# caishiqing/voice-tts

Measured on AMD Instinct MI355X. Metric: audio_seconds_per_second, higher is better.
Workload: dtype bf16

## Files before the change

### include/ixtts_hip.h

```cpp
#ifndef IXTTS_HIP_H
#define IXTTS_HIP_H

#include <stddef.h>
#include <stdint.h>

#ifdef __cplusplus
extern "C" {
#endif

#define IXTTS_OK 0
#define IXTTS_ERR_ARG (-1)
#define IXTTS_ERR_HIP (-2)
#define IXTTS_ERR_STATE (-3)
#define IXTTS_ERR_NOMEM (-4)
#define IXTTS_ERR_NAME (-5)

const char* ixtts_version(void);
const char* ixtts_last_error(void);

int ixtts_aa_snake_f32(const float* x_dev, float* y_dev, const float* up12_dev, const float* down12_dev,
                       const float* log_alpha_dev, const float* log_beta_dev, int B, int C, int T, void* stream);

size_t ixtts_attn_full_workspace_bytes(int B, int H, int T);
int ixtts_attn_full_f32(const float* q_dev, const float* k_dev, const float* v_dev, float* out_dev, int B, int H, int T,
                        int head_dim, long stride_b, long stride_t, long stride_h, long ostride_b, long ostride_t,
                        long ostride_h, float scale, void* workspace_dev, size_t workspace_bytes, void* stream);

size_t ixtts_attn_full_varlen_workspace_bytes(int nseq, int H, int total_tiles);
int ixtts_attn_full_varlen_f32(const float* q_dev, const float* k_dev, const float* v_dev, float* out_dev, const int* table_dev, int nseq,
                               int total_tiles, int n_work, int H, int head_dim, long stride_t, long stride_h, long ostride_t, long ostride_h,
                               float scale, void* workspace_dev, size_t workspace_bytes, void* stream);

int ixtts_adaln_rmsnorm_f32(const float* x_dev, const float* wb_dev, const float* g_dev, float* out_dev, int B, int T, int H, float eps,
                            void* stream);
int ixtts_ln_modulate_f32(const float* x_dev, const float* shift_scale_dev, float* out_dev, int B, int T, int H, float eps, void* stream);
int ixtts_rope_qk_f32(float* qkv_dev, const float* cos_sin_dev, int B, int T, int H, int head_dim, void* stream);
int ixtts_swiglu_f32(const float* u_dev, float* out_dev, long rows, int F, void* stream);
int ixtts_wn_gate_f32(const float* a_dev, const float* g_dev, float* out_dev, int B, int C, int T, long g_stride, int g_offset, void* stream);
int ixtts_wn_gate_rows_f32(const float* a_dev, const float* g_dev, float* out_dev, long rows, int C, long rows_per_batch, int B, long g_stride,
                           int g_offset, void* stream);
int ixtts_reflect_halo_rows_f32(float* p_dev, int B, int T, int C, int left, int right, void* stream);

int ixtts_adaln_rmsnorm_varlen_f32(const float* x_dev, const float* wb_dev, const float* g_dev, float* out_dev, const int* seq_off_dev, int nseq,
                                   long rows, int H, float eps, void* stream);
int ixtts_ln_modulate_varlen_f32(const float* x_dev, const float* shift_scale_dev, float* out_dev, const int* seq_off_dev, int nseq, long rows, int H,
                                 float eps, void* stream);
int ixtts_rope_qk_varlen_f32(float* qkv_dev, const float* cos_sin_dev, const int* seq_off_dev, int nseq, long rows, int H, int head_dim, void* stream);
int ixtts_wn_gate_rows_varlen_f32(const float* a_dev, const float* g_dev, float* out_dev, long rows, int C, const int* seq_off_dev, int nseq,
                                  long g_stride, int g_offset, void* stream);
int ixtts_reflect_halo_rows_varlen_f32(float* p_dev, const int* seq_off_dev, int nseq, int C, int left, int right, void* stream);

size_t ixtts_gemm_x6_packed_bytes(int N, int K);
int ixtts_gemm_x6_pack(const float* w_dev, void* packed_dev, int N, int K, void* stream);
long ixtts_gemm_x6_rows_padded(long rows);
int ixtts_gemm_x6_split(const float* a_dev, long lda, void* planes_dev, long rows, int K, void* stream);
int ixtts_gemm_x6_f32(const void* a_planes_dev, long rows_total, long row0, const void* packed_dev, const float* bias_dev, float* c_dev, long ldc,
                      int M, int N, int K, int accumulate, int tile, void* stream);
int ixtts_gemm_x6_pair_f32(const void* a_planes_dev, long rows_total, long row0, int taps, const void* packed_dev, const float* bias_dev,
                           const float* gate_dev, long gate_ld, long rows_per_batch, int nbatch, float* c_dev, long ldc, int M, int N, int K,
                           int epilogue, int tile, void* stream);
int ixtts_gemm_x6_pair_gate_varlen_f32(const void* a_planes_dev, long rows_total, long row0, int taps, const void* packed_dev, const float* bias_dev,
                                       const float* gate_dev, long gate_ld, const int* seq_off_dev, int nseq, float* c_dev, long ldc, int M, int N,
                                       int K, int tile, void* stream);

#define IXTTS_BIGVGAN_MAX_STAGES 8
#define IXTTS_BIGVGAN_MAX_RESK 4

typedef struct ixtts_bigvgan_cfg {
  int num_mels;
  int upsample_initial_channel;
  int n_stages;
  int upsample_rates[IXTTS_BIGVGAN_MAX_STAGES];
  int upsample_kernel_sizes[IXTTS_BIGVGAN_MAX_STAGES];
  int n_resblock_kernels;
  int resblock_kernel_sizes[IXTTS_BIGVGAN_MAX_RESK];
  int resblock_dilations[IXTTS_BIGVGAN_MAX_RESK][3];
  int max_frames;
  int fast_sin;
} ixtts_bigvgan_cfg;

typedef struct ixtts_bigvgan ixtts_bigvgan;

int ixtts_bigvgan_create(ixtts_bigvgan** out, const ixtts_bigvgan_cfg* cfg);
int ixtts_bigvgan_set_tensor(ixtts_bigvgan* h, const char* name, const float* data_host, const int64_t* shape, int ndim);
int ixtts_bigvgan_finalize(ixtts_bigvgan* h);
int ixtts_bigvgan_arena(ixtts_bigvgan* h, void** ptr_dev, size_t* bytes);
int ixtts_bigvgan_adopt_arena(ixtts_bigvgan* h);
int ixtts_bigvgan_forward(ixtts_bigvgan* h, const float* mel_dev, int B, int F, float* wav_dev, void* stream);
int ixtts_bigvgan_forward_varlen(ixtts_bigvgan* h, const float* mel_dev, const int* frames_dev, const int* frames_host, int B, int Fmax,
                                 float* wav_dev, void* stream);
double ixtts_bigvgan_flops(const ixtts_bigvgan* h, int B, int F);
int ixtts_bigvgan_destroy(ixtts_bigvgan* h);

#define IXTTS_DTYPE_F32 0
#define IXTTS_DTYPE_BF16 1
#define IXTTS_DTYPE_F16 2

typedef struct ixtts_gpt_cfg {
  int model_dim;
  int layers;
  int heads;
  int n_mel_codes;
  int n_mel_pos;
  int n_text_tokens;
  int n_text_pos;
  int start_mel_token;
  int stop_mel_token;
  int max_seq;
  int max_batch;
  int weight_dtype;
} ixtts_gpt_cfg;

#define IXTTS_NGRAM_MAX 8
#define IXTTS_SEQ_BIAS_MAX 64
#define IXTTS_SEQ_BIAS_LEN 8

typedef struct ixtts_sampler_cfg {
  float repetition_penalty;
  float temperature;
  int top_k;
  float top_p;
  int do_sample;
  int suppress_stop;
  uint64_t seed;
  float typical_mass;
  float length_penalty;
  int min_new_tokens;
  int no_repeat_ngram_size;
  float min_p;
  int exp_decay_start;
  double exp_decay_factor;
  float epsilon_cutoff;
  float eta_cutoff;
  int renormalize_logits;
  int forced_eos_step;
  int n_seq_bias;
} ixtts_sampler_cfg;

typedef struct ixtts_gpt ixtts_gpt;

// ... 103 lines not shown
```

### voice-tts_amd/_lib.py

```python
import ctypes as C
import os

HERE = os.path.dirname(os.path.abspath(__file__))
LIB_PATH = os.environ.get("IXTTS_LIB") or os.path.join(HERE, "libixtts_hip.so")

MAX_STAGES = 8
MAX_RESK = 4


class BigVGANCfg(C.Structure):
    _fields_ = [
        ("num_mels", C.c_int), ("upsample_initial_channel", C.c_int), ("n_stages", C.c_int),
        ("upsample_rates", C.c_int * MAX_STAGES), ("upsample_kernel_sizes", C.c_int * MAX_STAGES),
        ("n_resblock_kernels", C.c_int), ("resblock_kernel_sizes", C.c_int * MAX_RESK),
        ("resblock_dilations", (C.c_int * 3) * MAX_RESK), ("max_frames", C.c_int), ("fast_sin", C.c_int),
    ]


class GptCfg(C.Structure):
    _fields_ = [
        ("model_dim", C.c_int), ("layers", C.c_int), ("heads", C.c_int), ("n_mel_codes", C.c_int),
        ("n_mel_pos", C.c_int), ("n_text_tokens", C.c_int), ("n_text_pos", C.c_int),
        ("start_mel_token", C.c_int), ("stop_mel_token", C.c_int), ("max_seq", C.c_int),
        ("max_batch", C.c_int), ("weight_dtype", C.c_int),
    ]


class SamplerCfg(C.Structure):
    _fields_ = [
        ("repetition_penalty", C.c_float), ("temperature", C.c_float), ("top_k", C.c_int),
        ("top_p", C.c_float), ("do_sample", C.c_int), ("suppress_stop", C.c_int), ("seed", C.c_uint64),
        ("typical_mass", C.c_float), ("length_penalty", C.c_float),
        ("min_new_tokens", C.c_int), ("no_repeat_ngram_size", C.c_int), ("min_p", C.c_float),
        ("exp_decay_start", C.c_int), ("exp_decay_factor", C.c_double), ("epsilon_cutoff", C.c_float), ("eta_cutoff", C.c_float),
        ("renormalize_logits", C.c_int), ("forced_eos_step", C.c_int), ("n_seq_bias", C.c_int),
    ]


NGRAM_MAX = 8
SEQ_BIAS_MAX = 64
SEQ_BIAS_LEN = 8

QWEN_TOPK_MAX = 64
QWEN_MAX_EOS = 8
QWEN_MAX_SLOTS = 4


class QwenCfg(C.Structure):
    _fields_ = [
        ("hidden_size", C.c_int), ("layers", C.c_int), ("heads", C.c_int), ("kv_heads", C.c_int), ("head_dim", C.c_int),
        ("intermediate_size", C.c_int), ("vocab_size", C.c_int), ("rms_norm_eps", C.c_float), ("rope_theta", C.c_float),
        ("tie_word_embeddings", C.c_int), ("max_seq", C.c_int), ("weight_dtype", C.c_int), ("n_eos", C.c_int),
        ("eos_ids", C.c_int * QWEN_MAX_EOS),
    ]


class QwenSampling(C.Structure):
    _fields_ = [("do_sample", C.c_int), ("temperature", C.c_float), ("top_k", C.c_int), ("top_p", C.c_float), ("seed", C.c_uint64)]


_P = C.c_void_p
SYMBOLS = {
    "ixtts_version": (C.c_char_p, []),
    "ixtts_last_error": (C.c_char_p, []),
    "ixtts_aa_snake_f32": (C.c_int, [_P, _P, _P, _P, _P, _P, C.c_int, C.c_int, C.c_int, _P]),
    "ixtts_attn_full_workspace_bytes": (C.c_size_t, [C.c_int, C.c_int, C.c_int]),
    "ixtts_attn_full_f32": (C.c_int, [_P, _P, _P, _P, C.c_int, C.c_int, C.c_int, C.c_int, C.c_long, C.c_long, C.c_long, C.c_long, C.c_long,
                                      C.c_long, C.c_float, _P, C.c_size_t, _P]),
    "ixtts_attn_full_varlen_workspace_bytes": (C.c_size_t, [C.c_int, C.c_int, C.c_int]),
    "ixtts_attn_full_varlen_f32": (C.c_int, [_P, _P, _P, _P, _P, C.c_int, C.c_int, C.c_int, C.c_int, C.c_int, C.c_long, C.c_long, C.c_long, C.c_long,
                                             C.c_float, _P, C.c_size_t, _P]),
    "ixtts_adaln_rmsnorm_f32": (C.c_int, [_P, _P, _P, _P, C.c_int, C.c_int, C.c_int, C.c_float, _P]),
    "ixtts_ln_modulate_f32": (C.c_int, [_P, _P, _P, C.c_int, C.c_int, C.c_int, C.c_float, _P]),
    "ixtts_rope_qk_f32": (C.c_int, [_P, _P, C.c_int, C.c_int, C.c_int, C.c_int, _P]),
    "ixtts_swiglu_f32": (C.c_int, [_P, _P, C.c_long, C.c_int, _P]),
    "ixtts_wn_gate_f32": (C.c_int, [_P, _P, _P, C.c_int, C.c_int, C.c_int, C.c_long, C.c_int, _P]),
    "ixtts_wn_gate_rows_f32": (C.c_int, [_P, _P, _P, C.c_long, C.c_int, C.c_long, C.c_int, C.c_long, C.c_int, _P]),
    "ixtts_reflect_halo_rows_f32": (C.c_int, [_P, C.c_int, C.c_int, C.c_int, C.c_int, C.c_int, _P]),
    "ixtts_adaln_rmsnorm_varlen_f32": (C.c_int, [_P, _P, _P, _P, _P, C.c_int, C.c_long, C.c_int, C.c_float, _P]),
    "ixtts_ln_modulate_varlen_f32": (C.c_int, [_P, _P, _P, _P, C.c_int, C.c_long, C.c_int, C.c_float, _P]),
    "ixtts_rope_qk_varlen_f32": (C.c_int, [_P, _P, _P, C.c_int, C.c_long, C.c_int, C.c_int, _P]),
    "ixtts_wn_gate_rows_varlen_f32": (C.c_int, [_P, _P, _P, C.c_long, C.c_int, _P, C.c_int, C.c_long, C.c_int, _P]),
    "ixtts_reflect_halo_rows_varlen_f32": (C.c_int, [_P, _P, C.c_int, C.c_int, C.c_int, C.c_int, _P]),
    "ixtts_gemm_x6_packed_bytes": (C.c_size_t, [C.c_int, C.c_int]),
    "ixtts_gemm_x6_pack": (C.c_int, [_P, _P, C.c_int, C.c_int, _P]),
    "ixtts_gemm_x6_rows_padded": (C.c_long, [C.c_long]),
    "ixtts_gemm_x6_split": (C.c_int, [_P, C.c_long, _P, C.c_long, C.c_int, _P]),
    "ixtts_gemm_x6_f32": (C.c_int, [_P, C.c_long, C.c_long, _P, _P, _P, C.c_long, C.c_int, C.c_int, C.c_int, C.c_int, C.c_int, _P]),
    "ixtts_gemm_x6_pair_f32": (C.c_int, [_P, C.c_long, C.c_long, C.c_int, _P, _P, _P, C.c_long, C.c_long, C.c_int, _P, C.c_long, C.c_int, C.c_int,
                                         C.c_int, C.c_int, C.c_int, _P]),
    "ixtts_gemm_x6_pair_gate_varlen_f32": (C.c_int, [_P, C.c_long, C.c_long, C.c_int, _P, _P, _P, C.c_long, _P, C.c_int, _P, C.c_long, C.c_int, C.c_int,
                                                     C.c_int, C.c_int, _P]),
    "ixtts_bigvgan_create": (C.c_int, [C.POINTER(_P), C.POINTER(BigVGANCfg)]),
    "ixtts_bigvgan_set_tensor": (C.c_int, [_P, C.c_char_p, _P, C.POINTER(C.c_int64), C.c_int]),
    "ixtts_bigvgan_finalize": (C.c_int, [_P]),
    "ixtts_bigvgan_arena": (C.c_int, [_P, C.POINTER(_P), C.POINTER(C.c_size_t)]),
    "ixtts_bigvgan_adopt_arena": (C.c_int, [_P]),
    "ixtts_bigvgan_forward": (C.c_int, [_P, _P, C.c_int, C.c_int, _P, _P]),
    "ixtts_bigvgan_forward_varlen": (C.c_int, [_P, _P, _P, _P, C.c_int, C.c_int, _P, _P]),
    "ixtts_bigvgan_flops": (C.c_double, [_P, C.c_int, C.c_int]),
    "ixtts_bigvgan_destroy": (C.c_int, [_P]),
    "ixtts_gpt_create": (C.c_int, [C.POINTER(_P), C.POINTER(GptCfg)]),
    "ixtts_gpt_set_tensor": (C.c_int, [_P, C.c_char_p, _P, C.POINTER(C.c_int64), C.c_int]),
    "ixtts_gpt_finalize": (C.c_int, [_P]),
    "ixtts_gpt_arena": (C.c_int, [_P, C.POINTER(_P), C.POINTER(C.c_size_t)]),
    "ixtts_gpt_adopt_arena": (C.c_int, [_P]),
    "ixtts_gpt_share_arena": (C.c_int, [_P, _P]),
    "ixtts_gpt_prefill": (C.c_int, [_P, C.c_int, _P, C.c_int, C.c_int, _P]),
    "ixtts_gpt_decode": (C.c_int, [_P, C.c_int, C.c_int, C.POINTER(SamplerCfg), _P]),
    "ixtts_gpt_decode_slots": (C.c_int, [_P, C.c_int, C.c_int, C.POINTER(SamplerCfg), C.POINTER(C.c_uint32), _P]),
    "ixtts_gpt_read": (C.c_int, [_P, C.c_int, _P, C.c_int, C.POINTER(C.c_int), C.POINTER(C.c_int), _P]),
    "ixtts_gpt_read_logits": (C.c_int, [_P, C.c_int, _P, _P]),
    "ixtts_gpt_beam_begin": (C.c_int, [_P, C.c_int, _P]),
    "ixtts_gpt_beam_decode": (C.c_int, [_P, C.c_int, C.POINTER(SamplerCfg), _P]),
    "ixtts_gpt_beam_read": (C.c_int, [_P, C.c_int, _P, C.c_int, C.POINTER(C.c_int), C.POINTER(C.c_int), C.POINTER(C.c_float), _P, _P, _P, _P]),
    "ixtts_gpt_beam_force": (C.c_int, [_P, _P, C.c_int, _P]),
    "ixtts_gpt_beam_begin_group": (C.c_int, [_P, C.c_int, C.c_int, C.c_uint64, _P]),
    "ixtts_gpt_beam_park_group": (C.c_int, [_P, C.c_int, _P]),
    "ixtts_gpt_beam_decode_groups": (C.c_int, [_P, C.c_int, C.c_int, C.POINTER(SamplerCfg), _P]),
    "ixtts_gpt_beam_decode_groups_cfg": (C.c_int, [_P, C.c_int, C.c_int, C.POINTER(SamplerCfg), _P]),
    "ixtts_gpt_beam_read_group":(C.c_int, [_P, C.c_int, C.c_int, _P, C.c_int, C.POINTER(C.c_int), C.POINTER(C.c_int), C.POINTER(C.c_float), _P, _P, _P, _P]),
    "ixtts_gpt_beam_force_group": (C.c_int, [_P, C.c_int, _P, C.c_int, _P]),
    "ixtts_gpt_read_probs": (C.c_int, [_P, C.c_int, _P, _P]),
    "ixtts_gpt_force_next": (C.c_int, [_P, C.c_int, C.c_int32, _P]),
    "ixtts_gpt_set_bans": (C.c_int, [_P, C.c_int, _P, C.c_int, _P, C.c_int, _P]),
    "ixtts_gpt_set_sequence_bias": (C.c_int, [_P, C.c_int, _P, _P, _P, C.c_int, _P]),
    "ixtts_gpt_set_forced_eos": (C.c_int, [_P, C.c_int, _P, C.c_int, _P]),
    "ixtts_gpt_latent": (C.c_int, [_P, _P, C.c_int, _P, C.c_int, _P, _P]),
    "ixtts_gpt_bench_gemv": (C.c_int, [_P, C.c_int, C.c_int, C.c_int, _P]),
    "ixtts_gpt_step_bytes": (C.c_double, [_P, C.c_int, C.c_int]),
    "ixtts_gpt_max_batch": (C.c_int, []),
    "ixtts_gpt_max_batch_for": (C.c_int, [C.c_int]),
    "ixtts_gpt_destroy": (C.c_int, [_P]),
    "ixtts_qwen_create": (C.c_int, [C.POINTER(_P), C.POINTER(QwenCfg)]),
    "ixtts_qwen_set_tensor": (C.c_int, [_P, C.c_char_p, _P, C.POINTER(C.c_int64), C.c_int]),
    "ixtts_qwen_finalize": (C.c_int, [_P]),
    "ixtts_qwen_prefill": (C.c_int, [_P, _P, C.c_int, _P]),
    "ixtts_qwen_step": (C.c_int, [_P, C.c_int, C.POINTER(QwenSampling), _P]),
    "ixtts_qwen_read": (C.c_int, [_P, _P, C.c_int, C.POINTER(C.c_int), C.POINTER(C.c_int), _P]),
    "ixtts_qwen_generate": (C.c_int, [_P, C.c_int, C.POINTER(QwenSampling), _P, C.c_int, C.POINTER(C.c_int), C.POINTER(C.c_int), _P]),
    "ixtts_qwen_read_logits": (C.c_int, [_P, _P, _P]),
    "ixtts_qwen_read_kept": (C.c_int, [_P, _P, _P, C.c_int, C.POINTER(C.c_int), _P]),
    "ixtts_qwen_draw": (C.c_int, [_P, C.c_uint64, C.c_int, _P, _P]),
    "ixtts_qwen_step_bytes": (C.c_double, [_P, C.c_int]),
    "ixtts_qwen_create_slots": (C.c_int, [C.POINTER(_P), C.POINTER(QwenCfg), C.c_int]),
    "ixtts_qwen_prefill_slots": (C.c_int, [_P, C.c_int, _P, _P, _P]),
    "ixtts_qwen_step_slots": (C.c_int, [_P, C.c_int, C.c_int, C.POINTER(QwenSampling), _P]),
    "ixtts_qwen_generate_slots": (C.c_int, [_P, C.c_int, C.c_int, C.POINTER(QwenSampling), _P]),
    "ixtts_qwen_read_slot": (C.c_int, [_P, C.c_int, _P, C.c_int, C.POINTER(C.c_int), C.POINTER(C.c_int), _P]),
    "ixtts_qwen_read_logits_slot": (C.c_int, [_P, C.c_int, _P, _P]),
    "ixtts_qwen_read_kept_slot": (C.c_int, [_P, C.c_int, _P, _P, C.c_int, C.POINTER(C.c_int), _P]),
    "ixtts_qwen_destroy": (C.c_int, [_P]),
}

_lib = None


class IxttsError(RuntimeError):
    pass


def lib():
    global _lib
    if _lib is not None:
        return _lib
    import torch
# ... 40 lines not shown
```

### voice-tts_amd/csrc/attn_full.h

```cpp
#pragma once
#include "common.h"

namespace ixtts {

constexpr int AF_D = 64;
constexpr int AF_KT = 64;
constexpr int AF_QW = 32;
constexpr int AF_WAVES = 4;
constexpr int AF_KSPLIT = 4;
constexpr int AX_KSPLIT = 5;

struct AttnFullArgs {
  const float* q;
  const float* k;
  const float* v;
  float* o;
  long sb, st, sh;
  long osb, ost, osh;
  int B, H, T;
  float scale;
  float* ws_o;
  float* ws_ml;
  const int* vl_tab;
  int vl_n, vl_tiles;
};

size_t attn_full_x3_plane_bytes(int B, int H, int T);
int launch_attn_full_x3(const AttnFullArgs& a, void* planes, bool split, hipStream_t st);
int launch_attn_full_x3_varlen(const AttnFullArgs& a, void* planes, int n_work, hipStream_t st);

}
```

### voice-tts_amd/csrc/attn_full.hip

```cpp
#include "attn_full.h"

namespace ixtts {

typedef float f32x16 __attribute__((ext_vector_type(16)));

constexpr int AF_KP = AF_D + 4;

template <int KSPLIT>
__global__ __launch_bounds__(AF_WAVES * 64) void attn_full_f32_kernel(AttnFullArgs a) {
  __shared__ __attribute__((aligned(16))) float Ks[AF_KT * AF_KP];
  __shared__ __attribute__((aligned(16))) float Vs[AF_KT * AF_D];
  const int bh = blockIdx.y, b = bh / a.H, h = bh % a.H;
  const int lane = threadIdx.x & 63, wave = threadIdx.x >> 6;
  const int l31 = lane & 31, lh = lane >> 5;
  const int q0 = blockIdx.x * (AF_WAVES * AF_QW) + wave * AF_QW;
  const float* qb = a.q + b * a.sb + h * a.sh;
  const float* kb = a.k + b * a.sb + h * a.sh;
  const float* vb = a.v + b * a.sb + h * a.sh;

  float qr[AF_D / 2];
  {
    const int qi = min(q0 + l31, a.T - 1);
    const float* qp = qb + (long)qi * a.st + 4 * lh;
    const float qs = a.scale * 1.4426950408889634f;
// ... 78 lines not shown
        for (int r = 0; r < 16; ++r) ot[j][r] *= alpha;
    }
    float psum = 0.f;
    const float* vp = Vs + (4 * lh) * AF_D + l31;
    float va[2][2];
    va[0][0] = vp[0];
    va[0][1] = vp[32];
#pragma unroll
    for (int s = 0; s < 32; ++s) {
      const int j = s >> 4, r = s & 15;
      if (s + 1 < 32) {
        const int j1 = (s + 1) >> 4, r1 = (s + 1) & 15;
        const float* vrow = vp + (j1 * 32 + (r1 & 3) + 8 * (r1 >> 2)) * AF_D;
        va[(s + 1) & 1][0] = vrow[0];
        va[(s + 1) & 1][1] = vrow[32];
      }
      const float pv = __builtin_amdgcn_exp2f(st[j][r] - mn);
      psum += pv;
      ot[0] = __builtin_amdgcn_mfma_f32_32x32x2f32(va[s & 1][0], pv, ot[0], 0, 0, 0);
      ot[1] = __builtin_amdgcn_mfma_f32_32x32x2f32(va[s & 1][1], pv, ot[1], 0, 0, 0);
    }
    psum += __shfl_xor(psum, 32, 64);
    l_run = l_run * alpha + psum;
  }
  const int qi = q0 + l31;
  if (qi < a.T) {
    if constexpr (KSPLIT == 1) {
      const float inv = 1.0f / l_run;
      float* op = a.o + b * a.osb + (long)qi * a.ost + h * a.osh;
#pragma unroll
      for (int j = 0; j < 2; ++j)
#pragma unroll
        for (int r = 0; r < 16; ++r) op[j * 32 + (r & 3) + 8 * (r >> 2) + 4 * lh] = ot[j][r] * inv;
    } else {
      const long row = ((long)blockIdx.z * a.B * a.H + bh) * a.T + qi;
      float* op = a.ws_o + row * AF_D;
#pragma unroll
      for (int j = 0; j < 2; ++j)
#pragma unroll
        for (int r = 0; r < 16; ++r) op[j * 32 + (r & 3) + 8 * (r >> 2) + 4 * lh] = ot[j][r];
      if (lh == 0) *reinterpret_cast<float2*>(a.ws_ml + row * 2) = make_float2(m_run, l_run);
    }
  }
}

template <int KSPLIT>
__global__ __launch_bounds__(256) void attn_full_merge_kernel(AttnFullArgs a) {
  const long row = (long)blockIdx.x * 4 + (threadIdx.x >> 6);
  const long rows = (long)a.B * a.H * a.T;
  if (row >= rows) return;
  const int d = threadIdx.x & 63;
  const int t = (int)(row % a.T);
  const int bh = (int)(row / a.T), b = bh / a.H, h = bh % a.H;
  float2 ml[KSPLIT];
  float o[KSPLIT];
  float M = -INFINITY;
#pragma unroll
  for (int sp = 0; sp < KSPLIT; ++sp) {
    ml[sp] = *reinterpret_cast<const float2*>(a.ws_ml + ((long)sp * rows + row) * 2);
    o[sp] = a.ws_o[((long)sp * rows + row) * AF_D + d];
    M = fmaxf(M, ml[sp].x);
  }
  float L = 0.f, O = 0.f;
#pragma unroll
  for (int sp = 0; sp < KSPLIT; ++sp) {
    const float w = (ml[sp].x > -INFINITY) ? __builtin_amdgcn_exp2f(ml[sp].x - M) : 0.f;
    L = fmaf(ml[sp].y, w, L);
    O = fmaf(o[sp], w, O);
  }
  a.o[b * a.osb + (long)t * a.ost + h * a.osh + d] = O / L;
}

}

static size_t attn_partials_bytes(int B, int H, int T) {
  return (size_t)(ixtts::AF_KSPLIT > ixtts::AX_KSPLIT ? ixtts::AF_KSPLIT : ixtts::AX_KSPLIT) * B * H * T * (ixtts::AF_D + 2) * sizeof(float);
}

extern "C" size_t ixtts_attn_full_workspace_bytes(int B, int H, int T) {
  if (B <= 0 || H <= 0 || T <= 0) return 0;
  return attn_partials_bytes(B, H, T) + ixtts::attn_full_x3_plane_bytes(B, H, T);
}

extern "C" int ixtts_attn_full_f32(const float* q_dev, const float* k_dev, const float* v_dev, float* out_dev, int B, int H, int T,
                                   int head_dim, long stride_b, long stride_t, long stride_h, long ostride_b, long ostride_t,
                                   long ostride_h, float scale, void* workspace_dev, size_t workspace_bytes, void* stream) {
  using namespace ixtts;
  IX_ARG(q_dev && k_dev && v_dev && out_dev, "attn_full: null pointer");
  IX_ARG(head_dim == AF_D, "attn_full: head_dim %d (only 64 is built)", head_dim);
  IX_ARG(B > 0 && H > 0 && T > 0 && (long)B * H <= 65535, "attn_full: bad shape B=%d H=%d T=%d", B, H, T);
  IX_ARG(stride_t % 4 == 0 && stride_h % 4 == 0 && stride_b % 4 == 0, "attn_full: strides must keep 16-byte row alignment");
  AttnFullArgs a;
  a.q = q_dev; a.k = k_dev; a.v = v_dev; a.o = out_dev;
  a.sb = stride_b; a.st = stride_t; a.sh = stride_h;
  a.osb = ostride_b; a.ost = ostride_t; a.osh = ostride_h;
  a.B = B; a.H = H; a.T = T; a.scale = scale;
  a.ws_o = a.ws_ml = nullptr;
  a.vl_tab = nullptr; a.vl_n = a.vl_tiles = 0;
  hipStream_t st = (hipStream_t)stream;
  const int qblocks = ceil_div(T, AF_WAVES * AF_QW);
  const bool have_ws = workspace_dev && workspace_bytes >= ixtts_attn_full_workspace_bytes(B, H, T);
  const bool split = have_ws && T > 4 * AF_KT && (long)qblocks * B * H * AF_WAVES < 2 * 1024;
  const char* mode = getenv("IXTTS_ATTN_FULL");
  const bool x3 = !(mode && strcmp(mode, "f32") == 0);
  const bool use_x3 = x3 && have_ws;
  if (split) {
    a.ws_o = reinterpret_cast<float*>(workspace_dev);
    a.ws_ml = a.ws_o + (size_t)(use_x3 ? AX_KSPLIT : AF_KSPLIT) * B * H * T * AF_D;
  }
  if (use_x3) {
    IX_TRY(launch_attn_full_x3(a, reinterpret_cast<char*>(workspace_dev) + attn_partials_bytes(B, H, T), split, st));
    if (split) {
      const long rows = (long)B * H * T;
      hipLaunchKernelGGL(attn_full_merge_kernel<AX_KSPLIT>, dim3((unsigned)((rows + 3) / 4)), dim3(256), 0, st, a);
    }
    IX_HIP(hipGetLastError());
    return IXTTS_OK;
  }
  if (split) {
    hipLaunchKernelGGL(attn_full_f32_kernel<AF_KSPLIT>, dim3(qblocks, B * H, AF_KSPLIT), dim3(AF_WAVES * 64), 0, st, a);
    const long rows = (long)B * H * T;
    hipLaunchKernelGGL(attn_full_merge_kernel<AF_KSPLIT>, dim3((unsigned)((rows + 3) / 4)), dim3(256), 0, st, a);
  } else {
    hipLaunchKernelGGL(attn_full_f32_kernel<1>, dim3(qblocks, B * H), dim3(AF_WAVES * 64), 0, st, a);
  }
  IX_HIP(hipGetLastError());
  return IXTTS_OK;
}

extern "C" size_t ixtts_attn_full_varlen_workspace_bytes(int nseq, int H, int total_tiles) {
  if (nseq <= 0 || H <= 0 || total_tiles <= 0) return 0;
  return (size_t)H * total_tiles * 2 * 3 * 8 * 64 * 16;
}

extern "C" int ixtts_attn_full_varlen_f32(const float* q_dev, const float* k_dev, const float* v_dev, float* out_dev, const int* table_dev, int nseq,
                                          int total_tiles, int n_work, int H, int head_dim, long stride_t, long stride_h, long ostride_t, long ostride_h,
                                          float scale, void* workspace_dev, size_t workspace_bytes, void* stream) {
  using namespace ixtts;
  IX_ARG(q_dev && k_dev && v_dev && out_dev && table_dev, "attn_full_varlen: null pointer");
  IX_ARG(head_dim == AF_D, "attn_full_varlen: head_dim %d (only 64 is built)", head_dim);
  IX_ARG(nseq > 0 && total_tiles >= nseq && n_work >= nseq && H > 0 && H <= 65535, "attn_full_varlen: bad shape nseq=%d tiles=%d work=%d H=%d", nseq, total_tiles,
         n_work, H);
  IX_ARG(stride_t % 4 == 0 && stride_h % 4 == 0, "attn_full_varlen: strides must keep 16-byte row alignment");
  IX_ARG(workspace_dev && workspace_bytes >= ixtts_attn_full_varlen_workspace_bytes(nseq, H, total_tiles), "attn_full_varlen: workspace of %zu bytes, %zu needed",
         workspace_bytes, ixtts_attn_full_varlen_workspace_bytes(nseq, H, total_tiles));
  AttnFullArgs a;
  a.q = q_dev; a.k = k_dev; a.v = v_dev; a.o = out_dev;
  a.sb = 0; a.st = stride_t; a.sh = stride_h;
  a.osb = 0; a.ost = ostride_t; a.osh = ostride_h;
  a.B = 1; a.H = H; a.T = 0; a.scale = scale;
  a.ws_o = a.ws_ml = nullptr;
  a.vl_tab = table_dev; a.vl_n = nseq; a.vl_tiles = total_tiles;
  return launch_attn_full_x3_varlen(a, workspace_dev, n_work, (hipStream_t)stream);
}
```

### voice-tts_amd/csrc/attn_full_x3.hip

```cpp
#include "attn_full.h"

namespace ixtts {

typedef float ax_f32x16 __attribute__((ext_vector_type(16)));
typedef __bf16 ax_bf16x8 __attribute__((ext_vector_type(8)));

constexpr int AX_TILE_UNITS = 3 * 8 * 64;
constexpr int AX_WAVES = 4;

size_t attn_full_x3_plane_bytes(int B, int H, int T) {
  const size_t tiles = (size_t)(T + AF_KT - 1) / AF_KT;
  return (size_t)B * H * tiles * 2 * AX_TILE_UNITS * 16;
}


template <bool VL>
__global__ __launch_bounds__(256) void attn_kv_planes_kernel(AttnFullArgs a, uint4* __restrict__ planes) {
  int tile = blockIdx.x, T = a.T;
  const float *kb, *vb;
  uint4* kdst;
  if constexpr (VL) {
    const int h = blockIdx.y, s = seq_of_row(a.vl_tab + a.vl_n + 1, a.vl_n, tile);
    const int r0 = a.vl_tab[s];
    T = a.vl_tab[s + 1] - r0;
    kdst = planes + ((size_t)h * a.vl_tiles + tile) * 2 * AX_TILE_UNITS;
    tile -= a.vl_tab[a.vl_n + 1 + s];
    kb = a.k + (long)r0 * a.st + h * a.sh;
    vb = a.v + (long)r0 * a.st + h * a.sh;
  } else {
    const int bh = blockIdx.y, b = bh / a.H, h = bh % a.H;
    const int n_tiles = (a.T + AF_KT - 1) / AF_KT;
    kb = a.k + b * a.sb + h * a.sh;
    vb = a.v + b * a.sb + h * a.sh;
    kdst = planes + ((size_t)bh * n_tiles + tile) * 2 * AX_TILE_UNITS;
  }
  uint4* vdst = kdst + AX_TILE_UNITS;
  const int t0 = tile * AF_KT;
#pragma unroll
  for (int i = 0; i < 2; ++i) {
    const int uid = threadIdx.x + 256 * i;
    const int key = uid >> 3, oct = uid & 7;
    const int t = t0 + key;
    float v[8];
    const float4* src = reinterpret_cast<const float4*>(kb + (long)min(t, T - 1) * a.st + 8 * oct);
    const float4 x0 = src[0], x1 = src[1];
    const bool live = t < T;
    v[0] = live ? x0.x : 0.f; v[1] = live ? x0.y : 0.f; v[2] = live ? x0.z : 0.f; v[3] = live ? x0.w : 0.f;
    v[4] = live ? x1.x : 0.f; v[5] = live ? x1.y : 0.f; v[6] = live ? x1.z : 0.f; v[7] = live ? x1.w : 0.f;
    uint4 ph, pm, pl;
    split8_bf16x3(v, ph, pm, pl);
    kdst[(0 * 8 + oct) * 64 + key] = ph;
    kdst[(1 * 8 + oct) * 64 + key] = pm;
    kdst[(2 * 8 + oct) * 64 + key] = pl;
  }
#pragma unroll
  for (int i = 0; i < 2; ++i) {
    const int d = threadIdx.x & 63, un = (threadIdx.x >> 6) + 4 * i;
    const int j = un >> 2, u = (un >> 1) & 1, kh = un & 1;
    float v[8];
#pragma unroll
    for (int e = 0; e < 8; ++e) {
      const int t = t0 + 32 * j + 16 * u + 8 * (e >> 2) + 4 * kh + (e & 3);
      const float x = vb[(long)min(t, T - 1) * a.st + d];
      v[e] = t < T ? x : 0.f;
    }
    uint4 ph, pm, pl;
    split8_bf16x3(v, ph, pm, pl);
    vdst[(0 * 8 + un) * 64 + d] = ph;
    vdst[(1 * 8 + un) * 64 + d] = pm;
    vdst[(2 * 8 + un) * 64 + d] = pl;
  }
}

template <int KSPLIT, bool VL = false>
__global__ __launch_bounds__(AX_WAVES * 64, 3) void attn_full_x3_kernel(AttnFullArgs a, const uint4* __restrict__ planes) {
  __shared__ uint4 Ks[AX_TILE_UNITS];
  __shared__ uint4 Vs[AX_TILE_UNITS];
  static_assert(!VL || KSPLIT == 1, "packed sequences: no key-range split");
  const int lane = threadIdx.x & 63, wave = threadIdx.x >> 6;
  const int l31 = lane & 31, lh = lane >> 5;
  int T, q0;
  const float* qb;
  const uint4* pb;
  float* ob;
  if constexpr (VL) {
    const int h = blockIdx.y;
    const int* w = a.vl_tab + 2 * (a.vl_n + 1) + 2 * blockIdx.x;
    const int s = w[0], r0 = a.vl_tab[s];
    T = a.vl_tab[s + 1] - r0;
    q0 = w[1] * (AX_WAVES * AF_QW) + wave * AF_QW;
    qb = a.q + (long)r0 * a.st + h * a.sh;
    pb = planes + ((size_t)h * a.vl_tiles + a.vl_tab[a.vl_n + 1 + s]) * 2 * AX_TILE_UNITS;
    ob = a.o + (long)r0 * a.ost + h * a.osh;
  } else {
    const int bh = blockIdx.y, b = bh / a.H, h = bh % a.H;
    T = a.T;
    q0 = blockIdx.x * (AX_WAVES * AF_QW) + wave * AF_QW;
    qb = a.q + b * a.sb + h * a.sh;
    pb = planes + (size_t)bh * ((T + AF_KT - 1) / AF_KT) * 2 * AX_TILE_UNITS;
    ob = a.o + b * a.osb + h * a.osh;
  }

  uint4 qp[4][3];
  {
    const int qi = min(q0 + l31, T - 1);
    const float* qrow = qb + (long)qi * a.st + 8 * lh;
    const float qs = a.scale * 1.4426950408889634f;
#pragma unroll
    for (int s = 0; s < 4; ++s) {
      const float4 x0 = *reinterpret_cast<const float4*>(qrow + 16 * s), x1 = *reinterpret_cast<const float4*>(qrow + 16 * s + 4);
      const float v[8] = {x0.x * qs, x0.y * qs, x0.z * qs, x0.w * qs, x1.x * qs, x1.y * qs, x1.z * qs, x1.w * qs};
      split8_bf16x3(v, qp[s][0], qp[s][1], qp[s][2]);
    }
  }
  ax_f32x16 ot[2];
#pragma unroll
  for (int j = 0; j < 2; ++j)
#pragma unroll
    for (int r = 0; r < 16; ++r) ot[j][r] = 0.f;
  float m_run = -INFINITY, l_run = 0.f;

  const int n_tiles = (T + AF_KT - 1) / AF_KT;
  const int tiles_per = (n_tiles + KSPLIT - 1) / KSPLIT;
  const int tile_lo = KSPLIT > 1 ? blockIdx.z * tiles_per : 0;
  const int tile_hi = KSPLIT > 1 ? min(n_tiles, tile_lo + tiles_per) : n_tiles;
  auto issue_tile = [&](const uint4* __restrict__ src, uint4* __restrict__ dst) {
#pragma unroll
    for (int i = 0; i < AX_TILE_UNITS / (AX_WAVES * 64); ++i)
      __builtin_amdgcn_global_load_lds((const __attribute__((address_space(1))) void*)(src + i * (AX_WAVES * 64) + threadIdx.x),
                                       (__attribute__((address_space(3))) void*)(dst + i * (AX_WAVES * 64) + wave * 64), 16, 0, 0);
  };
  auto mfma6x2 = [](ax_f32x16& c0, ax_f32x16& c1, const uint4 (&A0)[3], const uint4 (&A1)[3], const uint4 (&Bq)[3]) {
    const ax_bf16x8 a0h = __builtin_bit_cast(ax_bf16x8, A0[0]), a0m = __builtin_bit_cast(ax_bf16x8, A0[1]), a0l = __builtin_bit_cast(ax_bf16x8, A0[2]);
    const ax_bf16x8 a1h = __builtin_bit_cast(ax_bf16x8, A1[0]), a1m = __builtin_bit_cast(ax_bf16x8, A1[1]), a1l = __builtin_bit_cast(ax_bf16x8, A1[2]);
    const ax_bf16x8 bh_ = __builtin_bit_cast(ax_bf16x8, Bq[0]), bm = __builtin_bit_cast(ax_bf16x8, Bq[1]), bl = __builtin_bit_cast(ax_bf16x8, Bq[2]);
    c0 = __builtin_amdgcn_mfma_f32_32x32x16_bf16(a0l, bh_, c0, 0, 0, 0);
    c1 = __builtin_amdgcn_mfma_f32_32x32x16_bf16(a1l, bh_, c1, 0, 0, 0);
    c0 = __builtin_amdgcn_mfma_f32_32x32x16_bf16(a0h, bl, c0, 0, 0, 0);
    c1 = __builtin_amdgcn_mfma_f32_32x32x16_bf16(a1h, bl, c1, 0, 0, 0);
    c0 = __builtin_amdgcn_mfma_f32_32x32x16_bf16(a0m, bm, c0, 0, 0, 0);
    c1 = __builtin_amdgcn_mfma_f32_32x32x16_bf16(a1m, bm, c1, 0, 0, 0);
    c0 = __builtin_amdgcn_mfma_f32_32x32x16_bf16(a0m, bh_, c0, 0, 0, 0);
    c1 = __builtin_amdgcn_mfma_f32_32x32x16_bf16(a1m, bh_, c1, 0, 0, 0);
    c0 = __builtin_amdgcn_mfma_f32_32x32x16_bf16(a0h, bm, c0, 0, 0, 0);
    c1 = __builtin_amdgcn_mfma_f32_32x32x16_bf16(a1h, bm, c1, 0, 0, 0);
    c0 = __builtin_amdgcn_mfma_f32_32x32x16_bf16(a0h, bh_, c0, 0, 0, 0);
    c1 = __builtin_amdgcn_mfma_f32_32x32x16_bf16(a1h, bh_, c1, 0, 0, 0);
  };
  if (tile_lo < tile_hi) issue_tile(pb + (size_t)tile_lo * 2 * AX_TILE_UNITS, Ks);
  for (int tile = tile_lo; tile < tile_hi; ++tile) {
    const int t0 = tile * AF_KT;
    asm volatile("s_waitcnt vmcnt(0)" ::: "memory");
    __builtin_amdgcn_s_barrier();
    issue_tile(pb + ((size_t)tile * 2 + 1) * AX_TILE_UNITS, Vs);
    ax_f32x16 st[2];
#pragma unroll
    for (int j = 0; j < 2; ++j)
#pragma unroll
      for (int r = 0; r < 16; ++r) st[j][r] = 0.f;
    const uint4* kp = Ks + lh * 64 + l31;
#pragma unroll
    for (int s = 0; s < 4; ++s) {
      uint4 ka[2][3];
#pragma unroll
      for (int j = 0; j < 2; ++j)
#pragma unroll
        for (int pl = 0; pl < 3; ++pl) ka[j][pl] = kp[(pl * 8 + 2 * s) * 64 + 32 * j];
      mfma6x2(st[0], st[1], ka[0], ka[1], qp[s]);
    }
    if (t0 + AF_KT > T) {
#pragma unroll
      for (int j = 0; j < 2; ++j)
#pragma unroll
        for (int r = 0; r < 16; ++r) {
          const int key = t0 + j * 32 + (r & 3) + 8 * (r >> 2) + 4 * lh;
          if (key >= T) st[j][r] = -INFINITY;
        }
    }
    float tmax = -INFINITY;
#pragma unroll
    for (int j = 0; j < 2; ++j)
#pragma unroll
      for (int r = 0; r < 16; ++r) tmax = fmaxf(tmax, st[j][r]);
    tmax = fmaxf(tmax, __shfl_xor(tmax, 32, 64));
    const float mn = fmaxf(m_run, tmax);
    const float alpha = __builtin_amdgcn_exp2f(m_run - mn);
    m_run = mn;
    if (alpha != 1.0f) {
#pragma unroll
      for (int j = 0; j < 2; ++j)
#pragma unroll
        for (int r = 0; r < 16; ++r) ot[j][r] *= alpha;
    }
    float psum = 0.f;
#pragma unroll
    for (int j = 0; j < 2; ++j)
#pragma unroll
      for (int r = 0; r < 16; ++r) {
        st[j][r] = __builtin_amdgcn_exp2f(st[j][r] - mn);
        psum += st[j][r];
      }
    psum += __shfl_xor(psum, 32, 64);
    l_run = l_run * alpha + psum;
    asm volatile("s_waitcnt vmcnt(0)" ::: "memory");
    __builtin_amdgcn_s_barrier();
    if (tile + 1 < tile_hi) issue_tile(pb + (size_t)(tile + 1) * 2 * AX_TILE_UNITS, Ks);
    const uint4* vp = Vs + lh * 64 + l31;
#pragma unroll
    for (int s = 0; s < 4; ++s) {
      const int j = s >> 1, u = s & 1;
      uint4 va[2][3];
#pragma unroll
      for (int dh = 0; dh < 2; ++dh)
#pragma unroll
        for (int pl = 0; pl < 3; ++pl) va[dh][pl] = vp[(pl * 8 + 2 * s) * 64 + 32 * dh];
      uint4 pp[3];
      {
        float pv[8];
#pragma unroll
        for (int e = 0; e < 8; ++e) pv[e] = st[j][8 * u + e];
        split8_bf16x3(pv, pp[0], pp[1], pp[2]);
      }
      mfma6x2(ot[0], ot[1], va[0], va[1], pp);
    }
  }
  asm volatile("s_waitcnt vmcnt(0)" ::: "memory");
  const int qi = q0 + l31;
  if (qi < T) {
    if constexpr (KSPLIT == 1) {
      const float inv = 1.0f / l_run;
      float* op = ob + (long)qi * a.ost;
#pragma unroll
      for (int j = 0; j < 2; ++j)
#pragma unroll
        for (int r = 0; r < 16; ++r) op[j * 32 + (r & 3) + 8 * (r >> 2) + 4 * lh] = ot[j][r] * inv;
    } else {
      const long row = ((long)blockIdx.z * a.B * a.H + blockIdx.y) * T + qi;
      float* op = a.ws_o + row * AF_D;
#pragma unroll
      for (int j = 0; j < 2; ++j)
#pragma unroll
        for (int r = 0; r < 16; ++r) op[j * 32 + (r & 3) + 8 * (r >> 2) + 4 * lh] = ot[j][r];
      if (lh == 0) *reinterpret_cast<float2*>(a.ws_ml + row * 2) = make_float2(m_run, l_run);
    }
  }
}

int launch_attn_full_x3(const AttnFullArgs& a, void* planes, bool split, hipStream_t st) {
  const int n_tiles = ceil_div(a.T, AF_KT);
  const int qblocks = ceil_div(a.T, AX_WAVES * AF_QW);
  uint4* pl = reinterpret_cast<uint4*>(planes);
  hipLaunchKernelGGL(attn_kv_planes_kernel<false>, dim3(n_tiles, a.B * a.H), dim3(256), 0, st, a, pl);
  if (split) hipLaunchKernelGGL(attn_full_x3_kernel<AX_KSPLIT>, dim3(qblocks, a.B * a.H, AX_KSPLIT), dim3(AX_WAVES * 64), 0, st, a, (const uint4*)pl);
  else hipLaunchKernelGGL(attn_full_x3_kernel<1>, dim3(qblocks, a.B * a.H), dim3(AX_WAVES * 64), 0, st, a, (const uint4*)pl);
  IX_HIP(hipGetLastError());
  return IXTTS_OK;
}

int launch_attn_full_x3_varlen(const AttnFullArgs& a, void* planes, int n_work, hipStream_t st) {
  uint4* pl = reinterpret_cast<uint4*>(planes);
  hipLaunchKernelGGL(attn_kv_planes_kernel<true>, dim3(a.vl_tiles, a.H), dim3(256), 0, st, a, pl);
  hipLaunchKernelGGL((attn_full_x3_kernel<1, true>), dim3(n_work, a.H), dim3(AX_WAVES * 64), 0, st, a, (const uint4*)pl);
  IX_HIP(hipGetLastError());
  return IXTTS_OK;
}

}
```

### voice-tts_amd/csrc/common.h

```cpp
#pragma once
#include <type_traits>
#include <hip/hip_runtime.h>
#include <hip/hip_bf16.h>
#include <stdint.h>
#include <stdio.h>
#include <string.h>
#include <string>

#include "../../include/ixtts_hip.h"

namespace ixtts {

void set_error(const char* fmt, ...);

#define IX_HIP(expr)                                                                   \
  do {                                                                                 \
    hipError_t _e = (expr);                                                            \
    if (_e != hipSuccess) {                                                            \
      ::ixtts::set_error("%s:%d: %s -> %s", __FILE__, __LINE__, #expr, hipGetErrorString(_e)); \
      return IXTTS_ERR_HIP;                                                            \
    }                                                                                  \
  } while (0)

#define IX_ARG(cond, ...)                  \
  do {                                     \
    if (!(cond)) {                         \
      ::ixtts::set_error(__VA_ARGS__);     \
      return IXTTS_ERR_ARG;                \
    }                                      \
  } while (0)

#define IX_TRY(expr)            \
  do {                          \
    int _r = (expr);            \
    if (_r != IXTTS_OK) return _r; \
  } while (0)

static inline int ceil_div(int a, int b) { return (a + b - 1) / b; }
static inline size_t align_up(size_t x, size_t a) { return (x + a - 1) / a * a; }

typedef __hip_bfloat16 bf16;

__device__ __forceinline__ float bf16_bits_to_f32(unsigned short b) {
  return __uint_as_float(((unsigned int)b) << 16);
}
__device__ __forceinline__ int seq_of_row(const int* __restrict__ off, int n, long row) {
  int lo = 0, hi = n - 1;
  while (lo < hi) {
    const int mid = (lo + hi + 1) >> 1;
    if ((long)off[mid] <= row) lo = mid;
    else hi = mid - 1;
  }
  return lo;
}

__device__ __forceinline__ float lo_bf16(unsigned int w) { return __uint_as_float(w << 16); }
__device__ __forceinline__ float hi_bf16(unsigned int w) { return __uint_as_float(w & 0xffff0000u); }

typedef _Float16 f16;
constexpr float F16_MAX = 65504.0f;
__device__ __forceinline__ float lo_f16(unsigned int w) { return (float)__builtin_bit_cast(f16, (unsigned short)(w & 0xffffu)); }
__device__ __forceinline__ float hi_f16(unsigned int w) { return (float)__builtin_bit_cast(f16, (unsigned short)(w >> 16)); }
__device__ __forceinline__ f16 f16_sat(float v) { return (f16)__builtin_fminf(__builtin_fmaxf(v, -F16_MAX), F16_MAX); }
template <typename T>
__device__ __forceinline__ void unpack8(const uint4& r, float (&o)[8]);
template <>
__device__ __forceinline__ void unpack8<bf16>(const uint4& r, float (&o)[8]) {
  o[0] = lo_bf16(r.x); o[1] = hi_bf16(r.x); o[2] = lo_bf16(r.y); o[3] = hi_bf16(r.y);
  o[4] = lo_bf16(r.z); o[5] = hi_bf16(r.z); o[6] = lo_bf16(r.w); o[7] = hi_bf16(r.w);
}
template <>
__device__ __forceinline__ void unpack8<f16>(const uint4& r, float (&o)[8]) {
  o[0] = lo_f16(r.x); o[1] = hi_f16(r.x); o[2] = lo_f16(r.y); o[3] = hi_f16(r.y);
  o[4] = lo_f16(r.z); o[5] = hi_f16(r.z); o[6] = lo_f16(r.w); o[7] = hi_f16(r.w);
}

template <int CTRL, int ROW_MASK, int BANK_MASK>
__device__ __forceinline__ float dpp_take(float v) {
  return __builtin_bit_cast(float, __builtin_amdgcn_update_dpp(0, __builtin_bit_cast(int, v), CTRL, ROW_MASK, BANK_MASK, true));
}
__device__ __forceinline__ float wave_sum63(float v) {
  float s = v + dpp_take<0x111, 0xf, 0xf>(v);
  s += dpp_take<0x112, 0xf, 0xf>(v);
  s += dpp_take<0x113, 0xf, 0xf>(v);
  s += dpp_take<0x114, 0xf, 0xe>(s);
  s += dpp_take<0x118, 0xf, 0xc>(s);
  s += dpp_take<0x142, 0xa, 0xf>(s);
  s += dpp_take<0x143, 0xc, 0xf>(s);
  return s;
}
__device__ __forceinline__ float wave_sum(float v) {
  return __builtin_bit_cast(float, __builtin_amdgcn_readlane(__builtin_bit_cast(int, wave_sum63(v)), 63));
}
__device__ __forceinline__ float wave_max(float v) {
#pragma unroll
  for (int o = 32; o >= 1; o >>= 1) v = fmaxf(v, __shfl_xor(v, o, 64));
  return v;
}
template <int CTRL, int ROW_MASK, int BANK_MASK>
__device__ __forceinline__ float dpp_take_or_self(float v) {
  return __builtin_bit_cast(float, __builtin_amdgcn_update_dpp(__builtin_bit_cast(int, v), __builtin_bit_cast(int, v), CTRL, ROW_MASK, BANK_MASK, false));
}
__device__ __forceinline__ float wave_max_dpp(float v) {
  float s = fmaxf(v, dpp_take_or_self<0x111, 0xf, 0xf>(v));
  s = fmaxf(s, dpp_take_or_self<0x112, 0xf, 0xf>(v));
  s = fmaxf(s, dpp_take_or_self<0x113, 0xf, 0xf>(v));
  s = fmaxf(s, dpp_take_or_self<0x114, 0xf, 0xe>(s));
  s = fmaxf(s, dpp_take_or_self<0x118, 0xf, 0xc>(s));
  s = fmaxf(s, dpp_take_or_self<0x142, 0xa, 0xf>(s));
  s = fmaxf(s, dpp_take_or_self<0x143, 0xc, 0xf>(s));
  return __builtin_bit_cast(float, __builtin_amdgcn_readlane(__builtin_bit_cast(int, s), 63));
}
__device__ __forceinline__ unsigned int wave_scan_u32(unsigned int v) {
  auto take = [](unsigned int x, auto ctrl, auto rm, auto bm) {
    return (unsigned int)__builtin_amdgcn_update_dpp(0, (int)x, decltype(ctrl)::value, decltype(rm)::value, decltype(bm)::value, true);
  };
  using std::integral_constant;
  unsigned int s = v + take(v, integral_constant<int, 0x111>{}, integral_constant<int, 0xf>{}, integral_constant<int, 0xf>{});
  s += take(v, integral_constant<int, 0x112>{}, integral_constant<int, 0xf>{}, integral_constant<int, 0xf>{});
  s += take(v, integral_constant<int, 0x113>{}, integral_constant<int, 0xf>{}, integral_constant<int, 0xf>{});
  s += take(s, integral_constant<int, 0x114>{}, integral_constant<int, 0xf>{}, integral_constant<int, 0xe>{});
  s += take(s, integral_constant<int, 0x118>{}, integral_constant<int, 0xf>{}, integral_constant<int, 0xc>{});
  s += take(s, integral_constant<int, 0x142>{}, integral_constant<int, 0xa>{}, integral_constant<int, 0xf>{});
  s += take(s, integral_constant<int, 0x143>{}, integral_constant<int, 0xc>{}, integral_constant<int, 0xf>{});
  return s;
}

__device__ __forceinline__ int wave_min_i32_dpp(int v) {
  auto take = [](int x, auto ctrl, auto rm, auto bm) {
    return __builtin_amdgcn_update_dpp(x, x, decltype(ctrl)::value, decltype(rm)::value, decltype(bm)::value, false);
  };
  using std::integral_constant;
  int s = min(v, take(v, integral_constant<int, 0x111>{}, integral_constant<int, 0xf>{}, integral_constant<int, 0xf>{}));
  s = min(s, take(v, integral_constant<int, 0x112>{}, integral_constant<int, 0xf>{}, integral_constant<int, 0xf>{}));
  s = min(s, take(v, integral_constant<int, 0x113>{}, integral_constant<int, 0xf>{}, integral_constant<int, 0xf>{}));
  s = min(s, take(s, integral_constant<int, 0x114>{}, integral_constant<int, 0xf>{}, integral_constant<int, 0xe>{}));
// ... 30 lines not shown
```

### voice-tts_amd/csrc/dit_ops.hip

```cpp
#include "common.h"

namespace ixtts {

constexpr int ROW_NV = 8;

template <bool CENTER>
__global__ __launch_bounds__(256) void row_norm_mod_kernel(const float* __restrict__ x, const float* __restrict__ mw, const float* __restrict__ mb,
                                                           const float* __restrict__ g, float* __restrict__ out, long rows, int T, int H, long mstride,
                                                           float eps, float wadd, const int* __restrict__ seq_off = nullptr, int nseq = 0) {
  const long row = (long)blockIdx.x * 4 + (threadIdx.x >> 6);
  if (row >= rows) return;
  const int lane = threadIdx.x & 63;
  const int H4 = H >> 2;
  const float4* xr = reinterpret_cast<const float4*>(x + row * H);
  float4 v[ROW_NV];
#pragma unroll
  for (int i = 0; i < ROW_NV; ++i) {
    const int c = lane + 64 * i;
    v[i] = (c < H4) ? xr[c] : make_float4(0.f, 0.f, 0.f, 0.f);
  }
  float mean = 0.f;
  if constexpr (CENTER) {
    float s = 0.f;
#pragma unroll
    for (int i = 0; i < ROW_NV; ++i) s += (v[i].x + v[i].y) + (v[i].z + v[i].w);
    mean = wave_sum(s) / (float)H;
  }
  float q = 0.f;
#pragma unroll
  for (int i = 0; i < ROW_NV; ++i) {
    const int c = lane + 64 * i;
    if (c < H4) {
      const float a = v[i].x - mean, b = v[i].y - mean, cc = v[i].z - mean, d = v[i].w - mean;
      q += (a * a + b * b) + (cc * cc + d * d);
    }
  }
  float var = wave_sum(q) / (float)H;
  float corr = 0.f;
  if constexpr (CENTER) {
    if (mean * mean > 16.0f * var) {
      float r = 0.f;
#pragma unroll
      for (int i = 0; i < ROW_NV; ++i)
        if (lane + 64 * i < H4) r += ((v[i].x - mean) + (v[i].y - mean)) + ((v[i].z - mean) + (v[i].w - mean));
      corr = wave_sum(r) / (float)H;
      float q2 = 0.f;
#pragma unroll
      for (int i = 0; i < ROW_NV; ++i)
        if (lane + 64 * i < H4) {
          const float a = (v[i].x - mean) - corr, b = (v[i].y - mean) - corr, cc = (v[i].z - mean) - corr, d = (v[i].w - mean) - corr;
          q2 += (a * a + b * b) + (cc * cc + d * d);
        }
      var = wave_sum(q2) / (float)H;
    }
  }
  const float rstd = 1.0f / sqrtf(var + eps);
  const long bidx = seq_off ? seq_of_row(seq_off, nseq, row) : row / T;
  const float4* w4 = reinterpret_cast<const float4*>(mw + bidx * mstride);
  const float4* b4 = reinterpret_cast<const float4*>(mb + bidx * mstride);
  const float4* g4 = reinterpret_cast<const float4*>(g);
  float4* o4 = reinterpret_cast<float4*>(out + row * H);
#pragma unroll
  for (int i = 0; i < ROW_NV; ++i) {
    const int c = lane + 64 * i;
    if (c < H4) {
      const float4 w = w4[c], b = b4[c];
      float4 n;
      if constexpr (CENTER) n = make_float4(((v[i].x - mean) - corr) * rstd, ((v[i].y - mean) - corr) * rstd, ((v[i].z - mean) - corr) * rstd, ((v[i].w - mean) - corr) * rstd);
      else n = make_float4(v[i].x * rstd, v[i].y * rstd, v[i].z * rstd, v[i].w * rstd);
      if (g) {
        const float4 gg = g4[c];
        n.x *= gg.x; n.y *= gg.y; n.z *= gg.z; n.w *= gg.w;
      }
      o4[c] = make_float4(fmaf(w.x + wadd, n.x, b.x), fmaf(w.y + wadd, n.y, b.y), fmaf(w.z + wadd, n.z, b.z), fmaf(w.w + wadd, n.w, b.w));
    }
  }
}

__global__ __launch_bounds__(256) void rope_qk_kernel(float* __restrict__ qkv, const float2* __restrict__ tab, long rows, int T, int H, int hd,
                                                      const int* __restrict__ seq_off = nullptr, int nseq = 0) {
  const int per_row = (2 * H) >> 2;
  const long idx = (long)blockIdx.x * 256 + threadIdx.x;
  if (idx >= rows * per_row) return;
  const long row = idx / per_row;
  const int c4 = (int)(idx % per_row);
  const int col = c4 * 4;
  const int t = seq_off ? (int)(row - seq_off[seq_of_row(seq_off, nseq, row)]) : (int)(row % T);
  const int p = (col % hd) >> 1;
  float4* ptr = reinterpret_cast<float4*>(qkv + row * 3 * H + col);
  const float4 v = *ptr;
  const float2 f0 = tab[(long)t * (hd >> 1) + p], f1 = tab[(long)t * (hd >> 1) + p + 1];
  *ptr = make_float4(v.x * f0.x - v.y * f0.y, v.y * f0.x + v.x * f0.y, v.z * f1.x - v.w * f1.y, v.w * f1.x + v.z * f1.y);
}

__global__ __launch_bounds__(256) void swiglu_kernel(const float* __restrict__ u, float* __restrict__ out, long rows, int Fd) {
  const int F4 = Fd >> 2;
  const long idx = (long)blockIdx.x * 256 + threadIdx.x;
  if (idx >= rows * F4) return;
  const long row = idx / F4;
  const int c = (int)(idx % F4);
  const float4 a = reinterpret_cast<const float4*>(u + row * 2 * Fd)[c];
  const float4 b = reinterpret_cast<const float4*>(u + row * 2 * Fd + Fd)[c];
  auto f = [](float x, float y) { return x / (1.0f + expf(-x)) * y; };
  reinterpret_cast<float4*>(out + row * Fd)[c] = make_float4(f(a.x, b.x), f(a.y, b.y), f(a.z, b.z), f(a.w, b.w));
}

__global__ __launch_bounds__(256) void wn_gate_kernel(const float* __restrict__ a, const float* __restrict__ gvec, float* __restrict__ out, int B, int C, int T,
                                                      long gstride, int goff) {
  const long idx = (long)blockIdx.x * 256 + threadIdx.x;
  const long n = (long)B * C * T;
  if (idx >= n) return;
  const int t = (int)(idx % T);
  const int c = (int)((idx / T) % C);
  const int b = (int)(idx / ((long)T * C));
  const float ga = gvec[b * gstride + goff + c], gb = gvec[b * gstride + goff + C + c];
  const float xa = a[((long)b * 2 * C + c) * T + t] + ga;
  const float xb = a[((long)b * 2 * C + C + c) * T + t] + gb;
  out[idx] = tanhf(xa) * (1.0f / (1.0f + expf(-xb)));
}

__global__ __launch_bounds__(256) void wn_gate_rows_kernel(const float* __restrict__ a, const float* __restrict__ gvec, float* __restrict__ out, long rows, int C,
                                                           long rows_per_batch, int B, long gstride, int goff, const int* __restrict__ seq_off = nullptr) {
  const long idx = (long)blockIdx.x * 256 + threadIdx.x;
  const int C4 = C >> 2;
  if (idx >= rows * C4) return;
  const long r = idx / C4;
  const int c = (int)(idx % C4) * 4;
  const int b = seq_off ? seq_of_row(seq_off, B, r) : (int)min(r / rows_per_batch, (long)B - 1);
  const float4 xa = *reinterpret_cast<const float4*>(a + r * 2 * C + c);
  const float4 xb = *reinterpret_cast<const float4*>(a + r * 2 * C + C + c);
  const float4 ga = *reinterpret_cast<const float4*>(gvec + b * gstride + goff + c);
  const float4 gb = *reinterpret_cast<const float4*>(gvec + b * gstride + goff + C + c);
  float4 o;
  o.x = tanhf(xa.x + ga.x) * (1.0f / (1.0f + expf(-(xb.x + gb.x))));
  o.y = tanhf(xa.y + ga.y) * (1.0f / (1.0f + expf(-(xb.y + gb.y))));
  o.z = tanhf(xa.z + ga.z) * (1.0f / (1.0f + expf(-(xb.z + gb.z))));
  o.w = tanhf(xa.w + ga.w) * (1.0f / (1.0f + expf(-(xb.w + gb.w))));
  *reinterpret_cast<float4*>(out + r * C + c) = o;
}

__global__ __launch_bounds__(256) void reflect_halo_rows_kernel(float* __restrict__ p, int B, int T, int C, int left, int right) {
  const int C4 = C >> 2;
  const long idx = (long)blockIdx.x * 256 + threadIdx.x;
  const long per_b = (long)(left + right) * C4;
  if (idx >= per_b * B) return;
  const int b = (int)(idx / per_b);
  const int h = (int)((idx % per_b) / C4);
  const int c = (int)(idx % C4) * 4;
  float* base = p + (long)b * (left + T + right) * C;
  const int dst = h < left ? left - 1 - h : left + T + (h - left);
  const int src = h < left ? left + h + 1 : left + T - 2 - (h - left);
  *reinterpret_cast<float4*>(base + (long)dst * C + c) = *reinterpret_cast<const float4*>(base + (long)src * C + c);
}

__global__ __launch_bounds__(256) void reflect_halo_rows_varlen_kernel(float* __restrict__ p, const int* __restrict__ off, int n, int C, int left, int right) {
  const int C4 = C >> 2;
  const long idx = (long)blockIdx.x * 256 + threadIdx.x;
  const long per_b = (long)(left + right) * C4;
  if (idx >= per_b * n) return;
  const int b = (int)(idx / per_b);
  const int h = (int)((idx % per_b) / C4);
  const int c = (int)(idx % C4) * 4;
  const int o0 = off[b], T = off[b + 1] - o0 - left - right;
  if (T <= left || T <= right) return;
  float* base = p + (long)o0 * C;
  const int dst = h < left ? left - 1 - h : left + T + (h - left);
  const int src = h < left ? left + h + 1 : left + T - 2 - (h - left);
  *reinterpret_cast<float4*>(base + (long)dst * C + c) = *reinterpret_cast<const float4*>(base + (long)src * C + c);
}

}

using namespace ixtts;

extern "C" int ixtts_adaln_rmsnorm_f32(const float* x_dev, const float* wb_dev, const float* g_dev, float* out_dev, int B, int T, int H, float eps,
                                       void* stream) {
  IX_ARG(x_dev && wb_dev && g_dev && out_dev, "adaln_rmsnorm: null pointer");
  IX_ARG(B > 0 && T > 0 && H > 0 && H % 4 == 0 && H <= 64 * ROW_NV * 4, "adaln_rmsnorm: bad shape B=%d T=%d H=%d", B, T, H);
  const long rows = (long)B * T;
  hipLaunchKernelGGL(row_norm_mod_kernel<false>, dim3((unsigned)((rows + 3) / 4)), dim3(256), 0, (hipStream_t)stream, x_dev, wb_dev, wb_dev + H, g_dev, out_dev,
                     rows, T, H, (long)2 * H, eps, 0.0f);
  IX_HIP(hipGetLastError());
  return IXTTS_OK;
}

extern "C" int ixtts_ln_modulate_f32(const float* x_dev, const float* shift_scale_dev, float* out_dev, int B, int T, int H, float eps, void* stream) {
  IX_ARG(x_dev && shift_scale_dev && out_dev, "ln_modulate: null pointer");
  IX_ARG(B > 0 && T > 0 && H > 0 && H % 4 == 0 && H <= 64 * ROW_NV * 4, "ln_modulate: bad shape B=%d T=%d H=%d", B, T, H);
  const long rows = (long)B * T;
  hipLaunchKernelGGL(row_norm_mod_kernel<true>, dim3((unsigned)((rows + 3) / 4)), dim3(256), 0, (hipStream_t)stream, x_dev, shift_scale_dev + H, shift_scale_dev,
                     (const float*)nullptr, out_dev, rows, T, H, (long)2 * H, eps, 1.0f);
  IX_HIP(hipGetLastError());
  return IXTTS_OK;
}

extern "C" int ixtts_rope_qk_f32(float* qkv_dev, const float* cos_sin_dev, int B, int T, int H, int head_dim, void* stream) {
  IX_ARG(qkv_dev && cos_sin_dev, "rope_qk: null pointer");
  IX_ARG(B > 0 && T > 0 && H > 0 && head_dim > 0 && head_dim % 4 == 0 && H % head_dim == 0, "rope_qk: bad shape B=%d T=%d H=%d hd=%d", B, T, H, head_dim);
  const long n = (long)B * T * (2 * H / 4);
  hipLaunchKernelGGL(rope_qk_kernel, dim3((unsigned)((n + 255) / 256)), dim3(256), 0, (hipStream_t)stream, qkv_dev, reinterpret_cast<const float2*>(cos_sin_dev),
                     (long)B * T, T, H, head_dim);
  IX_HIP(hipGetLastError());
  return IXTTS_OK;
}

extern "C" int ixtts_swiglu_f32(const float* u_dev, float* out_dev, long rows, int F, void* stream) {
  IX_ARG(u_dev && out_dev, "swiglu: null pointer");
  IX_ARG(rows > 0 && F > 0 && F % 4 == 0, "swiglu: bad shape rows=%ld F=%d", rows, F);
  const long n = rows * (F / 4);
  hipLaunchKernelGGL(swiglu_kernel, dim3((unsigned)((n + 255) / 256)), dim3(256), 0, (hipStream_t)stream, u_dev, out_dev, rows, F);
  IX_HIP(hipGetLastError());
  return IXTTS_OK;
}

extern "C" int ixtts_wn_gate_f32(const float* a_dev, const float* g_dev, float* out_dev, int B, int C, int T, long g_stride, int g_offset, void* stream) {
  IX_ARG(a_dev && g_dev && out_dev, "wn_gate: null pointer");
  IX_ARG(B > 0 && C > 0 && T > 0 && g_offset >= 0, "wn_gate: bad shape B=%d C=%d T=%d", B, C, T);
  const long n = (long)B * C * T;
  hipLaunchKernelGGL(wn_gate_kernel, dim3((unsigned)((n + 255) / 256)), dim3(256), 0, (hipStream_t)stream, a_dev, g_dev, out_dev, B, C, T, g_stride, g_offset);
  IX_HIP(hipGetLastError());
  return IXTTS_OK;
}

extern "C" int ixtts_wn_gate_rows_f32(const float* a_dev, const float* g_dev, float* out_dev, long rows, int C, long rows_per_batch, int B, long g_stride,
                                      int g_offset, void* stream) {
  IX_ARG(a_dev && g_dev && out_dev, "wn_gate_rows: null pointer");
  IX_ARG(rows > 0 && C > 0 && C % 4 == 0 && rows_per_batch > 0 && B > 0 && g_offset >= 0 && g_offset % 4 == 0 && g_stride % 4 == 0,
         "wn_gate_rows: bad shape rows=%ld C=%d rows_per_batch=%ld B=%d", rows, C, rows_per_batch, B);
  const long n = rows * (C / 4);
  hipLaunchKernelGGL(wn_gate_rows_kernel, dim3((unsigned)((n + 255) / 256)), dim3(256), 0, (hipStream_t)stream, a_dev, g_dev, out_dev, rows, C, rows_per_batch, B,
                     g_stride, g_offset);
  IX_HIP(hipGetLastError());
  return IXTTS_OK;
}

extern "C" int ixtts_reflect_halo_rows_f32(float* p_dev, int B, int T, int C, int left, int right, void* stream) {
  IX_ARG(p_dev, "reflect_halo_rows: null pointer");
  IX_ARG(B > 0 && C > 0 && C % 4 == 0 && left >= 0 && right >= 0 && T > left && T > right, "reflect_halo_rows: bad shape B=%d T=%d C=%d left=%d right=%d", B, T, C,
         left, right);
  const long n = (long)B * (left + right) * (C / 4);
  if (n == 0) return IXTTS_OK;
  hipLaunchKernelGGL(reflect_halo_rows_kernel, dim3((unsigned)((n + 255) / 256)), dim3(256), 0, (hipStream_t)stream, p_dev, B, T, C, left, right);
  IX_HIP(hipGetLastError());
  return IXTTS_OK;
}


extern "C" int ixtts_adaln_rmsnorm_varlen_f32(const float* x_dev, const float* wb_dev, const float* g_dev, float* out_dev, const int* seq_off_dev, int nseq,
                                              long rows, int H, float eps, void* stream) {
  IX_ARG(x_dev && wb_dev && g_dev && out_dev && seq_off_dev, "adaln_rmsnorm_varlen: null pointer");
  IX_ARG(nseq > 0 && rows > 0 && H > 0 && H % 4 == 0 && H <= 64 * ROW_NV * 4, "adaln_rmsnorm_varlen: bad shape nseq=%d rows=%ld H=%d", nseq, rows, H);
  hipLaunchKernelGGL(row_norm_mod_kernel<false>, dim3((unsigned)((rows + 3) / 4)), dim3(256), 0, (hipStream_t)stream, x_dev, wb_dev, wb_dev + H, g_dev, out_dev,
                     rows, 1, H, (long)2 * H, eps, 0.0f, seq_off_dev, nseq);
  IX_HIP(hipGetLastError());
  return IXTTS_OK;
}

extern "C" int ixtts_ln_modulate_varlen_f32(const float* x_dev, const float* shift_scale_dev, float* out_dev, const int* seq_off_dev, int nseq, long rows, int H,
                                            float eps, void* stream) {
  IX_ARG(x_dev && shift_scale_dev && out_dev && seq_off_dev, "ln_modulate_varlen: null pointer");
  IX_ARG(nseq > 0 && rows > 0 && H > 0 && H % 4 == 0 && H <= 64 * ROW_NV * 4, "ln_modulate_varlen: bad shape nseq=%d rows=%ld H=%d", nseq, rows, H);
  hipLaunchKernelGGL(row_norm_mod_kernel<true>, dim3((unsigned)((rows + 3) / 4)), dim3(256), 0, (hipStream_t)stream, x_dev, shift_scale_dev + H, shift_scale_dev,
                     (const float*)nullptr, out_dev, rows, 1, H, (long)2 * H, eps, 1.0f, seq_off_dev, nseq);
  IX_HIP(hipGetLastError());
  return IXTTS_OK;
}

extern "C" int ixtts_rope_qk_varlen_f32(float* qkv_dev, const float* cos_sin_dev, const int* seq_off_dev, int nseq, long rows, int H, int head_dim, void* stream) {
  IX_ARG(qkv_dev && cos_sin_dev && seq_off_dev, "rope_qk_varlen: null pointer");
  IX_ARG(nseq > 0 && rows > 0 && H > 0 && head_dim > 0 && head_dim % 4 == 0 && H % head_dim == 0, "rope_qk_varlen: bad shape nseq=%d rows=%ld H=%d hd=%d", nseq,
         rows, H, head_dim);
  const long n = rows * (2 * H / 4);
  hipLaunchKernelGGL(rope_qk_kernel, dim3((unsigned)((n + 255) / 256)), dim3(256), 0, (hipStream_t)stream, qkv_dev, reinterpret_cast<const float2*>(cos_sin_dev),
                     rows, 1, H, head_dim, seq_off_dev, nseq);
  IX_HIP(hipGetLastError());
  return IXTTS_OK;
}

extern "C" int ixtts_wn_gate_rows_varlen_f32(const float* a_dev, const float* g_dev, float* out_dev, long rows, int C, const int* seq_off_dev, int nseq,
                                             long g_stride, int g_offset, void* stream) {
  IX_ARG(a_dev && g_dev && out_dev && seq_off_dev, "wn_gate_rows_varlen: null pointer");
  IX_ARG(rows > 0 && C > 0 && C % 4 == 0 && nseq > 0 && g_offset >= 0 && g_offset % 4 == 0 && g_stride % 4 == 0,
         "wn_gate_rows_varlen: bad shape rows=%ld C=%d nseq=%d", rows, C, nseq);
  const long n = rows * (C / 4);
  hipLaunchKernelGGL(wn_gate_rows_kernel, dim3((unsigned)((n + 255) / 256)), dim3(256), 0, (hipStream_t)stream, a_dev, g_dev, out_dev, rows, C, (long)1, nseq,
                     g_stride, g_offset, seq_off_dev);
  IX_HIP(hipGetLastError());
  return IXTTS_OK;
}

extern "C" int ixtts_reflect_halo_rows_varlen_f32(float* p_dev, const int* seq_off_dev, int nseq, int C, int left, int right, void* stream) {
  IX_ARG(p_dev && seq_off_dev, "reflect_halo_rows_varlen: null pointer");
  IX_ARG(nseq > 0 && C > 0 && C % 4 == 0 && left >= 0 && right >= 0, "reflect_halo_rows_varlen: bad shape nseq=%d C=%d left=%d right=%d", nseq, C, left, right);
  const long n = (long)nseq * (left + right) * (C / 4);
  if (n == 0) return IXTTS_OK;
  hipLaunchKernelGGL(reflect_halo_rows_varlen_kernel, dim3((unsigned)((n + 255) / 256)), dim3(256), 0, (hipStream_t)stream, p_dev, seq_off_dev, nseq, C, left,
                     right);
  IX_HIP(hipGetLastError());
  return IXTTS_OK;
}
```

### voice-tts_amd/csrc/gemm_x6.hip

```cpp
#include "common.h"

namespace ixtts {

typedef float gx_f32x16 __attribute__((ext_vector_type(16)));
typedef __bf16 gx_bf16x8 __attribute__((ext_vector_type(8)));
typedef float gx_f32x4 __attribute__((ext_vector_type(4)));
typedef unsigned int gx_u32x4 __attribute__((ext_vector_type(4)));


__global__ void gemm_x6_pack_kernel(const float* __restrict__ w, uint4* __restrict__ out, int N, int K, int Npad) {
  const long total = (long)(K / 8) * Npad;
  for (long idx = blockIdx.x * (long)blockDim.x + threadIdx.x; idx < total; idx += (long)gridDim.x * blockDim.x) {
    const int n = (int)(idx % Npad);
    const int ko = (int)(idx / Npad);
    float v[8];
#pragma unroll
    for (int e = 0; e < 8; ++e) v[e] = n < N ? w[(long)n * K + ko * 8 + e] : 0.f;
    uint4 ph, pm, pl;
    split8_bf16x3(v, ph, pm, pl);
    const int g = ko >> 1, kh = ko & 1;
    uint4* base = out + ((long)g * 6) * Npad + n;
    base[(long)(0 * 2 + kh) * Npad] = ph;
    base[(long)(1 * 2 + kh) * Npad] = pm;
    base[(long)(2 * 2 + kh) * Npad] = pl;
  }
}

__global__ __launch_bounds__(256) void gemm_x6_split_kernel(const float* __restrict__ a, long lda, uint4* __restrict__ out, int M, int K, long Mpad) {
  __shared__ float tile[64][65];
  const int r0 = blockIdx.x * 64, k0 = blockIdx.y * 64;
  const int t = threadIdx.x;
#pragma unroll
  for (int i = 0; i < 4; ++i) {
    const int r = (t >> 4) + 16 * i, kq = t & 15;
    float4 v = make_float4(0.f, 0.f, 0.f, 0.f);
    if (r0 + r < M) v = *reinterpret_cast<const float4*>(a + (long)(r0 + r) * lda + k0 + 4 * kq);
    tile[r][4 * kq + 0] = v.x; tile[r][4 * kq + 1] = v.y; tile[r][4 * kq + 2] = v.z; tile[r][4 * kq + 3] = v.w;
  }
  __syncthreads();
#pragma unroll
  for (int u = 0; u < 2; ++u) {
    const int r = t & 63, o = (t >> 6) + 4 * u;
    float v[8];
#pragma unroll
    for (int e = 0; e < 8; ++e) v[e] = tile[r][o * 8 + e];
    uint4 ph, pm, pl;
    split8_bf16x3(v, ph, pm, pl);
    const int ko = (k0 >> 3) + o, g = ko >> 1, kh = ko & 1;
    uint4* base = out + ((long)g * 6) * Mpad + r0 + r;
    base[(long)(0 * 2 + kh) * Mpad] = ph;
    base[(long)(1 * 2 + kh) * Mpad] = pm;
    base[(long)(2 * 2 + kh) * Mpad] = pl;
  }
}

enum { EPI_PLAIN = 0, EPI_SWIGLU = 1, EPI_GATE = 2 };

struct GemmX6Params {
  const uint4* Ap;
  long Mpad;
  long arow0;
  const uint4* Wp;
  const float* bias;
  float* C;
  long ldc;
  int M, N, Npad, K, accumulate, m_tiles, n_tiles;
  int tap_steps;
  int epi;
  const float* gate;
  long gate_ld, rows_per_batch;
  int nbatch;
  const int* gate_seq_off;
  unsigned long long* dbg;
};


template <int MT, int NT, int NST, int EPI = EPI_PLAIN, int ACC = 0, int SEQ = 0, int DBG = 0, int PIN = 0>
__global__ __launch_bounds__(256, (NST * (MT + NT) * 6 * 64 * 16 <= 80 * 1024) ? 2 : 1) void gemm_x6_kernel(GemmX6Params p) {
  constexpr int BM = 64 * MT, BN = 64 * NT;
  constexpr int A_UNITS = 6 * BM, W_UNITS = 6 * BN, STAGE = A_UNITS + W_UNITS;
  constexpr int NDMA = (6 * (MT + NT)) / 4;
  constexpr int NA = (6 * MT) / 4, NW = NDMA - NA;
  static_assert((6 * MT) % 4 == 0 && (6 * NT) % 4 == 0, "the A pieces and the W pieces are each dealt evenly to the 4 waves");
  static_assert(EPI == EPI_PLAIN || (ACC == 0 && NT == 2), "pair epilogues: the wave's two 32-column blocks are the two halves");
  static_assert(EPI == EPI_GATE || SEQ == 0, "the sequence table belongs to the gate epilogue");
  constexpr int D = NST - 1;
  extern __shared__ uint4 smem[];

  const int nwg = p.m_tiles * p.n_tiles;
  const int bid = blockIdx.x;
  const int xcd = bid & 7, idx = bid >> 3;
  const int qd = nwg >> 3, rm = nwg & 7;
  const int lin = (xcd < rm ? xcd * (qd + 1) : rm * (qd + 1) + (xcd - rm) * qd) + idx;
  const int m_tile = lin / p.n_tiles, n_tile = lin - m_tile * p.n_tiles;
  const int m0 = m_tile * BM, n0 = n_tile * BN;

  const int tid = threadIdx.x, lane = tid & 63;
  const int wave = __builtin_amdgcn_readfirstlane(tid >> 6);
  const int wm = wave >> 1, wn = wave & 1;
  const int l31 = lane & 31, lh = lane >> 5;

  gx_f32x16 acc[MT][NT];
#pragma unroll
  for (int i = 0; i < MT; ++i)
#pragma unroll
    for (int j = 0; j < NT; ++j)
#pragma unroll
      for (int r = 0; r < 16; ++r) acc[i][j][r] = 0.f;

  const uint4* asrc = p.Ap + p.arow0 + m0 + lane;
  const uint4* wsrc = p.Wp + n0 + lane;
  long a_off[NA], w_off[NW];
  int a_lds[NA], w_lds[NW];
#pragma unroll
  for (int q = 0; q < NA; ++q) {
    const int e = q * 4 + wave, run = e / MT, piece = e % MT;
    a_off[q] = run * p.Mpad + piece * 64;
    a_lds[q] = run * BM + piece * 64;
  }
// ... 156 lines not shown
    const bool col_ok = col < p.N;
    const float bv = (p.bias != nullptr && col_ok) ? p.bias[col] : 0.f;
#pragma unroll
    for (int i = 0; i < MT; ++i) {
      const int rbase = m0 + wm * (32 * MT) + i * 32 + 4 * lh;
#pragma unroll
      for (int r = 0; r < 16; ++r) {
        const int row = rbase + (r & 3) + 8 * (r >> 2);
        if (col_ok && row < p.M) {
          float* c = p.C + (long)row * p.ldc + col;
          float v = acc[i][j][r] + bv;
          if constexpr (ACC != 0) v += *c;
          *c = v;
        }
      }
    }
  }
  if constexpr (DBG == 3) {
    asm volatile("s_waitcnt vmcnt(0)" ::: "memory");
    wg_stamp(3);
  }
}

template <int MT, int NT, int NST, int EPI = EPI_PLAIN, int ACC = 0, int SEQ = 0, int DBG = 0, int PIN = 0>
static int launch_gemm_x6(GemmX6Params p, hipStream_t st) {
  constexpr int BM = 64 * MT, BN = 64 * NT;
  constexpr size_t smem = (size_t)NST * (6 * BM + 6 * BN) * 16;
  static_assert(smem <= 160 * 1024, "LDS stages of this tile shape");
  p.m_tiles = ceil_div(p.M, BM);
  p.n_tiles = ceil_div(p.N, BN);
  IX_ARG((long)p.n_tiles * BN <= p.Npad, "gemm_x6: packed weights padded to %d features, the %d-wide tile needs %d", p.Npad, BN, p.n_tiles * BN);
  const int taps = (p.K >> 4) / p.tap_steps;
  IX_ARG(p.arow0 + (long)p.m_tiles * BM + taps - 1 <= p.Mpad, "gemm_x6: activation planes hold %ld rows, the %d-row tiles reach row %ld", p.Mpad, BM,
         p.arow0 + (long)p.m_tiles * BM + taps - 1);
  auto kern = gemm_x6_kernel<MT, NT, NST, EPI, ACC, SEQ, DBG, PIN>;
  static bool done = false;
  if (!done) {
    IX_HIP(hipFuncSetAttribute((const void*)kern, hipFuncAttributeMaxDynamicSharedMemorySize, (int)smem));
    done = true;
  }
  hipLaunchKernelGGL(kern, dim3(p.m_tiles * p.n_tiles), dim3(256), smem, st, p);
  IX_HIP(hipGetLastError());
  return IXTTS_OK;
}

template <int MT, int NT, int NST, bool PAIR>
static int launch_gemm_x6_epilogue(const GemmX6Params& p, hipStream_t st) {
  if (p.epi == EPI_PLAIN) return p.accumulate ? launch_gemm_x6<MT, NT, NST, EPI_PLAIN, 1>(p, st) : launch_gemm_x6<MT, NT, NST, EPI_PLAIN, 0>(p, st);
  if constexpr (PAIR) {
    if (p.epi == EPI_SWIGLU) return launch_gemm_x6<MT, NT, NST, EPI_SWIGLU>(p, st);
    if (p.epi == EPI_GATE)
      return p.gate_seq_off ? launch_gemm_x6<MT, NT, NST, EPI_GATE, 0, 1>(p, st) : launch_gemm_x6<MT, NT, NST, EPI_GATE, 0, 0>(p, st);
  }
  set_error("gemm_x6: epilogue %d on a tile shape built without it", p.epi);
  return IXTTS_ERR_ARG;
}

}

using namespace ixtts;

extern "C" size_t ixtts_gemm_x6_packed_bytes(int N, int K) {
  if (N <= 0 || K <= 0 || K % 64) return 0;
  const size_t Npad = (size_t)(N + 255) / 256 * 256;
  return (size_t)(K / 16) * 6 * Npad * 16;
}

extern "C" int ixtts_gemm_x6_pack(const float* w_dev, void* packed_dev, int N, int K, void* stream) {
  IX_ARG(w_dev && packed_dev && N > 0 && K > 0 && K % 64 == 0, "gemm_x6_pack: bad argument (K must be a multiple of 64)");
  const int Npad = (N + 255) / 256 * 256;
  const long total = (long)(K / 8) * Npad;
  hipLaunchKernelGGL(gemm_x6_pack_kernel, dim3((unsigned)std::min<long>((total + 255) / 256, 4096)), dim3(256), 0, (hipStream_t)stream, w_dev,
                     reinterpret_cast<uint4*>(packed_dev), N, K, Npad);
  IX_HIP(hipGetLastError());
  return IXTTS_OK;
}

extern "C" long ixtts_gemm_x6_rows_padded(long rows) { return rows <= 0 ? 0 : (rows + 255) / 256 * 256 + 256; }

extern "C" int ixtts_gemm_x6_split(const float* a_dev, long lda, void* planes_dev, long rows, int K, void* stream) {
  IX_ARG(a_dev && planes_dev && rows > 0 && K > 0 && K % 64 == 0, "gemm_x6_split: bad argument (K must be a multiple of 64)");
  IX_ARG(lda >= K && lda % 4 == 0 && (reinterpret_cast<uintptr_t>(a_dev) & 15) == 0, "gemm_x6_split: rows must be 16-byte aligned (lda %ld)", lda);
  const long Mpad = ixtts_gemm_x6_rows_padded(rows);
  hipLaunchKernelGGL(gemm_x6_split_kernel, dim3((unsigned)(Mpad / 64), K / 64), dim3(256), 0, (hipStream_t)stream, a_dev, lda,
                     reinterpret_cast<uint4*>(planes_dev), (int)rows, K, Mpad);
  IX_HIP(hipGetLastError());
  return IXTTS_OK;
}

static int run_gemm_x6(GemmX6Params p, int tile, hipStream_t st) {
  if (tile == 0) {
    const long t42 = (long)ceil_div(p.M, 256) * ceil_div(p.N, 128);
    tile = t42 >= 140 ? 2 : 3;
  }
  switch (tile) {
    case 2: return launch_gemm_x6_epilogue<4, 2, 2, true>(p, st);
    case 3: return launch_gemm_x6_epilogue<2, 2, 3, true>(p, st);
    case 4: return launch_gemm_x6_epilogue<4, 2, 4, false>(p, st);
    case 5: return launch_gemm_x6_epilogue<2, 2, 4, false>(p, st);
  }
  if (tile >= 12 && (p.epi != EPI_PLAIN || p.accumulate)) {
    set_error("gemm_x6: the developer variants (tile %d) are built with the plain, overwriting epilogue only", tile);
    return IXTTS_ERR_ARG;
  }
  switch (tile) {
    case 12: return launch_gemm_x6<4, 2, 2, EPI_PLAIN, 0, 0, 1>(p, st);
    case 22: return launch_gemm_x6<4, 2, 2, EPI_PLAIN, 0, 0, 2>(p, st);
    case 32: return launch_gemm_x6<4, 2, 2, EPI_PLAIN, 0, 0, 3>(p, st);
    case 33: return launch_gemm_x6<2, 2, 3, EPI_PLAIN, 0, 0, 3>(p, st);
    case 42: return launch_gemm_x6<4, 2, 2, EPI_PLAIN, 0, 0, 0, 1>(p, st);
    case 43: return launch_gemm_x6<2, 2, 3, EPI_PLAIN, 0, 0, 0, 1>(p, st);
  }
  set_error("gemm_x6: tile %d (0 auto; 2 / 3: 256x128 / 128x128, two workgroups per CU; 4 / 5: the same, one per CU with a 4-stage ring)", tile);
  return IXTTS_ERR_ARG;
}

extern "C" int ixtts_gemm_x6_f32(const void* a_planes_dev, long rows_total, long row0, const void* packed_dev, const float* bias_dev, float* c_dev,
                                 long ldc, int M, int N, int K, int accumulate, int tile, void* stream) {
  IX_ARG(a_planes_dev && packed_dev && c_dev && M > 0 && N > 0 && K > 0 && K % 64 == 0, "gemm_x6: bad argument (K must be a multiple of 64: the split pass works on 64-wide k blocks)");
  IX_ARG(ldc >= N && row0 >= 0 && row0 + M <= rows_total, "gemm_x6: rows [%ld, %ld) of %ld, ldc %ld", row0, row0 + M, rows_total, ldc);
  GemmX6Params p;
  p.Ap = reinterpret_cast<const uint4*>(a_planes_dev); p.Mpad = ixtts_gemm_x6_rows_padded(rows_total); p.arow0 = row0;
  p.Wp = reinterpret_cast<const uint4*>(packed_dev); p.bias = bias_dev; p.C = c_dev; p.ldc = ldc;
  p.M = M; p.N = N; p.Npad = (N + 255) / 256 * 256; p.K = K; p.accumulate = accumulate ? 1 : 0; p.m_tiles = p.n_tiles = 0;
  p.tap_steps = K >> 4; p.epi = EPI_PLAIN; p.gate = nullptr; p.gate_ld = 0; p.rows_per_batch = 1; p.nbatch = 1; p.gate_seq_off = nullptr;
  p.dbg = (tile == 32 || tile == 33) ? reinterpret_cast<unsigned long long*>(const_cast<float*>(bias_dev)) : nullptr;
  if (p.dbg) p.bias = nullptr;
  return run_gemm_x6(p, tile, (hipStream_t)stream);
}

extern "C" int ixtts_gemm_x6_pair_f32(const void* a_planes_dev, long rows_total, long row0, int taps, const void* packed_dev, const float* bias_dev,
                                      const float* gate_dev, long gate_ld, long rows_per_batch, int nbatch, float* c_dev, long ldc, int M, int N, int K,
                                      int epilogue, int tile, void* stream) {
  IX_ARG(a_planes_dev && packed_dev && c_dev && M > 0 && N > 0 && taps > 0 && K > 0, "gemm_x6_pair: bad argument");
  IX_ARG(K % taps == 0 && (K / taps) % 64 == 0 && N % 64 == 0, "gemm_x6_pair: K %d = %d taps of a multiple of 64, N %d a multiple of 64", K, taps, N);
  IX_ARG(epilogue == EPI_SWIGLU || (epilogue == EPI_GATE && gate_dev && rows_per_batch > 0 && nbatch > 0 && gate_ld >= N / 2),
         "gemm_x6_pair: epilogue %d (1 swiglu; 2 gate, with gate biases)", epilogue);
  IX_ARG(ldc >= N / 2 && row0 >= 0 && row0 + M + taps - 1 <= rows_total, "gemm_x6_pair: rows [%ld, %ld) + %d taps of %ld, ldc %ld", row0, row0 + M, taps,
         rows_total, ldc);
  IX_ARG(tile == 0 || tile == 2 || tile == 3, "gemm_x6_pair: tile %d (0 auto, 2, 3)", tile);
  GemmX6Params p;
  p.Ap = reinterpret_cast<const uint4*>(a_planes_dev); p.Mpad = ixtts_gemm_x6_rows_padded(rows_total); p.arow0 = row0;
  p.Wp = reinterpret_cast<const uint4*>(packed_dev); p.bias = bias_dev; p.C = c_dev; p.ldc = ldc;
  p.M = M; p.N = N; p.Npad = (N + 255) / 256 * 256; p.K = K; p.accumulate = 0; p.m_tiles = p.n_tiles = 0;
  p.tap_steps = (K / taps) >> 4; p.epi = epilogue; p.gate = gate_dev; p.gate_ld = gate_ld; p.rows_per_batch = rows_per_batch; p.nbatch = nbatch;
  p.gate_seq_off = nullptr;
  p.dbg = nullptr;
  return run_gemm_x6(p, tile, (hipStream_t)stream);
}

extern "C" int ixtts_gemm_x6_pair_gate_varlen_f32(const void* a_planes_dev, long rows_total, long row0, int taps, const void* packed_dev, const float* bias_dev,
                                                  const float* gate_dev, long gate_ld, const int* seq_off_dev, int nseq, float* c_dev, long ldc, int M, int N,
                                                  int K, int tile, void* stream) {
  IX_ARG(seq_off_dev && nseq > 0, "gemm_x6_pair_gate_varlen: null offsets table or nseq %d", nseq);
  IX_ARG(a_planes_dev && packed_dev && c_dev && gate_dev && M > 0 && N > 0 && taps > 0 && K > 0 && gate_ld >= N / 2, "gemm_x6_pair_gate_varlen: bad argument");
  IX_ARG(K % taps == 0 && (K / taps) % 64 == 0 && N % 64 == 0, "gemm_x6_pair_gate_varlen: K %d = %d taps of a multiple of 64, N %d a multiple of 64", K, taps, N);
  IX_ARG(ldc >= N / 2 && row0 >= 0 && row0 + M + taps - 1 <= rows_total, "gemm_x6_pair_gate_varlen: rows [%ld, %ld) + %d taps of %ld, ldc %ld", row0, row0 + M,
         taps, rows_total, ldc);
  IX_ARG(tile == 0 || tile == 2 || tile == 3, "gemm_x6_pair_gate_varlen: tile %d (0 auto, 2, 3)", tile);
  GemmX6Params p;
  p.Ap = reinterpret_cast<const uint4*>(a_planes_dev); p.Mpad = ixtts_gemm_x6_rows_padded(rows_total); p.arow0 = row0;
  p.Wp = reinterpret_cast<const uint4*>(packed_dev); p.bias = bias_dev; p.C = c_dev; p.ldc = ldc;
  p.M = M; p.N = N; p.Npad = (N + 255) / 256 * 256; p.K = K; p.accumulate = 0; p.m_tiles = p.n_tiles = 0;
  p.tap_steps = (K / taps) >> 4; p.epi = EPI_GATE; p.gate = gate_dev; p.gate_ld = gate_ld; p.rows_per_batch = 1; p.nbatch = nseq;
  p.gate_seq_off = seq_off_dev;
  p.dbg = nullptr;
  return run_gemm_x6(p, tile, (hipStream_t)stream);
}
// ... 1 lines not shown
```

### voice-tts_amd/gemm.py

```python
import ctypes as C

import torch

from . import _lib


class PackedLinear:

    __slots__ = ("N", "K", "packed", "bias")

    def __init__(self, weight, bias=None):
        assert weight.is_cuda and weight.dim() == 2 and weight.shape[1] % 64 == 0, tuple(weight.shape)
        w = weight.detach().to(torch.float32).contiguous()
        self.N, self.K = int(w.shape[0]), int(w.shape[1])
        nbytes = _lib.lib().ixtts_gemm_x6_packed_bytes(self.N, self.K)
        self.packed = torch.empty(nbytes, dtype=torch.uint8, device=w.device)
        with torch.cuda.device(w.device):
            _lib.check(_lib.lib().ixtts_gemm_x6_pack(w.data_ptr(), self.packed.data_ptr(), self.N, self.K, _lib.current_stream_ptr()), "ixtts_gemm_x6_pack")
            torch.cuda.current_stream().synchronize()
        self.bias = None if bias is None else bias.detach().to(w.device, torch.float32).contiguous()


class Planes:

    __slots__ = ("buf", "rows", "K")

    def __init__(self, buf, rows, K):
        self.buf, self.rows, self.K = buf, rows, K


_POOL = {}


def usable(x, K):
    return x.is_cuda and x.dtype == torch.float32 and K % 64 == 0 and x.shape[-1] == K and x.stride(-1) == 1 and x.data_ptr() % 16 == 0 and \
        (x.dim() == 1 or (x.stride(-2) % 4 == 0 and x.stride(-2) >= K))


def split(x, slot=0):
    K = int(x.shape[-1])
    if x.dim() != 2:
        x = x.reshape(-1, K) if x.is_contiguous() else x.contiguous().reshape(-1, K)
    rows, lda = int(x.shape[0]), int(x.stride(0))
    L = _lib.lib()
    nbytes = (K // 16) * 6 * int(L.ixtts_gemm_x6_rows_padded(rows)) * 16
    key = (x.device, nbytes, slot)
    buf = _POOL.get(key)
    if buf is None:
        buf = _POOL[key] = torch.empty(nbytes, dtype=torch.uint8, device=x.device)
    with torch.cuda.device(x.device):
        _lib.check(L.ixtts_gemm_x6_split(x.data_ptr(), lda, buf.data_ptr(), rows, K, _lib.current_stream_ptr()), "ixtts_gemm_x6_split")
    return Planes(buf, rows, K)


def linear(x, pl, out=None, accumulate=False, bias=True, tile=0, row0=0, rows=None, lead=None):
    K, N = pl.K, pl.N
    if not isinstance(x, Planes):
        lead = tuple(x.shape[:-1]) if lead is None else lead
        x = split(x)
    assert x.K == K, (x.K, K)
    M = (x.rows - row0) if rows is None else int(rows)
    if out is None:
        assert not accumulate
        out = torch.empty(*(lead if lead is not None else (M,)), N, dtype=torch.float32, device=pl.packed.device)
    assert out.shape[-1] == N and out.stride(-1) == 1 and out.numel() >= M * N
    ldc = int(out.stride(-2)) if out.dim() >= 2 else N
    b = pl.bias if (bias and pl.bias is not None) else None
    with torch.cuda.device(pl.packed.device):
        rc = _lib.lib().ixtts_gemm_x6_f32(x.buf.data_ptr(), x.rows, int(row0), pl.packed.data_ptr(), b.data_ptr() if b is not None else None, out.data_ptr(), ldc,
                                          M, N, K, 1 if accumulate else 0, int(tile), _lib.current_stream_ptr())
    _lib.check(rc, "ixtts_gemm_x6_f32")
    return out


SWIGLU, GATE = 1, 2


def interleave_halves(a, b):
    F = a.shape[0]
    assert b.shape == a.shape and F % 32 == 0, (tuple(a.shape), tuple(b.shape))
    return torch.stack([a.reshape(F // 32, 32, *a.shape[1:]), b.reshape(F // 32, 32, *b.shape[1:])], 1).reshape(2 * F, *a.shape[1:]).contiguous()


def pair_linear(x, pl, epilogue, taps=1, out=None, gate=None, gate_off=0, rows_per_batch=1, row0=0, rows=None, tile=0, seq_off=None):
    if not isinstance(x, Planes):
        x = split(x)
    assert pl.K == taps * x.K and pl.N % 64 == 0, (pl.K, taps, x.K, pl.N)
    M = (x.rows - row0 - (taps - 1)) if rows is None else int(rows)
    if out is None:
        out = torch.empty(M, pl.N // 2, dtype=torch.float32, device=pl.packed.device)
    assert out.shape[-1] == pl.N // 2 and out.stride(-1) == 1 and out.numel() >= M * (pl.N // 2)
    ldc = int(out.stride(-2)) if out.dim() >= 2 else pl.N // 2
    gp, gld, nb = None, 0, 1
    if epilogue == GATE:
        assert gate.is_contiguous() and gate.dim() == 2 and gate_off + pl.N <= gate.shape[1]
        gp, gld, nb = gate.data_ptr() + 4 * int(gate_off), int(gate.shape[1]), int(gate.shape[0])
    b = pl.bias
    if seq_off is not None:
        assert epilogue == GATE and seq_off.tab.is_cuda and gate.shape[0] >= seq_off.n
        with torch.cuda.device(pl.packed.device):
            rc = _lib.lib().ixtts_gemm_x6_pair_gate_varlen_f32(x.buf.data_ptr(), x.rows, int(row0), int(taps), pl.packed.data_ptr(),
                                                               b.data_ptr() if b is not None else None, gp, gld, seq_off.tab.data_ptr(), int(seq_off.n),
                                                               out.data_ptr(), ldc, M, pl.N, pl.K, int(tile), _lib.current_stream_ptr())
        _lib.check(rc, "ixtts_gemm_x6_pair_gate_varlen_f32")
        return out
    with torch.cuda.device(pl.packed.device):
        rc = _lib.lib().ixtts_gemm_x6_pair_f32(x.buf.data_ptr(), x.rows, int(row0), int(taps), pl.packed.data_ptr(), b.data_ptr() if b is not None else None,
                                               gp, gld, int(rows_per_batch), nb, out.data_ptr(), ldc, M, pl.N, pl.K, int(epilogue), int(tile),
                                               _lib.current_stream_ptr())
    _lib.check(rc, "ixtts_gemm_x6_pair_f32")
    return out
```

### voice-tts_amd/s2mel.py

```python
import math
import os

import torch
import torch.nn.functional as F

from . import gemm as G
from .convs import conv1d

from .weights import fold_weight_norm

S2MEL_CFG = dict(
    hidden_dim=512, num_heads=8, depth=13, in_channels=80, content_dim=512, style_dim=192,
    wavenet_hidden=512, wavenet_layers=8, wavenet_kernel=5, wavenet_dilation_rate=1,
    lr_channels=512, lr_in_channels=1024, lr_n_blocks=4, gpt_dim=1280, codebook_dim=8, codebook_size=8192, semantic_dim=1024,
)


def tiny_s2mel_cfg(**kw):
    c = dict(S2MEL_CFG)
    c.update(hidden_dim=64, num_heads=2, depth=5, content_dim=32, style_dim=12, wavenet_hidden=64, wavenet_layers=3,
             lr_channels=32, lr_in_channels=40, lr_n_blocks=2, gpt_dim=128, codebook_size=8194, semantic_dim=40)
    c.update(kw)
    return c


def _ffn_dim(dim):
    n_hidden = int(2 * (4 * dim) / 3)
    return n_hidden if n_hidden % 256 == 0 else n_hidden + 256 - (n_hidden % 256)


def s2mel_shapes(cfg=S2MEL_CFG):
    H, Hw, C = cfg["hidden_dim"], cfg["wavenet_hidden"], cfg["in_channels"]
    assert H == Hw, "FinalLayer's adaLN takes the DiT timestep embedding: wavenet.hidden_dim must equal DiT.hidden_dim"
    out = [("gpt_layer.0.weight", (256, cfg["gpt_dim"])), ("gpt_layer.0.bias", (256,)), ("gpt_layer.1.weight", (128, 256)),
           ("gpt_layer.1.bias", (128,)), ("gpt_layer.2.weight", (cfg["semantic_dim"], 128)), ("gpt_layer.2.bias", (cfg["semantic_dim"],)),
           ("quantizer.codebook.weight", (cfg["codebook_size"], cfg["codebook_dim"])),
           ("quantizer.out_project.weight", (cfg["semantic_dim"], cfg["codebook_dim"], 1)), ("quantizer.out_project.bias", (cfg["semantic_dim"],))]
    lr = cfg["lr_channels"]
    out += [("length_regulator.content_in_proj.weight", (lr, cfg["lr_in_channels"])), ("length_regulator.content_in_proj.bias", (lr,))]
    for i in range(cfg["lr_n_blocks"]):
        out += [(f"length_regulator.model.{3 * i}.weight", (lr, lr, 3)), (f"length_regulator.model.{3 * i}.bias", (lr,)),
                (f"length_regulator.model.{3 * i + 1}.weight", (lr,)), (f"length_regulator.model.{3 * i + 1}.bias", (lr,))]
    n = 3 * cfg["lr_n_blocks"]
    out += [(f"length_regulator.model.{n}.weight", (lr, lr, 1)), (f"length_regulator.model.{n}.bias", (lr,))]
    e = "cfm.estimator."
    out += [(e + "t_embedder.mlp.0.weight", (H, 256)), (e + "t_embedder.mlp.0.bias", (H,)), (e + "t_embedder.mlp.2.weight", (H, H)), (e + "t_embedder.mlp.2.bias", (H,)),
            (e + "t_embedder2.mlp.0.weight", (Hw, 256)), (e + "t_embedder2.mlp.0.bias", (Hw,)), (e + "t_embedder2.mlp.2.weight", (Hw, Hw)), (e + "t_embedder2.mlp.2.bias", (Hw,)),
            (e + "cond_projection.weight", (H, cfg["content_dim"])), (e + "cond_projection.bias", (H,)),
            (e + "cond_x_merge_linear.weight", (H, H + 2 * C + cfg["style_dim"])), (e + "cond_x_merge_linear.bias", (H,)),
            (e + "skip_linear.weight", (H, H + C)), (e + "skip_linear.bias", (H,)),
            (e + "conv1.weight", (Hw, H)), (e + "conv1.bias", (Hw,)), (e + "conv2.weight", (C, Hw, 1)), (e + "conv2.bias", (C,)),
            (e + "res_projection.weight", (Hw, H)), (e + "res_projection.bias", (Hw,)),
            (e + "final_layer.linear.weight", (Hw, Hw)), (e + "final_layer.linear.bias", (Hw,)),
            (e + "final_layer.adaLN_modulation.1.weight", (2 * Hw, Hw)), (e + "final_layer.adaLN_modulation.1.bias", (2 * Hw,))]
    t = e + "transformer."
    inter = _ffn_dim(H)
    for i in range(cfg["depth"]):
        p = t + f"layers.{i}."
        out += [(p + "attention.wqkv.weight", (3 * H, H)), (p + "attention.wo.weight", (H, H)),
                (p + "feed_forward.w1.weight", (inter, H)), (p + "feed_forward.w3.weight", (inter, H)), (p + "feed_forward.w2.weight", (H, inter)),
                (p + "ffn_norm.project_layer.weight", (2 * H, H)), (p + "ffn_norm.project_layer.bias", (2 * H,)), (p + "ffn_norm.norm.weight", (H,)),
                (p + "attention_norm.project_layer.weight", (2 * H, H)), (p + "attention_norm.project_layer.bias", (2 * H,)), (p + "attention_norm.norm.weight", (H,)),
                (p + "skip_in_linear.weight", (H, 2 * H)), (p + "skip_in_linear.bias", (H,))]
    out += [(t + "norm.project_layer.weight", (2 * H, H)), (t + "norm.project_layer.bias", (2 * H,)), (t + "norm.norm.weight", (H,))]
    w = e + "wavenet."
    nl, k = cfg["wavenet_layers"], cfg["wavenet_kernel"]
    out += [(w + "cond_layer.conv.conv.weight", (2 * Hw * nl, Hw, 1)), (w + "cond_layer.conv.conv.bias", (2 * Hw * nl,))]
    for i in range(nl):
        rs = 2 * Hw if i < nl - 1 else Hw
        out += [(w + f"in_layers.{i}.conv.conv.weight", (2 * Hw, Hw, k)), (w + f"in_layers.{i}.conv.conv.bias", (2 * Hw,)),
                (w + f"res_skip_layers.{i}.conv.conv.weight", (rs, Hw, 1)), (w + f"res_skip_layers.{i}.conv.conv.bias", (rs,))]
    return out


def make_s2mel_weights(cfg=S2MEL_CFG, seed=1234):
    g = torch.Generator().manual_seed(seed)
    W = {}
    for name, shape in s2mel_shapes(cfg):
        if name.endswith("norm.weight") or (".model." in name and len(shape) == 1 and name.endswith(".weight")):
            W[name] = 1.0 + 0.1 * torch.randn(*shape, generator=g)
        elif name.endswith(".bias"):
            W[name] = 0.02 * torch.randn(*shape, generator=g)
        elif name == "quantizer.codebook.weight":
            W[name] = torch.randn(*shape, generator=g)
        else:
            fan = 1
            for d in shape[1:]:
                fan *= d
            W[name] = torch.randn(*shape, generator=g) / math.sqrt(fan)
    return W


def _pad_reflect(x, left, right):
    L = x.shape[-1]
    extra = 0
    if L <= max(left, right):
        extra = max(left, right) - L + 1
        x = F.pad(x, (0, extra))
    y = F.pad(x, (left, right), mode="reflect")
    return y[..., : y.shape[-1] - extra]


def attn_full(q, k, v, scale=None):
    import ctypes as C

    from . import _lib

    B, T, Hh, d = q.shape
    assert d == 64 and q.is_cuda and q.dtype == torch.float32 and k.shape == q.shape and v.shape == q.shape
    for t in (q, k, v):
        assert t.stride(3) == 1 and t.stride() == q.stride() and t.stride(1) % 4 == 0 and t.data_ptr() % 16 == 0
    out = torch.empty(B, T, Hh, d, device=q.device, dtype=torch.float32)
    sc = float(scale if scale is not None else 1.0 / math.sqrt(d))
    L = _lib.lib()
    nws = L.ixtts_attn_full_workspace_bytes(B, Hh, T)
    ws = torch.empty(nws, device=q.device, dtype=torch.uint8)
    with torch.cuda.device(q.device):
        rc = L.ixtts_attn_full_f32(q.data_ptr(), k.data_ptr(), v.data_ptr(), out.data_ptr(), B, Hh, T, d, q.stride(0), q.stride(1),
                                   q.stride(2), out.stride(0), out.stride(1), out.stride(2), C.c_float(sc), ws.data_ptr(), nws,
                                   _lib.current_stream_ptr())
    _lib.check(rc, "ixtts_attn_full_f32")
    return out


def _lin(x, W, name):
    return F.linear(x, W[name + ".weight"], W.get(name + ".bias"))


def _hip_call(name, *args):
    from . import _lib

    _lib.check(getattr(_lib.lib(), name)(*args, _lib.current_stream_ptr()), name)


def adaln_rmsnorm(x, wb, g, eps=1e-5):
    B, T, H = x.shape
    if x.is_cuda:
        import ctypes as C

        x, wb = x.contiguous(), wb.contiguous()
        out = torch.empty_like(x)
        with torch.cuda.device(x.device):
            _hip_call("ixtts_adaln_rmsnorm_f32", x.data_ptr(), wb.data_ptr(), g.data_ptr(), out.data_ptr(), B, T, H, C.c_float(eps))
        return out
    w, b = wb[:, None, :H], wb[:, None, H:]
    return torch.addcmul(b, w, F.rms_norm(x, (H,), g, eps))


def ln_modulate(x, ss, eps=1e-6):
    B, T, H = x.shape
    if x.is_cuda:
        import ctypes as C

        x, ss = x.contiguous(), ss.contiguous()
        out = torch.empty_like(x)
        with torch.cuda.device(x.device):
            _hip_call("ixtts_ln_modulate_f32", x.data_ptr(), ss.data_ptr(), out.data_ptr(), B, T, H, C.c_float(eps))
        return out
    return F.layer_norm(x, (H,), None, None, eps) * (1 + ss[:, None, H:]) + ss[:, None, :H]


def swiglu(u):
    Fd = u.shape[-1] // 2
    if u.is_cuda:
        u = u.contiguous()
        out = torch.empty(*u.shape[:-1], Fd, device=u.device, dtype=u.dtype)
        with torch.cuda.device(u.device):
            _hip_call("ixtts_swiglu_f32", u.data_ptr(), out.data_ptr(), u.numel() // (2 * Fd), Fd)
        return out
    return F.silu(u[..., :Fd]) * u[..., Fd:]


def wn_gate(a, g, off, C_):
    B, _, T = a.shape
    if a.is_cuda:
        a, g = a.contiguous(), g.contiguous()
        out = torch.empty(B, C_, T, device=a.device, dtype=a.dtype)
        with torch.cuda.device(a.device):
            _hip_call("ixtts_wn_gate_f32", a.data_ptr(), g.data_ptr(), out.data_ptr(), B, C_, T, g.shape[1], off)
        return out
    x = a + g[:, off:off + 2 * C_, None]
    return torch.tanh(x[:, :C_]) * torch.sigmoid(x[:, C_:])


def wn_gate_rows(a, g, off, C_, rows_per_batch):
    rows, B = a.shape[0], g.shape[0]
    if a.is_cuda:
        a, g = a.contiguous(), g.contiguous()
        out = torch.empty(rows, C_, device=a.device, dtype=a.dtype)
        with torch.cuda.device(a.device):
            _hip_call("ixtts_wn_gate_rows_f32", a.data_ptr(), g.data_ptr(), out.data_ptr(), rows, C_, rows_per_batch, B, g.shape[1], off)
        return out
    b = (torch.arange(rows, device=a.device) // rows_per_batch).clamp(max=B - 1)
    x = a + g[b, off:off + 2 * C_]
    return torch.tanh(x[:, :C_]) * torch.sigmoid(x[:, C_:])


def reflect_halo_rows(p, T, left, right):
    B, _, C_ = p.shape
    if p.is_cuda:
        assert p.is_contiguous()
        with torch.cuda.device(p.device):
            _hip_call("ixtts_reflect_halo_rows_f32", p.data_ptr(), B, T, C_, left, right)
        return p
    if left:
        p[:, :left] = p[:, left + 1:2 * left + 1].flip(1)
    if right:
        p[:, left + T:] = p[:, left + T - 1 - right:left + T - 1].flip(1)
    return p


class RowPack:

    def __init__(self, lens, device):
        self.lens = [int(t) for t in lens]
        assert self.lens and min(self.lens) >= 1, self.lens
        self.n = len(self.lens)
        self.off = [0]
        for t in self.lens:
            self.off.append(self.off[-1] + t)
        self.rows = self.off[-1]
        self.device = torch.device(device)
        tiles = [0]
        for t in self.lens:
            tiles.append(tiles[-1] + (t + 63) // 64)
        self.tiles = tiles[-1]
        work = [(s, q) for s, t in enumerate(self.lens) for q in range((t + 127) // 128)]
        self.n_work = len(work)
        host = torch.tensor(self.off + tiles + [v for w in work for v in w], dtype=torch.int32)
        self.tab = host.to(self.device)
        if self.device.type != "cuda":
            self.seq = torch.repeat_interleave(torch.arange(self.n), torch.tensor(self.lens))
            self.pos = torch.arange(self.rows) - torch.tensor(self.off[:-1])[self.seq]

    def span(self, s):
        return self.off[s], self.off[s + 1]


def adaln_rmsnorm_packed(x, wb, g, pk, eps=1e-5):
    rows, H = x.shape
    if x.is_cuda:
        import ctypes as C

        x, wb = x.contiguous(), wb.contiguous()
        out = torch.empty_like(x)
        with torch.cuda.device(x.device):
            _hip_call("ixtts_adaln_rmsnorm_varlen_f32", x.data_ptr(), wb.data_ptr(), g.data_ptr(), out.data_ptr(), pk.tab.data_ptr(), pk.n, rows, H, C.c_float(eps))
        return out
    wbr = wb[pk.seq]
    return torch.addcmul(wbr[:, H:], wbr[:, :H], F.rms_norm(x, (H,), g, eps))


def ln_modulate_packed(x, ss, pk, eps=1e-6):
    rows, H = x.shape
    if x.is_cuda:
        import ctypes as C

        x, ss = x.contiguous(), ss.contiguous()
        out = torch.empty_like(x)
        with torch.cuda.device(x.device):
            _hip_call("ixtts_ln_modulate_varlen_f32", x.data_ptr(), ss.data_ptr(), out.data_ptr(), pk.tab.data_ptr(), pk.n, rows, H, C.c_float(eps))
        return out
    ssr = ss[pk.seq]
    return F.layer_norm(x, (H,), None, None, eps) * (1 + ssr[:, H:]) + ssr[:, :H]


def rope_qk_packed(qkv, fc, pk, head_dim):
    rows, H3 = qkv.shape
    H = H3 // 3
    if qkv.is_cuda:
        assert qkv.is_contiguous() and fc.shape[0] >= max(pk.lens)
        with torch.cuda.device(qkv.device):
            _hip_call("ixtts_rope_qk_varlen_f32", qkv.data_ptr(), torch.view_as_real(fc).data_ptr(), pk.tab.data_ptr(), pk.n, rows, H, head_dim)
        return qkv
    f = fc[pk.pos][:, None, :]
    out = qkv.clone()
    for j in range(2):
        xc = torch.view_as_complex(qkv[:, j * H:(j + 1) * H].reshape(rows, H // head_dim, head_dim // 2, 2).contiguous())
        out[:, j * H:(j + 1) * H] = torch.view_as_real(xc * f).reshape(rows, H)
    return out


def attn_full_packed(q, k, v, pk, scale=None):
    import ctypes as C

    from . import _lib

    rows, Hh, d = q.shape
    assert d == 64 and q.is_cuda and q.dtype == torch.float32 and k.shape == q.shape and v.shape == q.shape and rows == pk.rows
    for t in (q, k, v):
        assert t.stride(2) == 1 and t.stride() == q.stride() and t.stride(0) % 4 == 0 and t.data_ptr() % 16 == 0
    out = torch.empty(rows, Hh, d, device=q.device, dtype=torch.float32)
    sc = float(scale if scale is not None else 1.0 / math.sqrt(d))
    L = _lib.lib()
    nws = L.ixtts_attn_full_varlen_workspace_bytes(pk.n, Hh, pk.tiles)
    ws = torch.empty(nws, device=q.device, dtype=torch.uint8)
    with torch.cuda.device(q.device):
        rc = L.ixtts_attn_full_varlen_f32(q.data_ptr(), k.data_ptr(), v.data_ptr(), out.data_ptr(), pk.tab.data_ptr(), pk.n, pk.tiles, pk.n_work, Hh, d,
                                          q.stride(0), q.stride(1), out.stride(0), out.stride(1), C.c_float(sc), ws.data_ptr(), nws, _lib.current_stream_ptr())
    _lib.check(rc, "ixtts_attn_full_varlen_f32")
    return out


def wn_gate_rows_packed(a, g, off, C_, poff):
    rows = a.shape[0]
    if a.is_cuda:
        a, g = a.contiguous(), g.contiguous()
        out = torch.empty(rows, C_, device=a.device, dtype=a.dtype)
        with torch.cuda.device(a.device):
            _hip_call("ixtts_wn_gate_rows_varlen_f32", a.data_ptr(), g.data_ptr(), out.data_ptr(), rows, C_, poff.tab.data_ptr(), poff.n, g.shape[1], off)
        return out
    b = torch.cat([poff.seq, poff.seq.new_full((max(0, rows - poff.rows),), poff.n - 1)])[:rows]
    x = a + g[b, off:off + 2 * C_]
    return torch.tanh(x[:, :C_]) * torch.sigmoid(x[:, C_:])


def _reflect_src(T, left, right):
    idx = _pad_reflect(torch.arange(1, T + 1, dtype=torch.float64)[None, None], left, right)[0, 0].long() - 1
    dst = list(range(left)) + list(range(left + T, left + T + right))
    return dst, [int(idx[i]) + left if int(idx[i]) >= 0 else -1 for i in dst]


def reflect_halo_rows_packed(p, poff, left, right):
    if p.is_cuda:
        assert p.is_contiguous() and min(poff.lens) - left - right > max(left, right)
        with torch.cuda.device(p.device):
            _hip_call("ixtts_reflect_halo_rows_varlen_f32", p.data_ptr(), poff.tab.data_ptr(), poff.n, p.shape[1], left, right)
        return p
    if not hasattr(poff, "halo"):
        dst, src, zero = [], [], []
        for s, L in enumerate(poff.lens):
            o = poff.off[s]
            for d_, s_ in zip(*_reflect_src(L - left - right, left, right)):
                (dst.append(o + d_), src.append(o + s_)) if s_ >= 0 else zero.append(o + d_)
        poff.halo = (torch.tensor(dst, dtype=torch.long), torch.tensor(src, dtype=torch.long), torch.tensor(zero, dtype=torch.long))
    dst, src, zero = poff.halo
    p[dst] = p[src]
    if zero.numel():
        p[zero] = 0
    return p


S2MEL_BATCH_FRAMES = 16384

TUNED_GEMMS = os.path.join(os.path.dirname(os.path.abspath(__file__)), "tunable", "gfx950_s2mel.csv")


def use_tuned_gemms(path=TUNED_GEMMS):
    if not torch.cuda.is_available():
        return False
    import torch.cuda.tunable as tn

    tn.enable(True)
    tn.tuning_enable(os.environ.get("IXTTS_TUNE") == "1")
    try:
        import tempfile

        tn.set_filename(os.path.join(tempfile.gettempdir(), "ixtts_tunableop_online.csv"))
    except Exception:
        pass
    try:
        return bool(os.path.isfile(path) and tn.read_file(path))
    except Exception:
        return False


_TUNED_T0, _TUNED_TH0 = 2322, 1909
_tuned_lengths = set()


def extend_tuned_gemms(T, Th, path=TUNED_GEMMS):
    if (T, Th) in _tuned_lengths or (T, Th) == (_TUNED_T0, _TUNED_TH0):
        return False
    _tuned_lengths.add((T, Th))
    import tempfile

    import torch.cuda.tunable as tn

    sub = {str(2 * _TUNED_T0): str(2 * T), str(_TUNED_T0): str(T), str(_TUNED_TH0): str(Th), str(2 * _TUNED_TH0): str(2 * Th),
           str(2 * _TUNED_TH0 + 4): str(2 * Th + 4)}
    head, rows = [], []
    for line in open(path).read().splitlines():
        f = line.split(",")
        if f[0] == "Validator":
            head.append(line)
        elif len(f) >= 4 and f[2] != "Default" and f[0].endswith("_TN"):
            toks = f[1].split("_")
            if any(t in sub for t in toks):
                rows.append(",".join([f[0], "_".join(sub.get(t, t) for t in toks)] + f[2:]))
    if not rows:
        return False
    with tempfile.NamedTemporaryFile("w", suffix=".csv", delete=False) as fh:
        fh.write("\n".join(head + rows) + "\n")
    try:
        return bool(tn.read_file(fh.name))
    except Exception:
        return False
    finally:
        os.unlink(fh.name)


class S2Mel:
    def __init__(self, W, cfg=S2MEL_CFG, device="cpu", dtype=torch.float32):
        self.cfg = dict(cfg)
        self.device = torch.device(device)
        self.dtype = dtype
        if dtype not in (torch.float32, torch.float64) or (self.device.type == "cuda" and dtype != torch.float32):
            raise ValueError(f"S2Mel: dtype {dtype} on {self.device} (fp32 anywhere; fp64 on the CPU leg only: the HIP kernels are fp32)")
        self.tuned_gemms = False
        if self.device.type == "cuda" and os.environ.get("IXTTS_NO_TUNED_GEMMS") != "1":
            self.tuned_gemms = use_tuned_gemms()
        W = fold_weight_norm(dict(W))
        self.W = {k: v.to(self.device, torch.float32).to(dtype) for k, v in W.items()}
        H = cfg["hidden_dim"]
        self.head_dim = H // cfg["num_heads"]
        half = 128
        self.t_freqs = torch.exp(-math.log(10000.0) * torch.arange(half, dtype=torch.float32) / half).to(self.device).to(dtype)
        self._rope = None
        W, C_, L = self.W, cfg["in_channels"], cfg["depth"]
        t = "cfm.estimator.transformer."
        self.w13 = [torch.cat([W[t + f"layers.{i}.feed_forward.w1.weight"], W[t + f"layers.{i}.feed_forward.w3.weight"]], 0).contiguous() for i in range(L)]
        self.skip_w = {i: (W[t + f"layers.{i}.skip_in_linear.weight"][:, :H].contiguous(), W[t + f"layers.{i}.skip_in_linear.weight"][:, H:].contiguous())
                       for i in range(L // 2 + 1, L)}
        names = [t + f"layers.{i}.{n}" for i in range(L) for n in ("attention_norm", "ffn_norm")] + [t + "norm"]
        self.proj_w = torch.cat([W[n + ".project_layer.weight"] for n in names], 0).contiguous()
        self.proj_b = torch.cat([W[n + ".project_layer.bias"] for n in names], 0).contiguous()
        mw = W["cfm.estimator.cond_x_merge_linear.weight"]
        self.merge_x, self.merge_rest = mw[:, :C_].contiguous(), mw[:, C_:].contiguous()
        wn = "cfm.estimator.wavenet."
        self.wn_taps = [[W[wn + f"in_layers.{i}.conv.conv.weight"][:, :, j].contiguous() for j in range(cfg["wavenet_kernel"])]
                        for i in range(cfg["wavenet_layers"])]
        nl, Hw = cfg["wavenet_layers"], cfg["wavenet_hidden"]
        self.wn_r1, self.wn_r2, self.wn_bin = [], [], []
        carry = torch.zeros(Hw, device=self.device, dtype=dtype)
        self.wn_out_bias = torch.zeros(Hw, device=self.device, dtype=dtype)
        for i in range(nl):
            rw, rb = W[wn + f"res_skip_layers.{i}.conv.conv.weight"][:, :, 0], W[wn + f"res_skip_layers.{i}.conv.conv.bias"]
            self.wn_bin.append(W[wn + f"in_layers.{i}.conv.conv.bias"] + sum(self.wn_taps[i]) @ carry)
            if i < nl - 1:
                self.wn_r1.append(rw[:Hw].contiguous())
                self.wn_r2.append(rw[Hw:].contiguous())
                carry = carry + rb[:Hw]
                self.wn_out_bias = self.wn_out_bias + rb[Hw:]
            else:
                self.wn_r1.append(None)
                self.wn_r2.append(rw.contiguous())
                self.wn_out_bias = self.wn_out_bias + rb
        sw = W["cfm.estimator.skip_linear.weight"]
        self.skipl_res, self.skipl_x = sw[:, :H].contiguous(), sw[:, H:].contiguous()
        self.x6_w13, self.x6_wn = None, None
        if self.device.type == "cuda" and H % 64 == 0:
            inter = self.w13[0].shape[0] // 2
            self.x6_w13 = [G.PackedLinear(G.interleave_halves(w[:inter], w[inter:])) for w in self.w13]
            self.x6_wn = [G.PackedLinear(G.interleave_halves(torch.cat(tp, 1)[:Hw], torch.cat(tp, 1)[Hw:]), G.interleave_halves(b[:Hw], b[Hw:]))
                          for tp, b in zip(self.wn_taps, self.wn_bin)]

    def _x6(self, packs):
        return packs is not None and os.environ.get("IXTTS_S2MEL_GEMM", "x6") != "library"

    def gpt_layer(self, latent):
        x = _lin(latent, self.W, "gpt_layer.0")
        x = _lin(x, self.W, "gpt_layer.1")
        return _lin(x, self.W, "gpt_layer.2")

    def vq2emb(self, codes):
        emb = self.W["quantizer.codebook.weight"][codes.long()]
        out = conv1d(emb.transpose(1, 2), self.W["quantizer.out_project.weight"], self.W["quantizer.out_project.bias"])
        return out.transpose(1, 2)

    def length_regulator(self, x, ylens):
        W = self.W
        x = _lin(x, W, "length_regulator.content_in_proj")
        T = int(ylens.max())
        x = x.transpose(1, 2).contiguous()
        if x.dtype == torch.float32:
            x = F.interpolate(x, size=T, mode="nearest")
        else:
            src = F.interpolate(torch.arange(x.shape[-1], dtype=torch.float32)[None, None], size=T, mode="nearest")[0, 0].long()
            x = x[..., src.to(x.device)]
        for i in range(self.cfg["lr_n_blocks"]):
            x = conv1d(x, W[f"length_regulator.model.{3 * i}.weight"], W[f"length_regulator.model.{3 * i}.bias"], padding=1)
            x = F.group_norm(x, 1, W[f"length_regulator.model.{3 * i + 1}.weight"], W[f"length_regulator.model.{3 * i + 1}.bias"], 1e-5)
            x = F.mish(x)
        n = 3 * self.cfg["lr_n_blocks"]
        x = conv1d(x, W[f"length_regulator.model.{n}.weight"], W[f"length_regulator.model.{n}.bias"])
        mask = (torch.arange(T, device=x.device).unsqueeze(0) < ylens.unsqueeze(1)).unsqueeze(-1)
        return x.transpose(1, 2) * mask

    def _t_embed(self, t, prefix):
        args = 1000.0 * t[:, None].float() * self.t_freqs[None].float()
        emb = torch.cat([torch.cos(args), torch.sin(args)], dim=-1).to(self.dtype)
        h = F.silu(_lin(emb, self.W, prefix + ".mlp.0"))
        return _lin(h, self.W, prefix + ".mlp.2")

    def _rope_cache(self, T):
        if self._rope is None or self._rope.shape[0] < T:
            n = self.head_dim
            freqs = 1.0 / (10000.0 ** (torch.arange(0, n, 2)[: n // 2].float() / n))
            ang = torch.outer(torch.arange(max(T, 64)).float(), freqs)
            self._rope = torch.polar(torch.ones_like(ang), ang).to(self.device)
            if self.dtype == torch.float64:
                self._rope = self._rope.to(torch.complex128)
        return self._rope[:T]

    @staticmethod
    def _rotary(x, fc):
        xc = torch.view_as_complex(x.reshape(*x.shape[:-1], -1, 2))
        return torch.view_as_real(xc * fc.view(1, fc.shape[0], 1, fc.shape[1])).flatten(3)

    def _attention(self, qkv, B, T, mask):
        H, nh, hd = self.cfg["hidden_dim"], self.cfg["num_heads"], self.head_dim
        fc = self._rope_cache(T)
        if mask is None and hd == 64 and qkv.is_cuda:
            with torch.cuda.device(qkv.device):
                _hip_call("ixtts_rope_qk_f32", qkv.data_ptr(), torch.view_as_real(fc).data_ptr(), B, T, H, hd)
            v4 = qkv.view(B, T, 3, nh, hd)
            return attn_full(v4[:, :, 0], v4[:, :, 1], v4[:, :, 2]).reshape(B * T, H)
        q, k, v = qkv.view(B, T, 3 * H).split([H, H, H], dim=-1)
        q = self._rotary(q.reshape(B, T, nh, hd), fc)
        k = self._rotary(k.reshape(B, T, nh, hd), fc)
        v = v.reshape(B, T, nh, hd)
        y = F.scaled_dot_product_attention(q.transpose(1, 2), k.transpose(1, 2), v.transpose(1, 2), attn_mask=mask, dropout_p=0.0)
        return y.transpose(1, 2).reshape(B * T, H)

    def _transformer(self, x, c, mask):
        W, cfg = self.W, self.cfg
        B, T, H = x.shape
        L = cfg["depth"]
        wb_all = F.linear(c, self.proj_w, self.proj_b).view(B, 2 * L + 1, 2 * H).transpose(0, 1).contiguous()
        x = x.reshape(B * T, H)
        x6 = x.is_cuda and self._x6(self.x6_w13)
        skips = []
        for i in range(L):
            p = f"cfm.estimator.transformer.layers.{i}."
            if i > L // 2:
                wa, wb_ = self.skip_w[i]
                x = F.linear(skips.pop(), wb_, W[p + "skip_in_linear.bias"]).addmm_(x, wa.t())
            a = adaln_rmsnorm(x.view(B, T, H), wb_all[2 * i], W[p + "attention_norm.norm.weight"])
            y = self._attention(F.linear(a.view(B * T, H), W[p + "attention.wqkv.weight"]), B, T, mask)
            h = torch.addmm(x, y, W[p + "attention.wo.weight"].t()) if 0 < i <= L // 2 else x.addmm_(y, W[p + "attention.wo.weight"].t())
            f = adaln_rmsnorm(h.view(B, T, H), wb_all[2 * i + 1], W[p + "ffn_norm.norm.weight"]).view(B * T, H)
            u = G.pair_linear(f, self.x6_w13[i], G.SWIGLU) if x6 else swiglu(F.linear(f, self.w13[i]))
            x = h.addmm_(u, W[p + "feed_forward.w2.weight"].t())
            if i < L // 2:
                skips.append(x)
        return adaln_rmsnorm(x.view(B, T, H), wb_all[2 * L], W["cfm.estimator.transformer.norm.norm.weight"])

    def _wavenet(self, x, x_mask, g, full):
        W, cfg = self.W, self.cfg
        Hw, nl, k = cfg["wavenet_hidden"], cfg["wavenet_layers"], cfg["wavenet_kernel"]
        p = "cfm.estimator.wavenet."
        g = F.linear(g, W[p + "cond_layer.conv.conv.weight"][:, :, 0], W[p + "cond_layer.conv.conv.bias"])
        out = None
        for i in range(nl):
            d = cfg["wavenet_dilation_rate"] ** i
            tot = (k - 1) * d
            right = tot // 2
            xin = _pad_reflect(x, tot - right, right)
            if x.is_cuda:
                wk, T_ = self.wn_taps[i], x.shape[-1]
                acc = W[p + f"in_layers.{i}.conv.conv.bias"][None, :, None].expand(x.shape[0], -1, T_)
                for j in range(k):
                    wj, xj = wk[j].expand(x.shape[0], -1, -1), xin[:, :, j * d:j * d + T_]
                    acc = torch.baddbmm(acc, wj, xj) if j == 0 else acc.baddbmm_(wj, xj)
                xin = acc
            else:
                xin = conv1d(xin, W[p + f"in_layers.{i}.conv.conv.weight"], W[p + f"in_layers.{i}.conv.conv.bias"], dilation=d)
            acts = wn_gate(xin, g, i * 2 * Hw, Hw)
            rs = conv1d(acts, W[p + f"res_skip_layers.{i}.conv.conv.weight"], W[p + f"res_skip_layers.{i}.conv.conv.bias"])
            if i < nl - 1:
                x = x + rs[:, :Hw]
                if not full:
                    x = x * x_mask
                out = rs[:, Hw:] if out is None else out + rs[:, Hw:]
            else:
                out = rs if out is None else out + rs
        return out if full else out * x_mask

    def _wavenet_gemm(self, x, g):
        W, cfg = self.W, self.cfg
        Hw, nl, k = cfg["wavenet_hidden"], cfg["wavenet_layers"], cfg["wavenet_kernel"]
        B, _, T_ = x.shape
        p = "cfm.estimator.wavenet."
        g = F.linear(g, W[p + "cond_layer.conv.conv.weight"][:, :, 0], W[p + "cond_layer.conv.conv.bias"])
        x = x.contiguous()
        out = None
        for i in range(nl):
            d = cfg["wavenet_dilation_rate"] ** i
            tot = (k - 1) * d
            right = tot // 2
            xin = _pad_reflect(x, tot - right, right)
            acc = self.wn_bin[i][None, :, None].expand(B, -1, T_)
            for j in range(k):
                wj, xj = self.wn_taps[i][j].expand(B, -1, -1), xin[:, :, j * d:j * d + T_]
                acc = torch.baddbmm(acc, wj, xj) if j == 0 else acc.baddbmm_(wj, xj)
            acts = wn_gate(acc, g, i * 2 * Hw, Hw)
            if i < nl - 1:
                x = x.baddbmm_(self.wn_r1[i].expand(B, -1, -1), acts)
            r2 = self.wn_r2[i].expand(B, -1, -1)
            out = torch.bmm(r2, acts) if out is None else out.baddbmm_(r2, acts)
        return out

    def _wavenet_rows(self, h, g):
        W, cfg = self.W, self.cfg
        Hw, nl, k = cfg["wavenet_hidden"], cfg["wavenet_layers"], cfg["wavenet_kernel"]
        assert cfg["wavenet_dilation_rate"] == 1
        B, T_, _ = h.shape
        p = "cfm.estimator.wavenet."
        g = F.linear(g, W[p + "cond_layer.conv.conv.weight"][:, :, 0], W[p + "cond_layer.conv.conv.bias"])
        tot = k - 1
        right = tot // 2
        left = tot - right
        Tp = T_ + tot
        P = torch.empty(B, Tp, Hw, device=h.device, dtype=h.dtype)
        P[:, left:left + T_] = h
        P2 = P.view(B * Tp, Hw)
        M = B * Tp - tot
        centre = P2[left:left + M]
        out = torch.empty(B * Tp, Hw, device=h.device, dtype=h.dtype)
        x6 = self._x6(self.x6_wn)
        for i in range(nl):
            reflect_halo_rows(P, T_, left, right)
            if x6:
                acts = G.pair_linear(G.split(P2), self.x6_wn[i], G.GATE, taps=k, gate=g, gate_off=i * 2 * Hw, rows_per_batch=Tp)
            else:
                acc = torch.addmm(self.wn_bin[i], P2[:M], self.wn_taps[i][0].t())
                for j in range(1, k):
                    acc.addmm_(P2[j:j + M], self.wn_taps[i][j].t())
                acts = wn_gate_rows(acc, g, i * 2 * Hw, Hw, Tp)
            if i < nl - 1:
                centre.addmm_(acts, self.wn_r1[i].t())
            if i == 0:
                torch.mm(acts, self.wn_r2[i].t(), out=out[:M])
            else:
                out[:M].addmm_(acts, self.wn_r2[i].t())
        return out.view(B, Tp, Hw)[:, :T_]

    def dit_prepare(self, prompt_x, x_lens, style, cond):
        W = self.W
        e = "cfm.estimator."
        B, _, T = prompt_x.shape
        cond = _lin(cond, W, e + "cond_projection")
        rest = torch.cat([prompt_x.transpose(1, 2), cond, style[:, None, :].expand(B, T, style.shape[-1])], dim=-1)
        base = F.linear(rest, self.merge_rest, W[e + "cond_x_merge_linear.bias"])
        x_mask = (torch.arange(T, device=prompt_x.device).unsqueeze(0) < x_lens.unsqueeze(1)).unsqueeze(1)
        full = int(x_lens.min()) >= T
        if full:
            attn_mask = None
        else:
            attn_mask = x_mask[:, None, :].expand(x_mask.shape[0], 1, T, T)
            if attn_mask.shape[0] != B:
                attn_mask = attn_mask.expand(B, 1, T, T)
        return dict(B=B, T=T, base=base, x_mask=x_mask.to(base.dtype), attn_mask=attn_mask, full=full)

    def dit_step(self, ctx, x, t, out_from=0):
        W, cfg = self.W, self.cfg
        e = "cfm.estimator."
        B, T, base = ctx["B"], ctx["T"], ctx["base"]
        xt = x.transpose(1, 2)
        t1 = self._t_embed(t, e + "t_embedder")
        x_in = base + F.linear(xt, self.merge_x)
        x_res = self._transformer(x_in, t1, ctx["attn_mask"])
        halo = sum((cfg["wavenet_kernel"] - 1) * cfg["wavenet_dilation_rate"] ** i for i in range(cfg["wavenet_layers"])) // 2 + 1
        lo = max(0, out_from - halo) if (ctx["full"] and out_from > 0) else 0
        if lo > 0:
            x_res, xt = x_res[:, lo:], xt[:, lo:]
        Th = T - lo
        if self.tuned_gemms and os.environ.get("IXTTS_TUNED_ANY_LENGTH", "1") == "1":
            extend_tuned_gemms(T, Th)
        x_res = F.linear(x_res, self.skipl_res, W[e + "skip_linear.bias"]) + F.linear(xt, self.skipl_x)
        h = _lin(x_res, W, e + "conv1")
        t2 = self._t_embed(t, e + "t_embedder2")
        gemm_form = h.is_cuda and ctx["full"] and Th > 2 * cfg["wavenet_kernel"] * cfg["wavenet_dilation_rate"] ** (cfg["wavenet_layers"] - 1)
        if gemm_form and cfg["wavenet_dilation_rate"] == 1:
            h = self._wavenet_rows(h, t2) + F.linear(x_res, W[e + "res_projection.weight"], W[e + "res_projection.bias"] + self.wn_out_bias)
        elif gemm_form:
            h = self._wavenet_gemm(h.transpose(1, 2), t2).transpose(1, 2) + F.linear(x_res, W[e + "res_projection.weight"],
                                                                                     W[e + "res_projection.bias"] + self.wn_out_bias)
        else:
            mask = ctx["x_mask"][:, :, lo:] if lo > 0 else ctx["x_mask"]
            h = self._wavenet(h.transpose(1, 2), mask, t2, ctx["full"]).transpose(1, 2) + _lin(x_res, W, e + "res_projection")
        ss = _lin(F.silu(t1), W, e + "final_layer.adaLN_modulation.1")
        h = ln_modulate(h, ss)
        h = _lin(h, W, e + "final_layer.linear").transpose(1, 2)
        out = conv1d(h, W[e + "conv2.weight"], W[e + "conv2.bias"])
        return out[:, :, out_from - lo:] if out_from > 0 else out

    def dit(self, x, prompt_x, x_lens, t, style, cond):
        return self.dit_step(self.dit_prepare(prompt_x, x_lens, style, cond), x, t)

    @torch.no_grad()
    def cfm_inference(self, mu, x_lens, prompt, style, n_timesteps=25, inference_cfg_rate=0.7, noise=None, temperature=1.0):
        B, T = mu.shape[0], mu.shape[1]
        assert B == 1, "CFM inference is batch-1 (as the reference)"
        z = (torch.randn(B, self.cfg["in_channels"], T, device=mu.device) if noise is None else noise.to(mu.device, torch.float32)).to(self.dtype) * temperature
        t_span = torch.linspace(0, 1, n_timesteps + 1, device=mu.device)
        x = z.clone()
        Tp = prompt.shape[-1]
        prompt_x = torch.zeros_like(x)
        prompt_x[..., :Tp] = prompt[..., :Tp]
        x[..., :Tp] = 0
        if inference_cfg_rate > 0:
            ctx = self.dit_prepare(torch.cat([prompt_x, torch.zeros_like(prompt_x)], 0), x_lens, torch.cat([style, torch.zeros_like(style)], 0),
                                   torch.cat([mu, torch.zeros_like(mu)], 0))
        else:
            ctx = self.dit_prepare(prompt_x, x_lens, style, mu)
        t = t_span[0]
        skip = Tp if ctx["full"] else 0
        for step in range(1, len(t_span)):
            dt = t_span[step] - t_span[step - 1]
            if inference_cfg_rate > 0:
                d = self.dit_step(ctx, x, torch.stack([t, t]), out_from=skip)
                dphi = (1.0 + inference_cfg_rate) * d[0:1] - inference_cfg_rate * d[1:2]
            else:
                dphi = self.dit_step(ctx, x, t.expand(B), out_from=skip)
            if skip > 0:
                x[:, :, skip:] += dt * dphi
            else:
                x = x + dt * dphi
            t = t + dt
            x[:, :, :Tp] = 0
        return x

    @torch.no_grad()
    def __call__(self, latent, codes, code_lens, prompt_condition, ref_mel, style, n_timesteps=25, inference_cfg_rate=0.7, noise=None):
        lat = self.gpt_layer(latent)
        S = self.vq2emb(codes) + lat
        target = (code_lens * 1.72).long()
        cond = self.length_regulator(S, target)
        cat = torch.cat([prompt_condition, cond], dim=1)
        lens = torch.tensor([cat.shape[1]], device=cat.device, dtype=torch.long)
        mel = self.cfm_inference(cat, lens, ref_mel, style, n_timesteps, inference_cfg_rate, noise)
        return mel[:, :, ref_mel.shape[-1]:]

    def _attention_packed(self, qkv, pk):
        H, nh, hd = self.cfg["hidden_dim"], self.cfg["num_heads"], self.head_dim
        if qkv.is_cuda and hd == 64 and os.environ.get("IXTTS_ATTN_FULL", "x3") != "f32":
            rope_qk_packed(qkv, self._rope_cache(max(pk.lens)), pk, hd)
            v4 = qkv.view(pk.rows, 3, nh, hd)
            return attn_full_packed(v4[:, 0], v4[:, 1], v4[:, 2], pk).view(pk.rows, H)
        out = torch.empty(pk.rows, H, device=qkv.device, dtype=qkv.dtype)
        if qkv.is_cuda:
            for s in range(pk.n):
                a, b = pk.span(s)
                out[a:b] = self._attention(qkv[a:b], 1, b - a, None)
            return out
        qk = rope_qk_packed(qkv, self._rope_cache(max(pk.lens)), pk, hd)
        for s in range(pk.n):
            a, b = pk.span(s)
            q, k, v = (qk[a:b, :H], qk[a:b, H:2 * H], qkv[a:b, 2 * H:])
            y = F.scaled_dot_product_attention(*(z.reshape(1, b - a, nh, hd).transpose(1, 2) for z in (q, k, v)), dropout_p=0.0)
            out[a:b] = y.transpose(1, 2).reshape(b - a, H)
        return out

    def _transformer_packed(self, x, c, pk):
        W, cfg = self.W, self.cfg
        H, L = cfg["hidden_dim"], cfg["depth"]
        wb_all = F.linear(c, self.proj_w, self.proj_b).view(pk.n, 2 * L + 1, 2 * H).transpose(0, 1).contiguous()
        x6 = x.is_cuda and self._x6(self.x6_w13)
        skips = []
        for i in range(L):
            p = f"cfm.estimator.transformer.layers.{i}."
            if i > L // 2:
                wa, wb_ = self.skip_w[i]
                x = F.linear(skips.pop(), wb_, W[p + "skip_in_linear.bias"]).addmm_(x, wa.t())
            a = adaln_rmsnorm_packed(x, wb_all[2 * i], W[p + "attention_norm.norm.weight"], pk)
            y = self._attention_packed(F.linear(a, W[p + "attention.wqkv.weight"]), pk)
            h = torch.addmm(x, y, W[p + "attention.wo.weight"].t()) if 0 < i <= L // 2 else x.addmm_(y, W[p + "attention.wo.weight"].t())
            f = adaln_rmsnorm_packed(h, wb_all[2 * i + 1], W[p + "ffn_norm.norm.weight"], pk)
            u = G.pair_linear(f, self.x6_w13[i], G.SWIGLU) if x6 else swiglu(F.linear(f, self.w13[i]))
            x = h.addmm_(u, W[p + "feed_forward.w2.weight"].t())
            if i < L // 2:
                skips.append(x)
        return adaln_rmsnorm_packed(x, wb_all[2 * L], W["cfm.estimator.transformer.norm.norm.weight"], pk)

    def _wavenet_packed(self, h, g, hp):
        W, cfg = self.W, self.cfg
        Hw, nl, k = cfg["wavenet_hidden"], cfg["wavenet_layers"], cfg["wavenet_kernel"]
        assert cfg["wavenet_dilation_rate"] == 1
        p = "cfm.estimator.wavenet."
        g = F.linear(g, W[p + "cond_layer.conv.conv.weight"][:, :, 0], W[p + "cond_layer.conv.conv.bias"])
        tot = k - 1
        right = tot // 2
        left = tot - right
        pp, interior = hp.padded, hp.interior
        P2 = torch.empty(pp.rows, Hw, device=h.device, dtype=h.dtype)
        P2[interior] = h
        M = pp.rows - tot
        centre = P2[left:left + M]
        out = torch.empty(pp.rows, Hw, device=h.device, dtype=h.dtype)
        x6 = h.is_cuda and self._x6(self.x6_wn)
        for i in range(nl):
            reflect_halo_rows_packed(P2, pp, left, right)
            if x6:
                acts = G.pair_linear(G.split(P2), self.x6_wn[i], G.GATE, taps=k, gate=g, gate_off=i * 2 * Hw, seq_off=pp)
            else:
                acc = torch.addmm(self.wn_bin[i], P2[:M], self.wn_taps[i][0].t())
                for j in range(1, k):
                    acc.addmm_(P2[j:j + M], self.wn_taps[i][j].t())
                acts = wn_gate_rows_packed(acc, g, i * 2 * Hw, Hw, pp)
            if i < nl - 1:
                centre.addmm_(acts, self.wn_r1[i].t())
            if i == 0:
                torch.mm(acts, self.wn_r2[i].t(), out=out[:M])
            else:
                out[:M].addmm_(acts, self.wn_r2[i].t())
        return out[interior - left]

    def _halo(self):
        cfg = self.cfg
        return sum((cfg["wavenet_kernel"] - 1) * cfg["wavenet_dilation_rate"] ** i for i in range(cfg["wavenet_layers"])) // 2 + 1

    def packable(self, T, Tp, device=None):
        dev = self.device if device is None else torch.device(device)
        if dev.type != "cuda":
            return True
        cfg = self.cfg
        Th = T - max(0, Tp - self._halo())
        return cfg["wavenet_dilation_rate"] == 1 and Th > 2 * cfg["wavenet_kernel"]

    def _cfm_packed(self, segs, n_timesteps, inference_cfg_rate):
        W, cfg = self.W, self.cfg
        e = "cfm.estimator."
        dev = segs[0]["mu"].device
        C_, H = cfg["in_channels"], cfg["hidden_dim"]
        n = len(segs)
        lens = [s["mu"].shape[1] for s in segs]
        Tps = [min(s["prompt"].shape[-1], T) for s, T in zip(segs, lens)]
        R = sum(lens)
        cfg_on = inference_cfg_rate > 0
        nb = 2 if cfg_on else 1
        pk = RowPack(lens * nb, dev)
        xo = pk.off[:n + 1]
        x = torch.cat([s["z"][0].t() for s in segs], 0).contiguous()
        keep = torch.cat([torch.arange(xo[i] + Tps[i], xo[i + 1]) for i in range(n)]).to(dev)
        pmask = torch.ones(R, 1, device=dev, dtype=self.dtype)
        for i in range(n):
            pmask[xo[i]:xo[i] + Tps[i]] = 0
        x.mul_(pmask)
        prompt_rows = torch.zeros(R, C_, device=dev, dtype=self.dtype)
        for i, s in enumerate(segs):
            prompt_rows[xo[i]:xo[i] + Tps[i]] = s["prompt"][0, :, :Tps[i]].t()
        mu = torch.cat([s["mu"][0] for s in segs], 0)
        style = torch.cat([s["style"].expand(T, -1) for s, T in zip(segs, lens)], 0)
        rest = torch.cat([prompt_rows, _lin(mu, W, e + "cond_projection"), style], -1)
        if cfg_on:
            rest = torch.cat([rest, torch.cat([torch.zeros_like(prompt_rows), _lin(torch.zeros_like(mu), W, e + "cond_projection"), torch.zeros_like(style)], -1)], 0)
        base = F.linear(rest, self.merge_rest, W[e + "cond_x_merge_linear.bias"])
        halo, k = self._halo(), cfg["wavenet_kernel"]
        los = [max(0, Tp - halo) for Tp in Tps] * nb
        head_lens = [L - lo for L, lo in zip(pk.lens, los)]
        hp = RowPack(head_lens, dev)
        hp.padded = RowPack([t + k - 1 for t in head_lens], dev)
        right = (k - 1) // 2
        left = k - 1 - right
        hidx = torch.cat([torch.arange(pk.off[s] + los[s], pk.off[s + 1]) for s in range(pk.n)])
        hp.interior = torch.cat([torch.arange(hp.padded.off[s] + left, hp.padded.off[s] + left + head_lens[s]) for s in range(pk.n)]).to(dev)
        hrows = hidx.to(dev)
        hx = (hidx - torch.tensor(pk.off[:-1]).repeat_interleave(torch.tensor(head_lens)) +
              torch.tensor(xo[:-1] * nb).repeat_interleave(torch.tensor(head_lens))).to(dev)
        hsel = torch.cat([torch.arange(hp.off[s] + Tps[s % n] - los[s], hp.off[s + 1]) for s in range(pk.n)]).to(dev)
        nkeep = keep.numel()
        t_span = torch.linspace(0, 1, n_timesteps + 1, device=dev)
        t = t_span[0]
        for step in range(1, len(t_span)):
            dt = t_span[step] - t_span[step - 1]
            tt = t.expand(pk.n)
            t1 = self._t_embed(tt, e + "t_embedder")
            x_in = (base.view(nb, R, H) + F.linear(x, self.merge_x)).view(nb * R, H)
            x_res = self._transformer_packed(x_in, t1, pk)
            x_res = x_res.index_select(0, hrows)
            xt = x.index_select(0, hx)
            x_res = F.linear(x_res, self.skipl_res, W[e + "skip_linear.bias"]) + F.linear(xt, self.skipl_x)
            h = _lin(x_res, W, e + "conv1")
            t2 = self._t_embed(tt, e + "t_embedder2")
            h = self._wavenet_packed(h, t2, hp) + F.linear(x_res, W[e + "res_projection.weight"], W[e + "res_projection.bias"] + self.wn_out_bias)
            ss = _lin(F.silu(t1), W, e + "final_layer.adaLN_modulation.1")
            h = ln_modulate_packed(h, ss, hp)
            h = _lin(h, W, e + "final_layer.linear")
# ... 46 lines not shown
```

Baseline: 41.32.

## Fuse RoPE into attention, norm into plane split, halo into split; cache timestep constants

Adds attention entry points that rotate Q and K with RoPE inside the K/V plane builder and the Q load, so the separate rope pass goes away. Adds an AdaLN-RMSNorm variant that writes the split bf16 planes directly for the SwiGLU pair GEMM, and a split kernel that fills the reflect halo while splitting, removing the standalone halo kernel in the wavenet. Timestep-dependent embeddings and conditioning projections are also cached per (n_timesteps, step, batch) key. The goal is fewer kernel launches and fewer full-tensor passes through memory, at the cost of more template variants and cached state that could go stale if the weights change.

After: 41.92, median of 6. 1.5% higher.

```diff
diff --git a/include/ixtts_hip.h b/include/ixtts_hip.h
--- a/include/ixtts_hip.h
+++ b/include/ixtts_hip.h
@@ -30,6 +30,13 @@
 int ixtts_attn_full_varlen_f32(const float* q_dev, const float* k_dev, const float* v_dev, float* out_dev, const int* table_dev, int nseq,
                                int total_tiles, int n_work, int H, int head_dim, long stride_t, long stride_h, long ostride_t, long ostride_h,
                                float scale, void* workspace_dev, size_t workspace_bytes, void* stream);
+
+int ixtts_attn_full_rope_f32(const float* q_dev, const float* k_dev, const float* v_dev, float* out_dev, const float* cos_sin_dev, int rope_rows,
+                             int B, int H, int T, int head_dim, long stride_b, long stride_t, long stride_h, long ostride_b, long ostride_t,
+                             long ostride_h, float scale, void* workspace_dev, size_t workspace_bytes, void* stream);
+int ixtts_attn_full_rope_varlen_f32(const float* q_dev, const float* k_dev, const float* v_dev, float* out_dev, const float* cos_sin_dev,
+                                    const int* table_dev, int nseq, int total_tiles, int n_work, int H, int head_dim, long stride_t, long stride_h,
+                                    long ostride_t, long ostride_h, float scale, void* workspace_dev, size_t workspace_bytes, void* stream);
 
 int ixtts_adaln_rmsnorm_f32(const float* x_dev, const float* wb_dev, const float* g_dev, float* out_dev, int B, int T, int H, float eps,
                             void* stream);
@@ -50,12 +57,20 @@
                                   long g_stride, int g_offset, void* stream);
 int ixtts_reflect_halo_rows_varlen_f32(float* p_dev, const int* seq_off_dev, int nseq, int C, int left, int right, void* stream);
 
+int ixtts_adaln_rmsnorm_planes_f32(const float* x_dev, const float* wb_dev, const float* g_dev, void* planes_dev, int B, int T, int H, float eps,
+                                   void* stream);
+int ixtts_adaln_rmsnorm_planes_varlen_f32(const float* x_dev, const float* wb_dev, const float* g_dev, void* planes_dev, const int* seq_off_dev,
+                                          int nseq, long rows, int H, float eps, void* stream);
+
 size_t ixtts_gemm_x6_packed_bytes(int N, int K);
 int ixtts_gemm_x6_pack(const float* w_dev, void* packed_dev, int N, int K, void* stream);
 long ixtts_gemm_x6_rows_padded(long rows);
 int ixtts_gemm_x6_split(const float* a_dev, long lda, void* planes_dev, long rows, int K, void* stream);
 int ixtts_gemm_x6_f32(const void* a_planes_dev, long rows_total, long row0, const void* packed_dev, const float* bias_dev, float* c_dev, long ldc,
                       int M, int N, int K, int accumulate, int tile, void* stream);
+int ixtts_gemm_x6_split_halo(const float* a_dev, long lda, void* planes_dev, long rows, int K, int T, int left, int right, void* stream);
+int ixtts_gemm_x6_split_halo_varlen(const float* a_dev, long lda, void* planes_dev, long rows, int K, const int* seq_off_dev, int nseq, int left,
+                                    int right, void* stream);
 int ixtts_gemm_x6_pair_f32(const void* a_planes_dev, long rows_total, long row0, int taps, const void* packed_dev, const float* bias_dev,
                            const float* gate_dev, long gate_ld, long rows_per_batch, int nbatch, float* c_dev, long ldc, int M, int N, int K,
                            int epilogue, int tile, void* stream);
diff --git a/voice-tts_amd/_lib.py b/voice-tts_amd/_lib.py
--- a/voice-tts_amd/_lib.py
+++ b/voice-tts_amd/_lib.py
@@ -70,6 +70,10 @@
     "ixtts_attn_full_varlen_workspace_bytes": (C.c_size_t, [C.c_int, C.c_int, C.c_int]),
     "ixtts_attn_full_varlen_f32": (C.c_int, [_P, _P, _P, _P, _P, C.c_int, C.c_int, C.c_int, C.c_int, C.c_int, C.c_long, C.c_long, C.c_long, C.c_long,
                                              C.c_float, _P, C.c_size_t, _P]),
+    "ixtts_attn_full_rope_f32": (C.c_int, [_P, _P, _P, _P, _P, C.c_int, C.c_int, C.c_int, C.c_int, C.c_int, C.c_long, C.c_long, C.c_long, C.c_long,
+                                           C.c_long, C.c_long, C.c_float, _P, C.c_size_t, _P]),
+    "ixtts_attn_full_rope_varlen_f32": (C.c_int, [_P, _P, _P, _P, _P, _P, C.c_int, C.c_int, C.c_int, C.c_int, C.c_int, C.c_long, C.c_long, C.c_long,
+                                                  C.c_long, C.c_float, _P, C.c_size_t, _P]),
     "ixtts_adaln_rmsnorm_f32": (C.c_int, [_P, _P, _P, _P, C.c_int, C.c_int, C.c_int, C.c_float, _P]),
     "ixtts_ln_modulate_f32": (C.c_int, [_P, _P, _P, C.c_int, C.c_int, C.c_int, C.c_float, _P]),
     "ixtts_rope_qk_f32": (C.c_int, [_P, _P, C.c_int, C.c_int, C.c_int, C.c_int, _P]),
@@ -82,6 +86,10 @@
     "ixtts_rope_qk_varlen_f32": (C.c_int, [_P, _P, _P, C.c_int, C.c_long, C.c_int, C.c_int, _P]),
     "ixtts_wn_gate_rows_varlen_f32": (C.c_int, [_P, _P, _P, C.c_long, C.c_int, _P, C.c_int, C.c_long, C.c_int, _P]),
     "ixtts_reflect_halo_rows_varlen_f32": (C.c_int, [_P, _P, C.c_int, C.c_int, C.c_int, C.c_int, _P]),
+    "ixtts_adaln_rmsnorm_planes_f32": (C.c_int, [_P, _P, _P, _P, C.c_int, C.c_int, C.c_int, C.c_float, _P]),
+    "ixtts_adaln_rmsnorm_planes_varlen_f32": (C.c_int, [_P, _P, _P, _P, _P, C.c_int, C.c_long, C.c_int, C.c_float, _P]),
+    "ixtts_gemm_x6_split_halo": (C.c_int, [_P, C.c_long, _P, C.c_long, C.c_int, C.c_int, C.c_int, C.c_int, _P]),
+    "ixtts_gemm_x6_split_halo_varlen": (C.c_int, [_P, C.c_long, _P, C.c_long, C.c_int, _P, C.c_int, C.c_int, C.c_int, _P]),
     "ixtts_gemm_x6_packed_bytes": (C.c_size_t, [C.c_int, C.c_int]),
     "ixtts_gemm_x6_pack": (C.c_int, [_P, _P, C.c_int, C.c_int, _P]),
     "ixtts_gemm_x6_rows_padded": (C.c_long, [C.c_long]),
diff --git a/voice-tts_amd/csrc/attn_full.h b/voice-tts_amd/csrc/attn_full.h
--- a/voice-tts_amd/csrc/attn_full.h
+++ b/voice-tts_amd/csrc/attn_full.h
@@ -23,6 +23,7 @@
   float* ws_ml;
   const int* vl_tab;
   int vl_n, vl_tiles;
+  const float2* rope;
 };
 
 size_t attn_full_x3_plane_bytes(int B, int H, int T);
diff --git a/voice-tts_amd/csrc/attn_full.hip b/voice-tts_amd/csrc/attn_full.hip
--- a/voice-tts_amd/csrc/attn_full.hip
+++ b/voice-tts_amd/csrc/attn_full.hip
@@ -184,9 +184,9 @@
   return attn_partials_bytes(B, H, T) + ixtts::attn_full_x3_plane_bytes(B, H, T);
 }
 
-extern "C" int ixtts_attn_full_f32(const float* q_dev, const float* k_dev, const float* v_dev, float* out_dev, int B, int H, int T,
-                                   int head_dim, long stride_b, long stride_t, long stride_h, long ostride_b, long ostride_t,
-                                   long ostride_h, float scale, void* workspace_dev, size_t workspace_bytes, void* stream) {
+static int attn_full_run(const float* q_dev, const float* k_dev, const float* v_dev, float* out_dev, const float* rope_dev, int B, int H, int T, int head_dim,
+                         long stride_b, long stride_t, long stride_h, long ostride_b, long ostride_t, long ostride_h, float scale, void* workspace_dev,
+                         size_t workspace_bytes, void* stream) {
   using namespace ixtts;
   IX_ARG(q_dev && k_dev && v_dev && out_dev, "attn_full: null pointer");
   IX_ARG(head_dim == AF_D, "attn_full: head_dim %d (only 64 is built)", head_dim);
@@ -199,6 +199,7 @@
   a.B = B; a.H = H; a.T = T; a.scale = scale;
   a.ws_o = a.ws_ml = nullptr;
   a.vl_tab = nullptr; a.vl_n = a.vl_tiles = 0;
+  a.rope = reinterpret_cast<const float2*>(rope_dev);
   hipStream_t st = (hipStream_t)stream;
   const int qblocks = ceil_div(T, AF_WAVES * AF_QW);
   const bool have_ws = workspace_dev && workspace_bytes >= ixtts_attn_full_workspace_bytes(B, H, T);
@@ -206,6 +207,7 @@
   const char* mode = getenv("IXTTS_ATTN_FULL");
   const bool x3 = !(mode && strcmp(mode, "f32") == 0);
   const bool use_x3 = x3 && have_ws;
+  IX_ARG(!rope_dev || use_x3, "attn_full_rope: only the split-product build rotates (it needs the workspace, and IXTTS_ATTN_FULL unset or x3)");
   if (split) {
     a.ws_o = reinterpret_cast<float*>(workspace_dev);
     a.ws_ml = a.ws_o + (size_t)(use_x3 ? AX_KSPLIT : AF_KSPLIT) * B * H * T * AF_D;
@@ -230,14 +232,30 @@
   return IXTTS_OK;
 }
 
+extern "C" int ixtts_attn_full_f32(const float* q_dev, const float* k_dev, const float* v_dev, float* out_dev, int B, int H, int T,
+                                   int head_dim, long stride_b, long stride_t, long stride_h, long ostride_b, long ostride_t,
+                                   long ostride_h, float scale, void* workspace_dev, size_t workspace_bytes, void* stream) {
+  return attn_full_run(q_dev, k_dev, v_dev, out_dev, nullptr, B, H, T, head_dim, stride_b, stride_t, stride_h, ostride_b, ostride_t, ostride_h, scale,
+                       workspace_dev, workspace_bytes, stream);
+}
+
+extern "C" int ixtts_attn_full_rope_f32(const float* q_dev, const float* k_dev, const float* v_dev, float* out_dev, const float* cos_sin_dev, int rope_rows,
+                                        int B, int H, int T, int head_dim, long stride_b, long stride_t, long stride_h, long ostride_b, long ostride_t,
+                                        long ostride_h, float scale, void* workspace_dev, size_t workspace_bytes, void* stream) {
+  IX_ARG(cos_sin_dev && rope_rows >= T && (reinterpret_cast<uintptr_t>(cos_sin_dev) & 15) == 0,
+         "attn_full_rope: the (cos, sin) table must be 16-byte aligned and cover T=%d positions (it has %d)", T, rope_rows);
+  return attn_full_run(q_dev, k_dev, v_dev, out_dev, cos_sin_dev, B, H, T, head_dim, stride_b, stride_t, stride_h, ostride_b, ostride_t, ostride_h, scale,
+                       workspace_dev, workspace_bytes, stream);
+}
+
 extern "C" size_t ixtts_attn_full_varlen_workspace_bytes(int nseq, int H, int total_tiles) {
   if (nseq <= 0 || H <= 0 || total_tiles <= 0) return 0;
   return (size_t)H * total_tiles * 2 * 3 * 8 * 64 * 16;
 }
 
-extern "C" int ixtts_attn_full_varlen_f32(const float* q_dev, const float* k_dev, const float* v_dev, float* out_dev, const int* table_dev, int nseq,
-                                          int total_tiles, int n_work, int H, int head_dim, long stride_t, long stride_h, long ostride_t, long ostride_h,
-                                          float scale, void* workspace_dev, size_t workspace_bytes, void* stream) {
+static int attn_full_varlen_run(const float* q_dev, const float* k_dev, const float* v_dev, float* out_dev, const float* rope_dev, const int* table_dev,
+                                int nseq, int total_tiles, int n_work, int H, int head_dim, long stride_t, long stride_h, long ostride_t, long ostride_h,
+                                float scale, void* workspace_dev, size_t workspace_bytes, void* stream) {
   using namespace ixtts;
   IX_ARG(q_dev && k_dev && v_dev && out_dev && table_dev, "attn_full_varlen: null pointer");
   IX_ARG(head_dim == AF_D, "attn_full_varlen: head_dim %d (only 64 is built)", head_dim);
@@ -253,5 +271,21 @@
   a.B = 1; a.H = H; a.T = 0; a.scale = scale;
   a.ws_o = a.ws_ml = nullptr;
   a.vl_tab = table_dev; a.vl_n = nseq; a.vl_tiles = total_tiles;
+  a.rope = reinterpret_cast<const float2*>(rope_dev);
   return launch_attn_full_x3_varlen(a, workspace_dev, n_work, (hipStream_t)stream);
 }
+
+extern "C" int ixtts_attn_full_varlen_f32(const float* q_dev, const float* k_dev, const float* v_dev, float* out_dev, const int* table_dev, int nseq,
+                                          int total_tiles, int n_work, int H, int head_dim, long stride_t, long stride_h, long ostride_t, long ostride_h,
+                                          float scale, void* workspace_dev, size_t workspace_bytes, void* stream) {
+  return attn_full_varlen_run(q_dev, k_dev, v_dev, out_dev, nullptr, table_dev, nseq, total_tiles, n_work, H, head_dim, stride_t, stride_h, ostride_t, ostride_h,
+                              scale, workspace_dev, workspace_bytes, stream);
+}
+
+extern "C" int ixtts_attn_full_rope_varlen_f32(const float* q_dev, const float* k_dev, const float* v_dev, float* out_dev, const float* cos_sin_dev,
+                                               const int* table_dev, int nseq, int total_tiles, int n_work, int H, int head_dim, long stride_t, long stride_h,
+                                               long ostride_t, long ostride_h, float scale, void* workspace_dev, size_t workspace_bytes, void* stream) {
+  IX_ARG(cos_sin_dev && (reinterpret_cast<uintptr_t>(cos_sin_dev) & 15) == 0, "attn_full_rope_varlen: the (cos, sin) table must be 16-byte aligned");
+  return attn_full_varlen_run(q_dev, k_dev, v_dev, out_dev, cos_sin_dev, table_dev, nseq, total_tiles, n_work, H, head_dim, stride_t, stride_h, ostride_t,
+                              ostride_h, scale, workspace_dev, workspace_bytes, stream);
+}
diff --git a/voice-tts_amd/csrc/attn_full_x3.hip b/voice-tts_amd/csrc/attn_full_x3.hip
--- a/voice-tts_amd/csrc/attn_full_x3.hip
+++ b/voice-tts_amd/csrc/attn_full_x3.hip
@@ -14,7 +14,7 @@
 }
 
 
-template <bool VL>
+template <bool VL, bool ROPE = false>
 __global__ __launch_bounds__(256) void attn_kv_planes_kernel(AttnFullArgs a, uint4* __restrict__ planes) {
   int tile = blockIdx.x, T = a.T;
   const float *kb, *vb;
@@ -43,7 +43,15 @@
     const int t = t0 + key;
     float v[8];
     const float4* src = reinterpret_cast<const float4*>(kb + (long)min(t, T - 1) * a.st + 8 * oct);
-    const float4 x0 = src[0], x1 = src[1];
+    float4 x0 = src[0], x1 = src[1];
+    if constexpr (ROPE) {
+      const float4* f = reinterpret_cast<const float4*>(a.rope + (long)min(t, T - 1) * (AF_D / 2) + 4 * oct);
+      const float4 f01 = f[0], f23 = f[1];
+      const float2 r0 = rope_rotate(x0.x, x0.y, make_float2(f01.x, f01.y)), r1 = rope_rotate(x0.z, x0.w, make_float2(f01.z, f01.w));
+      const float2 r2 = rope_rotate(x1.x, x1.y, make_float2(f23.x, f23.y)), r3 = rope_rotate(x1.z, x1.w, make_float2(f23.z, f23.w));
+      x0 = make_float4(r0.x, r0.y, r1.x, r1.y);
+      x1 = make_float4(r2.x, r2.y, r3.x, r3.y);
+    }
     const bool live = t < T;
     v[0] = live ? x0.x : 0.f; v[1] = live ? x0.y : 0.f; v[2] = live ? x0.z : 0.f; v[3] = live ? x0.w : 0.f;
     v[4] = live ? x1.x : 0.f; v[5] = live ? x1.y : 0.f; v[6] = live ? x1.z : 0.f; v[7] = live ? x1.w : 0.f;
@@ -72,7 +80,7 @@
   }
 }
 
-template <int KSPLIT, bool VL = false>
+template <int KSPLIT, bool VL = false, bool ROPE = false>
 __global__ __launch_bounds__(AX_WAVES * 64, 3) void attn_full_x3_kernel(AttnFullArgs a, const uint4* __restrict__ planes) {
   __shared__ uint4 Ks[AX_TILE_UNITS];
   __shared__ uint4 Vs[AX_TILE_UNITS];
@@ -108,7 +116,15 @@
     const float qs = a.scale * 1.4426950408889634f;
 #pragma unroll
     for (int s = 0; s < 4; ++s) {
-      const float4 x0 = *reinterpret_cast<const float4*>(qrow + 16 * s), x1 = *reinterpret_cast<const float4*>(qrow + 16 * s + 4);
+      float4 x0 = *reinterpret_cast<const float4*>(qrow + 16 * s), x1 = *reinterpret_cast<const float4*>(qrow + 16 * s + 4);
+      if constexpr (ROPE) {
+        const float4* f = reinterpret_cast<const float4*>(a.rope + (long)qi * (AF_D / 2) + 8 * s + 4 * lh);
+        const float4 f01 = f[0], f23 = f[1];
+        const float2 r0 = rope_rotate(x0.x, x0.y, make_float2(f01.x, f01.y)), r1 = rope_rotate(x0.z, x0.w, make_float2(f01.z, f01.w));
+        const float2 r2 = rope_rotate(x1.x, x1.y, make_float2(f23.x, f23.y)), r3 = rope_rotate(x1.z, x1.w, make_float2(f23.z, f23.w));
+        x0 = make_float4(r0.x, r0.y, r1.x, r1.y);
+        x1 = make_float4(r2.x, r2.y, r3.x, r3.y);
+      }
       const float v[8] = {x0.x * qs, x0.y * qs, x0.z * qs, x0.w * qs, x1.x * qs, x1.y * qs, x1.z * qs, x1.w * qs};
       split8_bf16x3(v, qp[s][0], qp[s][1], qp[s][2]);
     }
@@ -250,6 +266,13 @@
   const int n_tiles = ceil_div(a.T, AF_KT);
   const int qblocks = ceil_div(a.T, AX_WAVES * AF_QW);
   uint4* pl = reinterpret_cast<uint4*>(planes);
+  if (a.rope) {
+    hipLaunchKernelGGL((attn_kv_planes_kernel<false, true>), dim3(n_tiles, a.B * a.H), dim3(256), 0, st, a, pl);
+    if (split) hipLaunchKernelGGL((attn_full_x3_kernel<AX_KSPLIT, false, true>), dim3(qblocks, a.B * a.H, AX_KSPLIT), dim3(AX_WAVES * 64), 0, st, a, (const uint4*)pl);
+    else hipLaunchKernelGGL((attn_full_x3_kernel<1, false, true>), dim3(qblocks, a.B * a.H), dim3(AX_WAVES * 64), 0, st, a, (const uint4*)pl);
+    IX_HIP(hipGetLastError());
+    return IXTTS_OK;
+  }
   hipLaunchKernelGGL(attn_kv_planes_kernel<false>, dim3(n_tiles, a.B * a.H), dim3(256), 0, st, a, pl);
   if (split) hipLaunchKernelGGL(attn_full_x3_kernel<AX_KSPLIT>, dim3(qblocks, a.B * a.H, AX_KSPLIT), dim3(AX_WAVES * 64), 0, st, a, (const uint4*)pl);
   else hipLaunchKernelGGL(attn_full_x3_kernel<1>, dim3(qblocks, a.B * a.H), dim3(AX_WAVES * 64), 0, st, a, (const uint4*)pl);
@@ -259,6 +282,12 @@
 
 int launch_attn_full_x3_varlen(const AttnFullArgs& a, void* planes, int n_work, hipStream_t st) {
   uint4* pl = reinterpret_cast<uint4*>(planes);
+  if (a.rope) {
+    hipLaunchKernelGGL((attn_kv_planes_kernel<true, true>), dim3(a.vl_tiles, a.H), dim3(256), 0, st, a, pl);
+    hipLaunchKernelGGL((attn_full_x3_kernel<1, true, true>), dim3(n_work, a.H), dim3(AX_WAVES * 64), 0, st, a, (const uint4*)pl);
+    IX_HIP(hipGetLastError());
+    return IXTTS_OK;
+  }
   hipLaunchKernelGGL(attn_kv_planes_kernel<true>, dim3(a.vl_tiles, a.H), dim3(256), 0, st, a, pl);
   hipLaunchKernelGGL((attn_full_x3_kernel<1, true>), dim3(n_work, a.H), dim3(AX_WAVES * 64), 0, st, a, (const uint4*)pl);
   IX_HIP(hipGetLastError());
diff --git a/voice-tts_amd/csrc/common.h b/voice-tts_amd/csrc/common.h
--- a/voice-tts_amd/csrc/common.h
+++ b/voice-tts_amd/csrc/common.h
@@ -52,6 +52,10 @@
     else hi = mid - 1;
   }
   return lo;
+}
+
+__device__ __forceinline__ float2 rope_rotate(float x, float y, float2 f) {
+  return make_float2(__fmaf_rn(x, f.x, -__fmul_rn(y, f.y)), __fmaf_rn(y, f.x, __fmul_rn(x, f.y)));
 }
 
 __device__ __forceinline__ float lo_bf16(unsigned int w) { return __uint_as_float(w << 16); }
diff --git a/voice-tts_amd/csrc/dit_ops.hip b/voice-tts_amd/csrc/dit_ops.hip
--- a/voice-tts_amd/csrc/dit_ops.hip
+++ b/voice-tts_amd/csrc/dit_ops.hip
@@ -4,12 +4,37 @@
 
 constexpr int ROW_NV = 8;
 
-template <bool CENTER>
-__global__ __launch_bounds__(256) void row_norm_mod_kernel(const float* __restrict__ x, const float* __restrict__ mw, const float* __restrict__ mb,
-                                                           const float* __restrict__ g, float* __restrict__ out, long rows, int T, int H, long mstride,
-                                                           float eps, float wadd, const int* __restrict__ seq_off = nullptr, int nseq = 0) {
-  const long row = (long)blockIdx.x * 4 + (threadIdx.x >> 6);
-  if (row >= rows) return;
+constexpr int NORM_PLANES_ROWS = 8;
+__device__ __forceinline__ void norm_planes_store(const float* tile, uint4* __restrict__ planes, long row0, int H, long Mpad) {
+  __syncthreads();
+  const int S = H + 4;
+  for (int idx = threadIdx.x; idx < H; idx += 64 * NORM_PLANES_ROWS) {
+    const int r = idx & 7, o = idx >> 3;
+    const float4 a = *reinterpret_cast<const float4*>(tile + r * S + 8 * o), b = *reinterpret_cast<const float4*>(tile + r * S + 8 * o + 4);
+    const float v[8] = {a.x, a.y, a.z, a.w, b.x, b.y, b.z, b.w};
+    uint4 ph, pm, pl;
+    split8_bf16x3(v, ph, pm, pl);
+    const int gk = o >> 1, kh = o & 1;
+    uint4* base = planes + ((long)gk * 6) * Mpad + row0 + r;
+    base[(long)(0 * 2 + kh) * Mpad] = ph;
+    base[(long)(1 * 2 + kh) * Mpad] = pm;
+    base[(long)(2 * 2 + kh) * Mpad] = pl;
+  }
+}
+
+template <bool CENTER, bool PLANES = false>
+__global__ __launch_bounds__(PLANES ? 64 * NORM_PLANES_ROWS : 256) void row_norm_mod_kernel(
+    const float* __restrict__ x, const float* __restrict__ mw, const float* __restrict__ mb, const float* __restrict__ g, float* __restrict__ out, long rows, int T,
+    int H, long mstride, float eps, float wadd, const int* __restrict__ seq_off = nullptr, int nseq = 0, long Mpad = 0) {
+  extern __shared__ float4 norm_tile[];
+  const long row = (long)blockIdx.x * (PLANES ? NORM_PLANES_ROWS : 4) + (threadIdx.x >> 6);
+  if (row >= rows) {
+    if constexpr (PLANES) {
+      for (int c = threadIdx.x & 63; c < (H >> 2); c += 64) norm_tile[(threadIdx.x >> 6) * ((H >> 2) + 1) + c] = make_float4(0.f, 0.f, 0.f, 0.f);
+      norm_planes_store(reinterpret_cast<const float*>(norm_tile), reinterpret_cast<uint4*>(out), (long)blockIdx.x * NORM_PLANES_ROWS, H, Mpad);
+    }
+    return;
+  }
   const int lane = threadIdx.x & 63;
   const int H4 = H >> 2;
   const float4* xr = reinterpret_cast<const float4*>(x + row * H);
@@ -72,9 +97,13 @@
         const float4 gg = g4[c];
         n.x *= gg.x; n.y *= gg.y; n.z *= gg.z; n.w *= gg.w;
       }
-      o4[c] = make_float4(fmaf(w.x + wadd, n.x, b.x), fmaf(w.y + wadd, n.y, b.y), fmaf(w.z + wadd, n.z, b.z), fmaf(w.w + wadd, n.w, b.w));
+      const float4 o = make_float4(fmaf(w.x + wadd, n.x, b.x), fmaf(w.y + wadd, n.y, b.y), fmaf(w.z + wadd, n.z, b.z), fmaf(w.w + wadd, n.w, b.w));
+      if constexpr (PLANES) norm_tile[(threadIdx.x >> 6) * (H4 + 1) + c] = o;
+      else o4[c] = o;
     }
   }
+  if constexpr (PLANES)
+    norm_planes_store(reinterpret_cast<const float*>(norm_tile), reinterpret_cast<uint4*>(out), (long)blockIdx.x * NORM_PLANES_ROWS, H, Mpad);
 }
 
 __global__ __launch_bounds__(256) void rope_qk_kernel(float* __restrict__ qkv, const float2* __restrict__ tab, long rows, int T, int H, int hd,
@@ -90,7 +119,8 @@
   float4* ptr = reinterpret_cast<float4*>(qkv + row * 3 * H + col);
   const float4 v = *ptr;
   const float2 f0 = tab[(long)t * (hd >> 1) + p], f1 = tab[(long)t * (hd >> 1) + p + 1];
-  *ptr = make_float4(v.x * f0.x - v.y * f0.y, v.y * f0.x + v.x * f0.y, v.z * f1.x - v.w * f1.y, v.w * f1.x + v.z * f1.y);
+  const float2 r0 = rope_rotate(v.x, v.y, f0), r1 = rope_rotate(v.z, v.w, f1);
+  *ptr = make_float4(r0.x, r0.y, r1.x, r1.y);
 }
 
 __global__ __launch_bounds__(256) void swiglu_kernel(const float* __restrict__ u, float* __restrict__ out, long rows, int Fd) {
@@ -184,6 +214,24 @@
   return IXTTS_OK;
 }
 
+static int launch_adaln_rmsnorm_planes(const float* x_dev, const float* wb_dev, const float* g_dev, void* planes_dev, long rows, int T, int H, float eps,
+                                       const int* seq_off_dev, int nseq, void* stream) {
+  const long Mpad = ixtts_gemm_x6_rows_padded(rows);
+  const size_t lds = (size_t)NORM_PLANES_ROWS * (H / 4 + 1) * sizeof(float4);
+  hipLaunchKernelGGL((row_norm_mod_kernel<false, true>), dim3((unsigned)(Mpad / NORM_PLANES_ROWS)), dim3(64 * NORM_PLANES_ROWS), lds, (hipStream_t)stream, x_dev,
+                     wb_dev, wb_dev + H, g_dev, reinterpret_cast<float*>(planes_dev), rows, T, H, (long)2 * H, eps, 0.0f, seq_off_dev, nseq, Mpad);
+  IX_HIP(hipGetLastError());
+  return IXTTS_OK;
+}
+
+extern "C" int ixtts_adaln_rmsnorm_planes_f32(const float* x_dev, const float* wb_dev, const float* g_dev, void* planes_dev, int B, int T, int H, float eps,
+                                              void* stream) {
+  IX_ARG(x_dev && wb_dev && g_dev && planes_dev, "adaln_rmsnorm_planes: null pointer");
+  IX_ARG(B > 0 && T > 0 && H > 0 && H % 64 == 0 && H <= 1024, "adaln_rmsnorm_planes: bad shape B=%d T=%d H=%d (H a multiple of 64, at most 1024)", B, T, H);
+  IX_ARG((reinterpret_cast<uintptr_t>(planes_dev) & 127) == 0, "adaln_rmsnorm_planes: planes must be 128-byte aligned");
+  return launch_adaln_rmsnorm_planes(x_dev, wb_dev, g_dev, planes_dev, (long)B * T, T, H, eps, nullptr, 0, stream);
+}
+
 extern "C" int ixtts_ln_modulate_f32(const float* x_dev, const float* shift_scale_dev, float* out_dev, int B, int T, int H, float eps, void* stream) {
   IX_ARG(x_dev && shift_scale_dev && out_dev, "ln_modulate: null pointer");
   IX_ARG(B > 0 && T > 0 && H > 0 && H % 4 == 0 && H <= 64 * ROW_NV * 4, "ln_modulate: bad shape B=%d T=%d H=%d", B, T, H);
@@ -256,6 +304,15 @@
   return IXTTS_OK;
 }
 
+extern "C" int ixtts_adaln_rmsnorm_planes_varlen_f32(const float* x_dev, const float* wb_dev, const float* g_dev, void* planes_dev, const int* seq_off_dev,
+                                                     int nseq, long rows, int H, float eps, void* stream) {
+  IX_ARG(x_dev && wb_dev && g_dev && planes_dev && seq_off_dev, "adaln_rmsnorm_planes_varlen: null pointer");
+  IX_ARG(nseq > 0 && rows > 0 && H > 0 && H % 64 == 0 && H <= 1024, "adaln_rmsnorm_planes_varlen: bad shape nseq=%d rows=%ld H=%d (H a multiple of 64, at most 1024)",
+         nseq, rows, H);
+  IX_ARG((reinterpret_cast<uintptr_t>(planes_dev) & 127) == 0, "adaln_rmsnorm_planes_varlen: planes must be 128-byte aligned");
+  return launch_adaln_rmsnorm_planes(x_dev, wb_dev, g_dev, planes_dev, rows, 1, H, eps, seq_off_dev, nseq, stream);
+}
+
 extern "C" int ixtts_ln_modulate_varlen_f32(const float* x_dev, const float* shift_scale_dev, float* out_dev, const int* seq_off_dev, int nseq, long rows, int H,
                                             float eps, void* stream) {
   IX_ARG(x_dev && shift_scale_dev && out_dev && seq_off_dev, "ln_modulate_varlen: null pointer");
diff --git a/voice-tts_amd/csrc/gemm_x6.hip b/voice-tts_amd/csrc/gemm_x6.hip
--- a/voice-tts_amd/csrc/gemm_x6.hip
+++ b/voice-tts_amd/csrc/gemm_x6.hip
@@ -26,7 +26,28 @@
   }
 }
 
-__global__ __launch_bounds__(256) void gemm_x6_split_kernel(const float* __restrict__ a, long lda, uint4* __restrict__ out, int M, int K, long Mpad) {
+template <int HALO>
+__device__ __forceinline__ long split_src_row(long rr, int hT, int hleft, int hright, const int* __restrict__ hoff, int hn) {
+  if constexpr (HALO == 0) return rr;
+  long o0;
+  int T = hT;
+  if constexpr (HALO == 1) {
+    o0 = rr / (hleft + hT + hright) * (hleft + hT + hright);
+  } else {
+    const int s = seq_of_row(hoff, hn, rr);
+    o0 = hoff[s];
+    T = hoff[s + 1] - (int)o0 - hleft - hright;
+    if (T <= hleft || T <= hright) return rr;
+  }
+  const int h = (int)(rr - o0);
+  if (h < hleft) return o0 + 2 * hleft - h;
+  if (h >= hleft + T && h < hleft + T + hright) return o0 + 2 * (hleft + T) - 2 - h;
+  return rr;
+}
+
+template <int HALO = 0>
+__global__ __launch_bounds__(256) void gemm_x6_split_kernel(const float* __restrict__ a, long lda, uint4* __restrict__ out, int M, int K, long Mpad, int hT = 0,
+                                                            int hleft = 0, int hright = 0, const int* __restrict__ hoff = nullptr, int hn = 0) {
   __shared__ float tile[64][65];
   const int r0 = blockIdx.x * 64, k0 = blockIdx.y * 64;
   const int t = threadIdx.x;
@@ -34,7 +55,7 @@
   for (int i = 0; i < 4; ++i) {
     const int r = (t >> 4) + 16 * i, kq = t & 15;
     float4 v = make_float4(0.f, 0.f, 0.f, 0.f);
-    if (r0 + r < M) v = *reinterpret_cast<const float4*>(a + (long)(r0 + r) * lda + k0 + 4 * kq);
+    if (r0 + r < M) v = *reinterpret_cast<const float4*>(a + split_src_row<HALO>(r0 + r, hT, hleft, hright, hoff, hn) * lda + k0 + 4 * kq);
     tile[r][4 * kq + 0] = v.x; tile[r][4 * kq + 1] = v.y; tile[r][4 * kq + 2] = v.z; tile[r][4 * kq + 3] = v.w;
   }
   __syncthreads();
@@ -357,8 +378,32 @@
   IX_ARG(a_dev && planes_dev && rows > 0 && K > 0 && K % 64 == 0, "gemm_x6_split: bad argument (K must be a multiple of 64)");
   IX_ARG(lda >= K && lda % 4 == 0 && (reinterpret_cast<uintptr_t>(a_dev) & 15) == 0, "gemm_x6_split: rows must be 16-byte aligned (lda %ld)", lda);
   const long Mpad = ixtts_gemm_x6_rows_padded(rows);
-  hipLaunchKernelGGL(gemm_x6_split_kernel, dim3((unsigned)(Mpad / 64), K / 64), dim3(256), 0, (hipStream_t)stream, a_dev, lda,
+  hipLaunchKernelGGL(gemm_x6_split_kernel<0>, dim3((unsigned)(Mpad / 64), K / 64), dim3(256), 0, (hipStream_t)stream, a_dev, lda,
                      reinterpret_cast<uint4*>(planes_dev), (int)rows, K, Mpad);
+  IX_HIP(hipGetLastError());
+  return IXTTS_OK;
+}
+
+extern "C" int ixtts_gemm_x6_split_halo(const float* a_dev, long lda, void* planes_dev, long rows, int K, int T, int left, int right, void* stream) {
+  IX_ARG(a_dev && planes_dev && rows > 0 && K > 0 && K % 64 == 0, "gemm_x6_split_halo: bad argument (K must be a multiple of 64)");
+  IX_ARG(lda >= K && lda % 4 == 0 && (reinterpret_cast<uintptr_t>(a_dev) & 15) == 0, "gemm_x6_split_halo: rows must be 16-byte aligned (lda %ld)", lda);
+  IX_ARG(left >= 0 && right >= 0 && T > left && T > right && rows % (left + T + right) == 0,
+         "gemm_x6_split_halo: bad shape rows=%ld T=%d left=%d right=%d (rows = whole sequences of left + T + right)", rows, T, left, right);
+  const long Mpad = ixtts_gemm_x6_rows_padded(rows);
+  hipLaunchKernelGGL(gemm_x6_split_kernel<1>, dim3((unsigned)(Mpad / 64), K / 64), dim3(256), 0, (hipStream_t)stream, a_dev, lda,
+                     reinterpret_cast<uint4*>(planes_dev), (int)rows, K, Mpad, T, left, right);
+  IX_HIP(hipGetLastError());
+  return IXTTS_OK;
+}
+
+extern "C" int ixtts_gemm_x6_split_halo_varlen(const float* a_dev, long lda, void* planes_dev, long rows, int K, const int* seq_off_dev, int nseq, int left,
+                                               int right, void* stream) {
+  IX_ARG(a_dev && planes_dev && seq_off_dev && rows > 0 && K > 0 && K % 64 == 0, "gemm_x6_split_halo_varlen: bad argument (K must be a multiple of 64)");
+  IX_ARG(lda >= K && lda % 4 == 0 && (reinterpret_cast<uintptr_t>(a_dev) & 15) == 0, "gemm_x6_split_halo_varlen: rows must be 16-byte aligned (lda %ld)", lda);
+  IX_ARG(nseq > 0 && left >= 0 && right >= 0, "gemm_x6_split_halo_varlen: bad shape nseq=%d left=%d right=%d", nseq, left, right);
+  const long Mpad = ixtts_gemm_x6_rows_padded(rows);
+  hipLaunchKernelGGL(gemm_x6_split_kernel<2>, dim3((unsigned)(Mpad / 64), K / 64), dim3(256), 0, (hipStream_t)stream, a_dev, lda,
+                     reinterpret_cast<uint4*>(planes_dev), (int)rows, K, Mpad, 0, left, right, seq_off_dev, nseq);
   IX_HIP(hipGetLastError());
   return IXTTS_OK;
 }
diff --git a/voice-tts_amd/gemm.py b/voice-tts_amd/gemm.py
--- a/voice-tts_amd/gemm.py
+++ b/voice-tts_amd/gemm.py
@@ -1,4 +1,5 @@
 import ctypes as C
+import os
 
 import torch
 
@@ -37,19 +38,38 @@
         (x.dim() == 1 or (x.stride(-2) % 4 == 0 and x.stride(-2) >= K))
 
 
-def split(x, slot=0):
+def fused():
+    return os.environ.get("IXTTS_S2MEL_FUSED", "1") != "0"
+
+
+def planes_buffer(rows, K, device, slot=0):
+    nbytes = (K // 16) * 6 * int(_lib.lib().ixtts_gemm_x6_rows_padded(rows)) * 16
+    key = (device, nbytes, slot)
+    buf = _POOL.get(key)
+    if buf is None:
+        buf = _POOL[key] = torch.empty(nbytes, dtype=torch.uint8, device=device)
+    return buf
+
+
+def split(x, slot=0, halo=None):
     K = int(x.shape[-1])
     if x.dim() != 2:
         x = x.reshape(-1, K) if x.is_contiguous() else x.contiguous().reshape(-1, K)
     rows, lda = int(x.shape[0]), int(x.stride(0))
     L = _lib.lib()
-    nbytes = (K // 16) * 6 * int(L.ixtts_gemm_x6_rows_padded(rows)) * 16
-    key = (x.device, nbytes, slot)
-    buf = _POOL.get(key)
-    if buf is None:
-        buf = _POOL[key] = torch.empty(nbytes, dtype=torch.uint8, device=x.device)
+    buf = planes_buffer(rows, K, x.device, slot)
     with torch.cuda.device(x.device):
-        _lib.check(L.ixtts_gemm_x6_split(x.data_ptr(), lda, buf.data_ptr(), rows, K, _lib.current_stream_ptr()), "ixtts_gemm_x6_split")
+        if halo is None:
+            _lib.check(L.ixtts_gemm_x6_split(x.data_ptr(), lda, buf.data_ptr(), rows, K, _lib.current_stream_ptr()), "ixtts_gemm_x6_split")
+        elif isinstance(halo[0], int):
+            T, left, right = halo
+            _lib.check(L.ixtts_gemm_x6_split_halo(x.data_ptr(), lda, buf.data_ptr(), rows, K, T, left, right, _lib.current_stream_ptr()),
+                       "ixtts_gemm_x6_split_halo")
+        else:
+            pk, left, right = halo
+            assert rows == pk.rows and min(pk.lens) - left - right > max(left, right)
+            _lib.check(L.ixtts_gemm_x6_split_halo_varlen(x.data_ptr(), lda, buf.data_ptr(), rows, K, pk.tab.data_ptr(), pk.n, left, right,
+                                                         _lib.current_stream_ptr()), "ixtts_gemm_x6_split_halo_varlen")
     return Planes(buf, rows, K)
 
 
diff --git a/voice-tts_amd/s2mel.py b/voice-tts_amd/s2mel.py
--- a/voice-tts_amd/s2mel.py
+++ b/voice-tts_amd/s2mel.py
@@ -101,7 +101,7 @@
     return y[..., : y.shape[-1] - extra]
 
 
-def attn_full(q, k, v, scale=None):
+def attn_full(q, k, v, scale=None, rope=None):
     import ctypes as C
 
     from . import _lib
@@ -116,10 +116,16 @@
     nws = L.ixtts_attn_full_workspace_bytes(B, Hh, T)
     ws = torch.empty(nws, device=q.device, dtype=torch.uint8)
     with torch.cuda.device(q.device):
-        rc = L.ixtts_attn_full_f32(q.data_ptr(), k.data_ptr(), v.data_ptr(), out.data_ptr(), B, Hh, T, d, q.stride(0), q.stride(1),
-                                   q.stride(2), out.stride(0), out.stride(1), out.stride(2), C.c_float(sc), ws.data_ptr(), nws,
-                                   _lib.current_stream_ptr())
-    _lib.check(rc, "ixtts_attn_full_f32")
+        if rope is not None:
+            assert rope.dtype == torch.complex64 and rope.is_contiguous() and rope.shape[0] >= T and rope.shape[1] == d // 2
+            rc = L.ixtts_attn_full_rope_f32(q.data_ptr(), k.data_ptr(), v.data_ptr(), out.data_ptr(), torch.view_as_real(rope).data_ptr(), rope.shape[0], B, Hh,
+                                            T, d, q.stride(0), q.stride(1), q.stride(2), out.stride(0), out.stride(1), out.stride(2), C.c_float(sc),
+                                            ws.data_ptr(), nws, _lib.current_stream_ptr())
+        else:
+            rc = L.ixtts_attn_full_f32(q.data_ptr(), k.data_ptr(), v.data_ptr(), out.data_ptr(), B, Hh, T, d, q.stride(0), q.stride(1),
+                                       q.stride(2), out.stride(0), out.stride(1), out.stride(2), C.c_float(sc), ws.data_ptr(), nws,
+                                       _lib.current_stream_ptr())
+    _lib.check(rc, "ixtts_attn_full_rope_f32" if rope is not None else "ixtts_attn_full_f32")
     return out
 
 
@@ -145,6 +151,23 @@
         return out
     w, b = wb[:, None, :H], wb[:, None, H:]
     return torch.addcmul(b, w, F.rms_norm(x, (H,), g, eps))
+
+
+def adaln_rmsnorm_planes(x, wb, g, eps=1e-5, pk=None):
+    import ctypes as C
+
+    H = x.shape[-1]
+    rows = x.numel() // H
+    x, wb = x.contiguous(), wb.contiguous()
+    buf = G.planes_buffer(rows, H, x.device)
+    with torch.cuda.device(x.device):
+        if pk is None:
+            B, T, _ = x.shape
+            _hip_call("ixtts_adaln_rmsnorm_planes_f32", x.data_ptr(), wb.data_ptr(), g.data_ptr(), buf.data_ptr(), B, T, H, C.c_float(eps))
+        else:
+            _hip_call("ixtts_adaln_rmsnorm_planes_varlen_f32", x.data_ptr(), wb.data_ptr(), g.data_ptr(), buf.data_ptr(), pk.tab.data_ptr(), pk.n, rows, H,
+                      C.c_float(eps))
+    return G.Planes(buf, rows, H)
 
 
 def ln_modulate(x, ss, eps=1e-6):
@@ -281,7 +304,7 @@
     return out
 
 
-def attn_full_packed(q, k, v, pk, scale=None):
+def attn_full_packed(q, k, v, pk, scale=None, rope=None):
     import ctypes as C
 
     from . import _lib
@@ -296,9 +319,16 @@
     nws = L.ixtts_attn_full_varlen_workspace_bytes(pk.n, Hh, pk.tiles)
     ws = torch.empty(nws, device=q.device, dtype=torch.uint8)
     with torch.cuda.device(q.device):
-        rc = L.ixtts_attn_full_varlen_f32(q.data_ptr(), k.data_ptr(), v.data_ptr(), out.data_ptr(), pk.tab.data_ptr(), pk.n, pk.tiles, pk.n_work, Hh, d,
-                                          q.stride(0), q.stride(1), out.stride(0), out.stride(1), C.c_float(sc), ws.data_ptr(), nws, _lib.current_stream_ptr())
-    _lib.check(rc, "ixtts_attn_full_varlen_f32")
+        if rope is not None:
+            assert rope.dtype == torch.complex64 and rope.is_contiguous() and rope.shape[0] >= max(pk.lens) and rope.shape[1] == d // 2
+            rc = L.ixtts_attn_full_rope_varlen_f32(q.data_ptr(), k.data_ptr(), v.data_ptr(), out.data_ptr(), torch.view_as_real(rope).data_ptr(),
+                                                   pk.tab.data_ptr(), pk.n, pk.tiles, pk.n_work, Hh, d, q.stride(0), q.stride(1), out.stride(0), out.stride(1),
+                                                   C.c_float(sc), ws.data_ptr(), nws, _lib.current_stream_ptr())
+        else:
+            rc = L.ixtts_attn_full_varlen_f32(q.data_ptr(), k.data_ptr(), v.data_ptr(), out.data_ptr(), pk.tab.data_ptr(), pk.n, pk.tiles, pk.n_work, Hh, d,
+                                              q.stride(0), q.stride(1), out.stride(0), out.stride(1), C.c_float(sc), ws.data_ptr(), nws,
+                                              _lib.current_stream_ptr())
+    _lib.check(rc, "ixtts_attn_full_rope_varlen_f32" if rope is not None else "ixtts_attn_full_varlen_f32")
     return out
 
 
@@ -417,6 +447,7 @@
         half = 128
         self.t_freqs = torch.exp(-math.log(10000.0) * torch.arange(half, dtype=torch.float32) / half).to(self.device).to(dtype)
         self._rope = None
+        self._t_consts = {}
         W, C_, L = self.W, cfg["in_channels"], cfg["depth"]
         t = "cfm.estimator.transformer."
         self.w13 = [torch.cat([W[t + f"layers.{i}.feed_forward.w1.weight"], W[t + f"layers.{i}.feed_forward.w3.weight"]], 0).contiguous() for i in range(L)]
@@ -493,6 +524,14 @@
         h = F.silu(_lin(emb, self.W, prefix + ".mlp.0"))
         return _lin(h, self.W, prefix + ".mlp.2")
 
+    def _t_const(self, tkey, name, fn):
+        if tkey is None or os.environ.get("IXTTS_S2MEL_TCACHE", "1") == "0":
+            return fn()
+        v = self._t_consts.get((tkey, name))
+        if v is None:
+            v = self._t_consts[(tkey, name)] = fn()
+        return v
+
     def _rope_cache(self, T):
         if self._rope is None or self._rope.shape[0] < T:
             n = self.head_dim
@@ -512,9 +551,11 @@
         H, nh, hd = self.cfg["hidden_dim"], self.cfg["num_heads"], self.head_dim
         fc = self._rope_cache(T)
         if mask is None and hd == 64 and qkv.is_cuda:
+            v4 = qkv.view(B, T, 3, nh, hd)
+            if G.fused() and fc.dtype == torch.complex64 and os.environ.get("IXTTS_ATTN_FULL", "x3") != "f32":
+                return attn_full(v4[:, :, 0], v4[:, :, 1], v4[:, :, 2], rope=fc).reshape(B * T, H)
             with torch.cuda.device(qkv.device):
                 _hip_call("ixtts_rope_qk_f32", qkv.data_ptr(), torch.view_as_real(fc).data_ptr(), B, T, H, hd)
-            v4 = qkv.view(B, T, 3, nh, hd)
             return attn_full(v4[:, :, 0], v4[:, :, 1], v4[:, :, 2]).reshape(B * T, H)
         q, k, v = qkv.view(B, T, 3 * H).split([H, H, H], dim=-1)
         q = self._rotary(q.reshape(B, T, nh, hd), fc)
@@ -523,13 +564,14 @@
         y = F.scaled_dot_product_attention(q.transpose(1, 2), k.transpose(1, 2), v.transpose(1, 2), attn_mask=mask, dropout_p=0.0)
         return y.transpose(1, 2).reshape(B * T, H)
 
-    def _transformer(self, x, c, mask):
+    def _transformer(self, x, c, mask, tkey=None):
         W, cfg = self.W, self.cfg
         B, T, H = x.shape
         L = cfg["depth"]
-        wb_all = F.linear(c, self.proj_w, self.proj_b).view(B, 2 * L + 1, 2 * H).transpose(0, 1).contiguous()
+        wb_all = self._t_const(tkey, "wb_all", lambda: F.linear(c, self.proj_w, self.proj_b).view(B, 2 * L + 1, 2 * H).transpose(0, 1).contiguous())
         x = x.reshape(B * T, H)
         x6 = x.is_cuda and self._x6(self.x6_w13)
+        fuse = G.fused() and H % 64 == 0 and H <= 1024
         skips = []
         for i in range(L):
             p = f"cfm.estimator.transformer.layers.{i}."
@@ -539,8 +581,11 @@
             a = adaln_rmsnorm(x.view(B, T, H), wb_all[2 * i], W[p + "attention_norm.norm.weight"])
             y = self._attention(F.linear(a.view(B * T, H), W[p + "attention.wqkv.weight"]), B, T, mask)
             h = torch.addmm(x, y, W[p + "attention.wo.weight"].t()) if 0 < i <= L // 2 else x.addmm_(y, W[p + "attention.wo.weight"].t())
-            f = adaln_rmsnorm(h.view(B, T, H), wb_all[2 * i + 1], W[p + "ffn_norm.norm.weight"]).view(B * T, H)
-            u = G.pair_linear(f, self.x6_w13[i], G.SWIGLU) if x6 else swiglu(F.linear(f, self.w13[i]))
+            if x6 and fuse:
+                u = G.pair_linear(adaln_rmsnorm_planes(h.view(B, T, H), wb_all[2 * i + 1], W[p + "ffn_norm.norm.weight"]), self.x6_w13[i], G.SWIGLU)
+            else:
+                f = adaln_rmsnorm(h.view(B, T, H), wb_all[2 * i + 1], W[p + "ffn_norm.norm.weight"]).view(B * T, H)
+                u = G.pair_linear(f, self.x6_w13[i], G.SWIGLU) if x6 else swiglu(F.linear(f, self.w13[i]))
             x = h.addmm_(u, W[p + "feed_forward.w2.weight"].t())
             if i < L // 2:
                 skips.append(x)
@@ -601,13 +646,13 @@
             out = torch.bmm(r2, acts) if out is None else out.baddbmm_(r2, acts)
         return out
 
-    def _wavenet_rows(self, h, g):
+    def _wavenet_rows(self, h, g, tkey=None):
         W, cfg = self.W, self.cfg
         Hw, nl, k = cfg["wavenet_hidden"], cfg["wavenet_layers"], cfg["wavenet_kernel"]
         assert cfg["wavenet_dilation_rate"] == 1
         B, T_, _ = h.shape
         p = "cfm.estimator.wavenet."
-        g = F.linear(g, W[p + "cond_layer.conv.conv.weight"][:, :, 0], W[p + "cond_layer.conv.conv.bias"])
+        g = self._t_const(tkey, "wn_cond", lambda: F.linear(g, W[p + "cond_layer.conv.conv.weight"][:, :, 0], W[p + "cond_layer.conv.conv.bias"]))
         tot = k - 1
         right = tot // 2
         left = tot - right
@@ -619,11 +664,15 @@
         centre = P2[left:left + M]
         out = torch.empty(B * Tp, Hw, device=h.device, dtype=h.dtype)
         x6 = self._x6(self.x6_wn)
+        fuse = G.fused()
         for i in range(nl):
-            reflect_halo_rows(P, T_, left, right)
             if x6:
-                acts = G.pair_linear(G.split(P2), self.x6_wn[i], G.GATE, taps=k, gate=g, gate_off=i * 2 * Hw, rows_per_batch=Tp)
-            else:
+                if not fuse:
+                    reflect_halo_rows(P, T_, left, right)
+                acts = G.pair_linear(G.split(P2, halo=(T_, left, right) if fuse else None), self.x6_wn[i], G.GATE, taps=k, gate=g, gate_off=i * 2 * Hw,
+                                     rows_per_batch=Tp)
+            else:
+                reflect_halo_rows(P, T_, left, right)
                 acc = torch.addmm(self.wn_bin[i], P2[:M], self.wn_taps[i][0].t())
                 for j in range(1, k):
                     acc.addmm_(P2[j:j + M], self.wn_taps[i][j].t())
@@ -653,14 +702,16 @@
                 attn_mask = attn_mask.expand(B, 1, T, T)
         return dict(B=B, T=T, base=base, x_mask=x_mask.to(base.dtype), attn_mask=attn_mask, full=full)
 
-    def dit_step(self, ctx, x, t, out_from=0):
+    def dit_step(self, ctx, x, t, out_from=0, tkey=None):
         W, cfg = self.W, self.cfg
         e = "cfm.estimator."
         B, T, base = ctx["B"], ctx["T"], ctx["base"]
         xt = x.transpose(1, 2)
-        t1 = self._t_embed(t, e + "t_embedder")
+        if tkey is not None:
+            tkey = tuple(tkey) + (int(t.shape[0]),)
+        t1 = self._t_const(tkey, "t1", lambda: self._t_embed(t, e + "t_embedder"))
         x_in = base + F.linear(xt, self.merge_x)
-        x_res = self._transformer(x_in, t1, ctx["attn_mask"])
+        x_res = self._transformer(x_in, t1, ctx["attn_mask"], tkey)
         halo = sum((cfg["wavenet_kernel"] - 1) * cfg["wavenet_dilation_rate"] ** i for i in range(cfg["wavenet_layers"])) // 2 + 1
         lo = max(0, out_from - halo) if (ctx["full"] and out_from > 0) else 0
         if lo > 0:
@@ -670,17 +721,17 @@
             extend_tuned_gemms(T, Th)
         x_res = F.linear(x_res, self.skipl_res, W[e + "skip_linear.bias"]) + F.linear(xt, self.skipl_x)
         h = _lin(x_res, W, e + "conv1")
-        t2 = self._t_embed(t, e + "t_embedder2")
+        t2 = self._t_const(tkey, "t2", lambda: self._t_embed(t, e + "t_embedder2"))
         gemm_form = h.is_cuda and ctx["full"] and Th > 2 * cfg["wavenet_kernel"] * cfg["wavenet_dilation_rate"] ** (cfg["wavenet_layers"] - 1)
         if gemm_form and cfg["wavenet_dilation_rate"] == 1:
-            h = self._wavenet_rows(h, t2) + F.linear(x_res, W[e + "res_projection.weight"], W[e + "res_projection.bias"] + self.wn_out_bias)
+            h = self._wavenet_rows(h, t2, tkey) + F.linear(x_res, W[e + "res_projection.weight"], W[e + "res_projection.bias"] + self.wn_out_bias)
         elif gemm_form:
             h = self._wavenet_gemm(h.transpose(1, 2), t2).transpose(1, 2) + F.linear(x_res, W[e + "res_projection.weight"],
                                                                                      W[e + "res_projection.bias"] + self.wn_out_bias)
         else:
             mask = ctx["x_mask"][:, :, lo:] if lo > 0 else ctx["x_mask"]
             h = self._wavenet(h.transpose(1, 2), mask, t2, ctx["full"]).transpose(1, 2) + _lin(x_res, W, e + "res_projection")
-        ss = _lin(F.silu(t1), W, e + "final_layer.adaLN_modulation.1")
+        ss = self._t_const(tkey, "final_ss", lambda: _lin(F.silu(t1), W, e + "final_layer.adaLN_modulation.1"))
         h = ln_modulate(h, ss)
         h = _lin(h, W, e + "final_layer.linear").transpose(1, 2)
         out = conv1d(h, W[e + "conv2.weight"], W[e + "conv2.bias"])
@@ -710,10 +761,10 @@
         for step in range(1, len(t_span)):
             dt = t_span[step] - t_span[step - 1]
             if inference_cfg_rate > 0:
-                d = self.dit_step(ctx, x, torch.stack([t, t]), out_from=skip)
+                d = self.dit_step(ctx, x, torch.stack([t, t]), out_from=skip, tkey=(n_timesteps, step))
                 dphi = (1.0 + inference_cfg_rate) * d[0:1] - inference_cfg_rate * d[1:2]
             else:
-                dphi = self.dit_step(ctx, x, t.expand(B), out_from=skip)
+                dphi = self.dit_step(ctx, x, t.expand(B), out_from=skip, tkey=(n_timesteps, step))
             if skip > 0:
                 x[:, :, skip:] += dt * dphi
             else:
@@ -736,8 +787,11 @@
     def _attention_packed(self, qkv, pk):
         H, nh, hd = self.cfg["hidden_dim"], self.cfg["num_heads"], self.head_dim
         if qkv.is_cuda and hd == 64 and os.environ.get("IXTTS_ATTN_FULL", "x3") != "f32":
-            rope_qk_packed(qkv, self._rope_cache(max(pk.lens)), pk, hd)
+            fc = self._rope_cache(max(pk.lens))
             v4 = qkv.view(pk.rows, 3, nh, hd)
+            if G.fused() and fc.dtype == torch.complex64:
+                return attn_full_packed(v4[:, 0], v4[:, 1], v4[:, 2], pk, rope=fc).view(pk.rows, H)
+            rope_qk_packed(qkv, fc, pk, hd)
             return attn_full_packed(v4[:, 0], v4[:, 1], v4[:, 2], pk).view(pk.rows, H)
         out = torch.empty(pk.rows, H, device=qkv.device, dtype=qkv.dtype)
         if qkv.is_cuda:
@@ -758,6 +812,7 @@
         H, L = cfg["hidden_dim"], cfg["depth"]
         wb_all = F.linear(c, self.proj_w, self.proj_b).view(pk.n, 2 * L + 1, 2 * H).transpose(0, 1).contiguous()
         x6 = x.is_cuda and self._x6(self.x6_w13)
+        fuse = G.fused() and H % 64 == 0 and H <= 1024
         skips = []
         for i in range(L):
             p = f"cfm.estimator.transformer.layers.{i}."
@@ -767,8 +822,11 @@
             a = adaln_rmsnorm_packed(x, wb_all[2 * i], W[p + "attention_norm.norm.weight"], pk)
             y = self._attention_packed(F.linear(a, W[p + "attention.wqkv.weight"]), pk)
             h = torch.addmm(x, y, W[p + "attention.wo.weight"].t()) if 0 < i <= L // 2 else x.addmm_(y, W[p + "attention.wo.weight"].t())
-            f = adaln_rmsnorm_packed(h, wb_all[2 * i + 1], W[p + "ffn_norm.norm.weight"], pk)
-            u = G.pair_linear(f, self.x6_w13[i], G.SWIGLU) if x6 else swiglu(F.linear(f, self.w13[i]))
+            if x6 and fuse:
+                u = G.pair_linear(adaln_rmsnorm_planes(h, wb_all[2 * i + 1], W[p + "ffn_norm.norm.weight"], pk=pk), self.x6_w13[i], G.SWIGLU)
+            else:
+                f = adaln_rmsnorm_packed(h, wb_all[2 * i + 1], W[p + "ffn_norm.norm.weight"], pk)
+                u = G.pair_linear(f, self.x6_w13[i], G.SWIGLU) if x6 else swiglu(F.linear(f, self.w13[i]))
             x = h.addmm_(u, W[p + "feed_forward.w2.weight"].t())
             if i < L // 2:
                 skips.append(x)
@@ -790,11 +848,15 @@
         centre = P2[left:left + M]
         out = torch.empty(pp.rows, Hw, device=h.device, dtype=h.dtype)
         x6 = h.is_cuda and self._x6(self.x6_wn)
+        fuse = G.fused()
         for i in range(nl):
-            reflect_halo_rows_packed(P2, pp, left, right)
             if x6:
-                acts = G.pair_linear(G.split(P2), self.x6_wn[i], G.GATE, taps=k, gate=g, gate_off=i * 2 * Hw, seq_off=pp)
-            else:
+                if not fuse:
+                    reflect_halo_rows_packed(P2, pp, left, right)
+                acts = G.pair_linear(G.split(P2, halo=(pp, left, right) if fuse else None), self.x6_wn[i], G.GATE, taps=k, gate=g, gate_off=i * 2 * Hw,
+                                     seq_off=pp)
+            else:
+                reflect_halo_rows_packed(P2, pp, left, right)
                 acc = torch.addmm(self.wn_bin[i], P2[:M], self.wn_taps[i][0].t())
                 for j in range(1, k):
                     acc.addmm_(P2[j:j + M], self.wn_taps[i][j].t())
```
